# Totoro97/f2-nerf

Hardware: NVIDIA B200
Metric: training rays/sec (higher is better)
Workload: dtype f32 march/composite, f16 hash table + MLP operands (f32 accumulate)

## Files before the change

f2nerf_b200/_lib.py:

```python
import ctypes
import os

import torch

_HERE = os.path.dirname(os.path.abspath(__file__))
LIB_PATH = os.path.join(_HERE, "libf2nerf_b200.so")


class F2BError(RuntimeError):
    """Raised when a C-ABI call returns a negative status (message from f2b_last_error)."""


def _load():
    if not os.path.exists(LIB_PATH):
        raise ImportError(
            f"f2nerf_b200: CUDA extension {LIB_PATH} is missing — run `python -c 'import __graft_entry__ as g; g.build()'` "
            "(or `make`) first; there is no CPU fallback.")
    lib = ctypes.CDLL(LIB_PATH)
    lib.f2b_last_error.restype = ctypes.c_char_p
    return lib


lib = _load()

c_int, c_float, c_void_p, c_i64 = ctypes.c_int, ctypes.c_float, ctypes.c_void_p, ctypes.c_int64

_P = c_void_p
SIGNATURES = {
    "f2b_abi_version": [],
    "f2b_device_info": [_P, _P],
    "f2b_sampler_count": [_P, c_int, _P, c_int, _P, _P, _P, c_int, c_float, c_float, c_float, c_int, c_int, c_int, _P, _P, _P, _P],
    "f2b_sampler_fill": [_P, c_int, _P, c_int, _P, _P, _P, c_int, c_float, c_float, c_float, c_int, c_int, _P, _P, _P, _P, _P, _P, _P, _P],
    "f2b_sampler_march": [_P, c_int, _P, c_int, _P, _P, _P, c_int, c_float, c_float, c_float, c_int, c_int, c_int, _P, _P, _P, _P,
                          _P, _P, _P, _P, _P],
    "f2b_sampler_march_bg": [_P, c_int, _P, c_int, _P, _P, _P, c_int, c_float, c_float, c_float, c_int, c_int, c_int, _P, _P, _P, _P,
                             _P, _P, _P, _P, _P],
    "f2b_sampler_gather": [_P, _P, c_int, _P, _P, _P, _P, _P, _P, _P, _P, _P, _P],
    "f2b_edge_samples": [_P, _P, _P, _P, c_int, _P, _P, _P],
    "f2b_oct_mark_visit": [_P, c_int, _P, c_int, _P, _P, _P, _P, _P, _P, _P],
    "f2b_oct_update_stats": [_P, _P, _P, _P, _P, _P, c_int, _P],
    "f2b_hash_level_scales": [_P],
    "f2b_table_to_half": [_P, _P, c_i64, _P],
    "f2b_hash_fwd": [_P, _P, _P, c_int, c_int, _P, _P, c_int, c_int, _P, _P],
    "f2b_hash_fwd_levels": [_P, _P, _P, c_int, c_int, _P, _P, c_int, c_int, c_int, c_int, _P, _P],
    "f2b_hash_bwd": [_P, _P, c_int, c_int, _P, _P, c_int, c_int, _P, c_int, c_float, _P, _P],
    "f2b_hash_bwd_levels": [_P, _P, c_int, c_int, _P, _P, c_int, c_int, _P, c_int, c_float, _P, c_int, c_int, _P],
    "f2b_mlp_fwd": [_P, _P, c_int, c_int, _P, _P, _P],
    "f2b_mlp_fwd_f32": [_P, _P, c_int, c_int, _P, _P, _P, _P],
    "f2b_mlp_bwd": [_P, _P, _P, _P, c_int, c_int, _P, _P, _P],
    "f2b_field_shade_fwd": [_P, _P, _P, _P, _P, c_int, _P, _P, _P, _P],
    "f2b_shader_mlp_rgb_fwd": [_P, _P, c_int, _P, _P, _P, _P],
    "f2b_mlp_bwd2": [_P, _P, _P, _P, _P, c_int, c_int, _P, _P, _P],
    "f2b_mlp_fwd_v0": [_P, _P, c_int, c_int, _P, _P, _P],
    "f2b_mlp_bwd_v0": [_P, _P, _P, _P, c_int, c_int, _P, _P, _P],
    "f2b_mlp_fwd_tc": [_P, _P, c_int, c_int, _P, _P, _P],
    "f2b_mlp_bwd_tc": [_P, _P, _P, _P, c_int, c_int, _P, _P, _P],
    "f2b_field_fwd": [_P, _P, _P, c_int, c_int, _P, _P, _P, c_int, c_int, c_int, _P, _P, _P, _P],
    "f2b_field_fwd_slots": [_P, _P, _P, c_int, c_int, _P, _P, _P, c_int, _P, c_int, c_int, c_int, _P, _P, _P],
    "f2b_set_mlp_impl": [c_int],
    "f2b_get_mlp_impl": [],
    "f2b_cast_f32_to_f16": [_P, _P, c_i64, c_float, _P],
    "f2b_cast_f16_to_f32": [_P, _P, c_i64, c_float, _P],
    "f2b_sh_encode": [_P, c_int, c_int, _P, _P],
    "f2b_scatter_idx": [_P, _P, c_int, _P, _P],
    "f2b_shader_prep": [_P, _P, _P, _P, c_int, _P, _P],
    "f2b_shader_act": [_P, c_int, _P, _P],
    "f2b_shader_act_bwd": [_P, _P, c_int, c_float, _P, _P],
    "f2b_shader_prep_bwd": [_P, _P, _P, c_int, c_float, _P, _P, _P],
    "f2b_shader_prep_bwd_f16": [_P, _P, _P, _P, c_int, c_float, c_float, _P, _P, _P],
    "f2b_octree_proc": [_P, _P, _P, _P, c_int, c_int, c_int, _P, _P, _P, _P, _P, _P, _P],
    "f2b_octree_mark_invisible": [_P, c_int, _P, _P, _P, c_int, _P],
    "f2b_img2world_rays": [_P, _P, _P, _P, _P, c_int, _P, _P, _P],
    "f2b_gather_pixels": [_P, _P, _P, c_int, c_int, c_int, _P, _P],
    "f2b_adam_step": [_P, _P, _P, _P, c_i64, c_i64, ctypes.c_double, ctypes.c_double, ctypes.c_double, ctypes.c_double,
                      ctypes.c_double, c_i64, _P, _P],
    "f2b_early_stop": [_P, c_int, _P, _P, c_int, _P, _P, _P, _P, _P, _P, _P],
    "f2b_early_stop_rays": [_P, c_int, _P, _P, c_int, _P, _P, _P, _P, _P],
    "f2b_count_scan": [_P, c_int, _P, _P, _P],
    "f2b_slot_bounds": [_P, c_int, c_int, c_int, _P, _P],
    "f2b_compact_slots": [_P, _P, _P, c_int, _P, _P, _P, _P, _P, _P, _P, _P, _P, _P, _P, _P, _P],
    "f2b_compact_samples": [_P, _P, _P, c_int, _P, _P, _P, _P, _P, _P, _P, _P, _P, _P, _P, _P, _P],
    "f2b_composite_fwd": [_P, c_int, _P, _P, _P, _P, _P, c_int, _P, _P, _P, _P, _P],
    "f2b_composite_bwd": [_P, c_int, _P, _P, _P, _P, _P, c_int, _P, _P, _P, _P, c_float, _P, c_int, _P, _P],
    "f2b_composite_act_bwd": [_P, c_int, _P, _P, _P, _P, _P, c_int, _P, _P, _P, _P, c_float, _P, c_float, _P, c_int, _P, _P],
    "f2b_flex_sum": [_P, c_int, _P, c_int, _P, _P],
    "f2b_flex_accumulate_sum": [_P, _P, c_int, c_int, _P, _P],
    "f2b_weight_var_fwd": [_P, _P, c_int, _P, _P],
    "f2b_weight_var_bwd": [_P, _P, c_int, _P, _P, _P],
    "f2b_render_fwd_fused": [_P, _P, _P, c_int, c_int, _P, _P, _P, _P, _P, _P, _P, _P, _P, c_int, c_int, _P, _P, _P, _P, _P, _P, _P, _P],
    "f2b_gather_kept_weights": [_P, _P, c_int, c_int, _P, _P],
}



class RenderArgs(ctypes.Structure):
    _P, _I, _F, _L = c_void_p, c_int, c_float, c_i64
    _fields_ = [
        ("tree_nodes", _P), ("n_nodes", _I), ("trans", _P), ("n_trans", _I), ("edge_pool", _P),
        ("near_t", _F), ("far_t", _F), ("sample_l", _F), ("scale_by_dis", _I), ("max_hits", _I), ("count_all_hits", _I),
        ("table16", _P), ("prim", _P), ("bias", _P), ("n_volumes", _I), ("local_size", _I),
        ("field_params", _P), ("n_field_params", _I), ("shader_params", _P), ("n_shader_params", _I),
        ("fparams16", _P), ("sparams16", _P),
        ("app_emb", _P), ("n_emb", _I),
        ("n_rays", _I), ("rays_o", _P), ("rays_d", _P), ("noise", _P), ("bg", _P),
        ("ray_emb_idx", _P),
        ("skip_march", _I),
        ("s_pts", _P), ("s_dt", _P), ("s_t", _P), ("s_anchors", _P), ("counts", _P), ("chunk_bounds", _P), ("slot_bounds", _P),
        ("first_oct_dis", _P), ("totals", _P),
        ("logit_s", _P), ("feat_s", _P), ("w0", _P), ("a0", _P), ("keep", _P), ("kept_counts", _P), ("new_bounds", _P), ("total_kept", _P),
        ("n_kept", _I), ("n_edge_pairs", _I),
        ("pts", _P), ("dirs", _P), ("dt", _P), ("t", _P), ("anchors", _P), ("feat_q", _P),
        ("edge_idx", _P), ("edge_coord", _P), ("e_pts", _P), ("e_anc", _P),
        ("pt_emb_idx", _P),
        ("logit", _P), ("mlp_in", _P), ("f_hidden", _P), ("edge32", _P), ("raw", _P), ("rgb", _P), ("s_hidden", _P),
        ("colors", _P), ("disparity", _P), ("depth", _P), ("weights", _P),
        ("d_colors", _P), ("d_disparity", _P), ("d_depth", _P), ("d_weights", _P), ("d_edge", _P),
        ("gs_progress", _F), ("shader_loss_scale", _F), ("field_loss_scale", _F), ("table_grad_mul", _F),
        ("d_logit", _P), ("d_raw", _P), ("d_in16", _P), ("d_scene16", _P), ("dfeat16", _P),
        ("d_sparams", _P), ("d_fparams", _P), ("d_table", _P), ("table_numel", _L), ("table_live", _L), ("d_app", _P),
        ("scatter_mode", _I),
        ("nonfinite", _P),
        ("stream", _P), ("side_stream", _P),
    ]

    def set(self, **kw):
        for k, v in kw.items():
            if isinstance(v, torch.Tensor):
                if not v.is_contiguous():
                    raise ValueError(f"f2nerf_b200: tensor {k} crossing the C ABI must be contiguous")
                v = v.data_ptr()
            setattr(self, k, v)
        return self


SIGNATURES["f2b_render_sizeof"] = []
for _name in ("f2b_render_phase1", "f2b_render_phase2_fwd", "f2b_render_bwd", "f2b_render_grad_finalize"):
    SIGNATURES[_name] = [ctypes.POINTER(RenderArgs)]
lib.f2b_render_sizeof.restype = c_int
lib.f2b_render_sizeof.argtypes = []
if lib.f2b_render_sizeof() != ctypes.sizeof(RenderArgs):
    raise ImportError(f"f2nerf_b200: struct f2b_render is {lib.f2b_render_sizeof()} bytes in the library but "
                      f"{ctypes.sizeof(RenderArgs)} in the binding — header / _lib.py out of step")

for _name, _args in SIGNATURES.items():
    _fn = getattr(lib, _name)
    _fn.argtypes = _args
    _fn.restype = c_int


def ptr(t):
    if t is None:
        return None
    if isinstance(t, torch.Tensor):
        if not t.is_contiguous():
            raise ValueError("f2nerf_b200: tensor crossing the C ABI must be contiguous")
        return t.data_ptr()
    return t


def stream():
    return torch.cuda.current_stream().cuda_stream


KERNELS_PER_CALL = {"f2b_render_sizeof": 0, "f2b_render_phase1": 7, "f2b_render_phase2_fwd": 10, "f2b_render_bwd": 8, "f2b_render_grad_finalize": 2,
                    "f2b_sampler_count": 2, "f2b_sampler_march": 2, "f2b_sampler_march_bg": 2, "f2b_early_stop": 2, "f2b_hash_level_scales": 1, "f2b_device_info": 0,
                    "f2b_abi_version": 0, "f2b_set_mlp_impl": 0, "f2b_get_mlp_impl": 0}
LAUNCHES = 0
TRACE = None


def call(name, *args):
    global LAUNCHES
    fn = getattr(lib, name)
    conv = [ptr(a) if isinstance(a, torch.Tensor) or a is None else (ctypes.byref(a) if isinstance(a, ctypes.Structure) else a)
            for a in args]
    if TRACE is not None:
        e0, e1 = torch.cuda.Event(enable_timing=True), torch.cuda.Event(enable_timing=True)
        e0.record()
        rc = fn(*conv)
        e1.record()
        TRACE.append((name, e0, e1, [a for a in args if isinstance(a, int) and not isinstance(a, bool)]))
    else:
        rc = fn(*conv)
    if rc != 0:
        raise F2BError(f"{name} -> {rc}: {lib.f2b_last_error().decode()}")
    LAUNCHES += KERNELS_PER_CALL.get(name, 1)
    return rc
```

f2nerf_b200/csrc/hash.cu:

```cuda
#include "common.cuh"
#include "hash.cuh"
#include <stdlib.h>

namespace f2b {

__global__ void __launch_bounds__(128)
hash_fwd_kernel(const __half* __restrict__ table, const int* __restrict__ prim_pool,
                const float* __restrict__ bias_pool, int n_volumes, int local_size,
                const float* __restrict__ pts, const int* __restrict__ vol, int vol_stride, int n_pts,
                __half* __restrict__ out) {
  __shared__ float s_scale[F2B_N_LEVELS];
  if (threadIdx.x < F2B_N_LEVELS) s_scale[threadIdx.x] = level_scale(threadIdx.x);
  __syncthreads();
  const int i = blockIdx.x * blockDim.x + threadIdx.x;
  if (i >= n_pts) return;
  uint32_t o[16];
  encode_point(table, prim_pool, bias_pool, n_volumes, local_size, s_scale, __ldg(pts + size_t(i) * 3),
               __ldg(pts + size_t(i) * 3 + 1), __ldg(pts + size_t(i) * 3 + 2),
               __ldg(vol + size_t(i) * vol_stride), o);
  uint4* dst = reinterpret_cast<uint4*>(out + size_t(i) * 32);
#pragma unroll
  for (int q = 0; q < 4; q++) dst[q] = make_uint4(o[4 * q], o[4 * q + 1], o[4 * q + 2], o[4 * q + 3]);
}

__global__ void __launch_bounds__(128)
hash_fwd_levels_kernel(const __half* __restrict__ table, const int* __restrict__ prim_pool,
                       const float* __restrict__ bias_pool, int n_volumes, int local_size,
                       const float* __restrict__ pts, const int* __restrict__ vol, int vol_stride, int n_pts,
                       int level_lo, int n_levels, __half* __restrict__ out) {
  __shared__ float s_scale[F2B_N_LEVELS];
  if (threadIdx.x < F2B_N_LEVELS) s_scale[threadIdx.x] = level_scale(threadIdx.x);
  __syncthreads();
  const int i = blockIdx.x * blockDim.x + threadIdx.x;
  if (i >= n_pts) return;
  const float p0 = __ldg(pts + size_t(i) * 3), p1 = __ldg(pts + size_t(i) * 3 + 1), p2 = __ldg(pts + size_t(i) * 3 + 2);
  const float x0 = fmul(fadd(p0, 1.f), .5f), x1 = fmul(fadd(p1, 1.f), .5f), x2 = fmul(fadd(p2, 1.f), .5f);
  const int v = __ldg(vol + size_t(i) * vol_stride);
  uint32_t* dst = reinterpret_cast<uint32_t*>(out + size_t(i) * 32);
  for (int l = level_lo; l < level_lo + n_levels; l++) {
    const int tv = l * n_volumes + v;
    Corner8 c;
    corners(x0, x1, x2, s_scale[l], prim_pool + tv * 3, bias_pool + tv * 3, (unsigned)local_size, c);
    dst[l] = encode_level(table, l, local_size, c);
  }
}

constexpr int kDirectHeads = 24;

template <bool GRAD_F16>
__device__ __forceinline__ void hash_bwd_task(int64_t group, int l, int lane, const int* __restrict__ prim_pool,
                                              const float* __restrict__ bias_pool, int n_volumes, int local_size,
                                              const float* __restrict__ pts, const int* __restrict__ vol, int vol_stride, int n_pts,
                                              const void* __restrict__ grad_feat, float grad_mul, float* __restrict__ grad_table) {
  const int64_t i = group * 32 + lane;
  const bool valid = i < n_pts;
  float g0 = 0.f, g1 = 0.f;
  if (valid) {
    if (GRAD_F16) {
      const float2 gf = __half22float2(reinterpret_cast<const __half2*>(grad_feat)[i * 16 + l]);
      g0 = gf.x; g1 = gf.y;
    } else {
      const float2 gf = reinterpret_cast<const float2*>(grad_feat)[i * 16 + l];
      g0 = gf.x; g1 = gf.y;
    }
  }
  const bool live = valid && !(g0 == 0.f && g1 == 0.f);
  if (!__any_sync(0xffffffffu, live)) return;
  g0 *= grad_mul; g1 *= grad_mul;
  Corner8 c;
  int v = -1;
  if (live) {
    const float p0 = __ldg(pts + i * 3), p1 = __ldg(pts + i * 3 + 1), p2 = __ldg(pts + i * 3 + 2);
    const float x0 = fmul(fadd(p0, 1.f), .5f), x1 = fmul(fadd(p1, 1.f), .5f), x2 = fmul(fadd(p2, 1.f), .5f);
    v = __ldg(vol + i * vol_stride);
    const int tv = l * n_volumes + v;
    corners(x0, x1, x2, level_scale(l), prim_pool + tv * 3, bias_pool + tv * 3, (unsigned)local_size, c);
  } else {
#pragma unroll
    for (int k = 0; k < 8; k++) { c.idx[k] = 0; c.w[k] = 0.f; }
    c.cell[0] = c.cell[1] = c.cell[2] = 0;
  }
  const unsigned pcx = __shfl_up_sync(0xffffffffu, c.cell[0], 1), pcy = __shfl_up_sync(0xffffffffu, c.cell[1], 1),
                 pcz = __shfl_up_sync(0xffffffffu, c.cell[2], 1);
  const int prev_v = __shfl_up_sync(0xffffffffu, v, 1);
  const bool head = (lane == 0) || !live || c.cell[0] != pcx || c.cell[1] != pcy || c.cell[2] != pcz || v != prev_v;
  const unsigned heads = __ballot_sync(0xffffffffu, head);
  float* base = grad_table + size_t(l) * local_size;
  if (__popc(heads) > kDirectHeads) {
    if (live) {
#pragma unroll
      for (int k = 0; k < 8; k++)
        atomicAdd(reinterpret_cast<float2*>(base + size_t(c.idx[k]) * 2), make_float2(c.w[k] * g0, c.w[k] * g1));
    }
    return;
  }
  const unsigned below = heads & ((2u << lane) - 1u);
  const int run_start = 31 - __clz(below);
  float s[16];
#pragma unroll
  for (int k = 0; k < 8; k++) { s[2 * k] = c.w[k] * g0; s[2 * k + 1] = c.w[k] * g1; }
  const int max_run = __reduce_max_sync(0xffffffffu, lane - run_start + 1);
#pragma unroll
  for (int o = 1; o < 32; o <<= 1) {
    if (o >= max_run) break;
    const bool take = (lane - o) >= run_start;
#pragma unroll
    for (int k = 0; k < 16; k++) {
      const float u = __shfl_up_sync(0xffffffffu, s[k], o);
      if (take) s[k] += u;
    }
  }
  const bool tail = (lane == 31) || ((heads >> (lane + 1)) & 1u);
  if (live && tail) {
#pragma unroll
    for (int k = 0; k < 8; k++)
      atomicAdd(reinterpret_cast<float2*>(base + size_t(c.idx[k]) * 2), make_float2(s[2 * k], s[2 * k + 1]));
  }
}

template <bool GRAD_F16>
__global__ void __launch_bounds__(256)
hash_bwd_kernel(const int* __restrict__ prim_pool, const float* __restrict__ bias_pool, int n_volumes,
                int local_size, const float* __restrict__ pts, const int* __restrict__ vol,
                int vol_stride, int n_pts, const void* __restrict__ grad_feat, float grad_mul,
                float* __restrict__ grad_table, int64_t n_tasks, int level_lo, int log2_levels) {
  const int lane = threadIdx.x & 31;
  const int64_t stride = (int64_t(gridDim.x) * blockDim.x) >> 5;
  const int lmask = (1 << log2_levels) - 1;
  int k = 0;
  for (int64_t w = (int64_t(blockIdx.x) * blockDim.x + threadIdx.x) >> 5; w < n_tasks; w += stride, k++)
    hash_bwd_task<GRAD_F16>(w >> log2_levels, level_lo + ((int(w & lmask) + k) & lmask), lane, prim_pool, bias_pool, n_volumes, local_size,
                            pts, vol, vol_stride, n_pts, grad_feat, grad_mul, grad_table);
}

__global__ void level_scales_kernel(float* out) {
  if (threadIdx.x < F2B_N_LEVELS) out[threadIdx.x] = level_scale(threadIdx.x);
}

}

using namespace f2b;

extern "C" int f2b_hash_level_scales(float* scales16_host) {
  F2B_REQUIRE(scales16_host, "f2b_hash_level_scales: null pointer");
  float* d = nullptr;
  if (cudaMalloc(&d, 16 * sizeof(float)) != cudaSuccess) { set_error("f2b_hash_level_scales: cudaMalloc failed"); cudaGetLastError(); return F2B_ECUDA; }
  level_scales_kernel<<<1, 32>>>(d);
  cudaError_t e = cudaMemcpy(scales16_host, d, 16 * sizeof(float), cudaMemcpyDeviceToHost);
  cudaFree(d);
  if (e != cudaSuccess) { set_error("f2b_hash_level_scales: %s", cudaGetErrorString(e)); return F2B_ECUDA; }
  return F2B_OK;
}

extern "C" int f2b_hash_fwd(const void* table_f16, const int* prim_pool, const float* bias_pool,
                            int n_volumes, int local_size, const float* pts, const int* vol,
                            int vol_stride, int n_pts, void* out_f16, void* stream) {
  if (n_pts <= 0) return F2B_OK;
  F2B_REQUIRE(table_f16 && prim_pool && bias_pool && pts && vol && out_f16, "f2b_hash_fwd: null pointer");
  F2B_REQUIRE(n_volumes > 0 && local_size > 0 && (local_size % 2) == 0, "f2b_hash_fwd: bad n_volumes/local_size");
  hash_fwd_kernel<<<div_up(n_pts, 128), 128, 0, as_stream(stream)>>>(
      (const __half*)table_f16, prim_pool, bias_pool, n_volumes, local_size, pts, vol, vol_stride, n_pts,
      (__half*)out_f16);
  return check_launch("f2b_hash_fwd");
}

extern "C" int f2b_hash_fwd_levels(const void* table_f16, const int* prim_pool, const float* bias_pool,
                                   int n_volumes, int local_size, const float* pts, const int* vol,
                                   int vol_stride, int n_pts, int level_lo, int n_levels, void* out_f16, void* stream) {
  if (n_pts <= 0) return F2B_OK;
  F2B_REQUIRE(table_f16 && prim_pool && bias_pool && pts && vol && out_f16, "f2b_hash_fwd_levels: null pointer");
  F2B_REQUIRE(n_volumes > 0 && local_size > 0 && (local_size % 2) == 0, "f2b_hash_fwd_levels: bad n_volumes/local_size");
  F2B_REQUIRE(level_lo >= 0 && n_levels > 0 && level_lo + n_levels <= F2B_N_LEVELS, "f2b_hash_fwd_levels: level range outside [0,16)");
  hash_fwd_levels_kernel<<<div_up(n_pts, 128), 128, 0, as_stream(stream)>>>(
      (const __half*)table_f16, prim_pool, bias_pool, n_volumes, local_size, pts, vol, vol_stride, n_pts, level_lo, n_levels,
      (__half*)out_f16);
  return check_launch("f2b_hash_fwd_levels");
}

extern "C" int f2b_hash_bwd_levels(const int* prim_pool, const float* bias_pool, int n_volumes, int local_size,
                                   const float* pts, const int* vol, int vol_stride, int n_pts,
                                   const void* grad_feat, int grad_is_f16, float grad_mul, float* grad_table,
                                   int level_lo, int n_levels, void* stream) {
  if (n_pts <= 0) return F2B_OK;
  F2B_REQUIRE(prim_pool && bias_pool && pts && vol && grad_feat && grad_table, "f2b_hash_bwd: null pointer");
  F2B_REQUIRE(n_levels > 0 && (n_levels & (n_levels - 1)) == 0 && level_lo >= 0 && level_lo + n_levels <= F2B_N_LEVELS,
              "f2b_hash_bwd_levels: n_levels must be a power of two and the range inside [0,16)");
  int log2_levels = 0;
  while ((1 << log2_levels) < n_levels) log2_levels++;
  const int64_t n_tasks = int64_t(div_up(n_pts, 32)) * n_levels;
  static int ctas_per_sm = -1;
  if (ctas_per_sm < 0) { const char* e = getenv("F2B_SCATTER_CTAS"); ctas_per_sm = e ? atoi(e) : 8; if (ctas_per_sm < 1) ctas_per_sm = 1; }
  int sms = 148;
  f2b_device_info(&sms, nullptr);
  const int64_t want = div_up(n_tasks * 32, int64_t(256));
  int blocks = int(want < int64_t(sms) * ctas_per_sm ? want : int64_t(sms) * ctas_per_sm);
  if (blocks < want && ((blocks * 8) % n_levels) != 0) blocks = blocks > 1 ? blocks - 1 : int(want);
  if (grad_is_f16)
    hash_bwd_kernel<true><<<blocks, 256, 0, as_stream(stream)>>>(prim_pool, bias_pool, n_volumes, local_size, pts, vol, vol_stride,
                                                                 n_pts, grad_feat, grad_mul, grad_table, n_tasks, level_lo, log2_levels);
  else
    hash_bwd_kernel<false><<<blocks, 256, 0, as_stream(stream)>>>(prim_pool, bias_pool, n_volumes, local_size, pts, vol, vol_stride,
                                                                  n_pts, grad_feat, grad_mul, grad_table, n_tasks, level_lo, log2_levels);
  return check_launch("f2b_hash_bwd");
}

extern "C" int f2b_hash_bwd(const int* prim_pool, const float* bias_pool, int n_volumes, int local_size,
                            const float* pts, const int* vol, int vol_stride, int n_pts,
                            const void* grad_feat, int grad_is_f16, float grad_mul, float* grad_table,
                            void* stream) {
  return f2b_hash_bwd_levels(prim_pool, bias_pool, n_volumes, local_size, pts, vol, vol_stride, n_pts, grad_feat, grad_is_f16, grad_mul,
                             grad_table, 0, F2B_N_LEVELS, stream);
}
```

f2nerf_b200/csrc/hash.cuh:

```cuda
#pragma once
#include "common.cuh"

namespace f2b {

__device__ __forceinline__ float level_scale(int l) {
  return exp2f(fadd(fdiv((float)(7 * l), 15.f), 3.f));
}

struct Corner8 {
  unsigned idx[8];
  float w[8];
  unsigned cell[3];
};

__device__ __forceinline__ void corners(float x0, float x1, float x2, float scale,
                                        const int* __restrict__ prim, const float* __restrict__ bias,
                                        unsigned local_size, Corner8& c) {
  const float px = ffma(x0, scale, __ldg(bias)), py = ffma(x1, scale, __ldg(bias + 1)),
              pz = ffma(x2, scale, __ldg(bias + 2));
  const float fx = floorf(px), fy = floorf(py), fz = floorf(pz);
  const unsigned ix = (unsigned)fx, iy = (unsigned)fy, iz = (unsigned)fz;
  c.cell[0] = ix; c.cell[1] = iy; c.cell[2] = iz;
  const unsigned pa = (unsigned)__ldg(prim), pb = (unsigned)__ldg(prim + 1), pc = (unsigned)__ldg(prim + 2);
  const unsigned hx0 = ix * pa, hx1 = hx0 + pa, hy0 = iy * pb, hy1 = hy0 + pb, hz0 = iz * pc, hz1 = hz0 + pc;
  const bool pow2 = (local_size & (local_size - 1)) == 0;
  const unsigned mask = local_size - 1;
#define F2B_MOD(v) (pow2 ? ((v) & mask) : ((v) % local_size))
  c.idx[0] = F2B_MOD(hx0 ^ hy0 ^ hz0);
  c.idx[1] = F2B_MOD(hx0 ^ hy0 ^ hz1);
  c.idx[2] = F2B_MOD(hx0 ^ hy1 ^ hz0);
  c.idx[3] = F2B_MOD(hx0 ^ hy1 ^ hz1);
  c.idx[4] = F2B_MOD(hx1 ^ hy0 ^ hz0);
  c.idx[5] = F2B_MOD(hx1 ^ hy0 ^ hz1);
  c.idx[6] = F2B_MOD(hx1 ^ hy1 ^ hz0);
  c.idx[7] = F2B_MOD(hx1 ^ hy1 ^ hz1);
#undef F2B_MOD
  const float a = fsub(px, fx), b = fsub(py, fy), cc = fsub(pz, fz);
  const float na = fsub(1.f, a), nb = fsub(1.f, b), nc = fsub(1.f, cc);
  const float nanb = fmul(na, nb), nab = fmul(na, b), anb = fmul(a, nb), ab = fmul(a, b);
  c.w[0] = fmul(nanb, nc); c.w[1] = fmul(cc, nanb);
  c.w[2] = fmul(nab, nc);  c.w[3] = fmul(nab, cc);
  c.w[4] = fmul(anb, nc);  c.w[5] = fmul(cc, anb);
  c.w[6] = fmul(ab, nc);   c.w[7] = fmul(ab, cc);
}

__device__ __forceinline__ uint32_t ldg_nc_u32(const void* p) {
  uint32_t v;
  asm volatile("ld.global.nc.b32 %0, [%1];" : "=r"(v) : "l"(p));
  return v;
}

__device__ __forceinline__ uint32_t encode_level(const __half* __restrict__ table, int l, int local_size,
                                                 const Corner8& c) {
  const __half* base = table + size_t(l) * local_size;
  uint32_t raw[8];
#pragma unroll
  for (int k = 0; k < 8; k++) raw[k] = ldg_nc_u32(base + size_t(c.idx[k]) * 2);
  float2 f[8];
#pragma unroll
  for (int k = 0; k < 8; k++) f[k] = __half22float2(*reinterpret_cast<const __half2*>(&raw[k]));
  float a0 = fmul(c.w[1], f[1].x), a1 = fmul(c.w[1], f[1].y);
  a0 = ffma(c.w[0], f[0].x, a0); a1 = ffma(c.w[0], f[0].y, a1);
#pragma unroll
  for (int k = 2; k < 8; k++) { a0 = ffma(c.w[k], f[k].x, a0); a1 = ffma(c.w[k], f[k].y, a1); }
  const __half2 h = __floats2half2_rn(a0, a1);
  return *reinterpret_cast<const uint32_t*>(&h);
}

__device__ __forceinline__ void encode_point(const __half* __restrict__ table,
                                             const int* __restrict__ prim_pool,
                                             const float* __restrict__ bias_pool, int n_volumes,
                                             int local_size, const float* scales, float p0, float p1,
                                             float p2, int v, uint32_t out[16]) {
  const float x0 = fmul(fadd(p0, 1.f), .5f), x1 = fmul(fadd(p1, 1.f), .5f), x2 = fmul(fadd(p2, 1.f), .5f);
#pragma unroll
  for (int l = 0; l < F2B_N_LEVELS; l++) {
    const int tv = l * n_volumes + v;
    Corner8 c;
    corners(x0, x1, x2, scales[l], prim_pool + tv * 3, bias_pool + tv * 3, (unsigned)local_size, c);
    out[l] = encode_level(table, l, local_size, c);
  }
}

}
```

f2nerf_b200/csrc/mlp_tc_bwd.cu:

```cuda
#include "common.cuh"
#include "tc.cuh"

namespace f2b {
using namespace tc;

constexpr int kBT = 128;

template <int NH>
struct BwdSmem {
  static constexpr int W0 = 0;
  static constexpr int WH = 4096;
  static constexpr int WO = NH ? 12288 : 4096;
  static constexpr int STAGE0 = WO + 2048;
  static constexpr int DO = 0;
  static constexpr int X = 4096;
  static constexpr int H0 = 12288;
  static constexpr int H1 = 28672;
  static constexpr int STAGE_BYTES = NH ? 45056 : 28672;
  static constexpr int BAR = STAGE0 + 2 * STAGE_BYTES;
  static constexpr int BYTES = BAR + 64 + 1024;
  static constexpr int TMEM_COLS = NH ? 256 : 128;
  static constexpr int C_ACT = 0, C_GW0 = 64, C_GWO = 96, C_GWH = 128;
};

__device__ __forceinline__ uint32_t pk(float a, float b) {
  const __half2 h = __floats2half2_rn(a, b);
  return *reinterpret_cast<const uint32_t*>(&h);
}

__device__ __forceinline__ uint64_t mnmajor_desc(uint32_t tile, int row_bytes, int k_step) {
  const uint64_t layout = row_bytes == 128 ? kLayoutSW128 : (row_bytes == 64 ? kLayoutSW64 : kLayoutSW32);
  return make_desc(tile + k_step * 16 * row_bytes, 16, 8 * row_bytes, layout);
}

template <int K>
__device__ __forceinline__ void stage_w(const __half* __restrict__ w, int rows, unsigned char* dst) {
  constexpr int chunks = K / 8;
  for (int i = threadIdx.x; i < rows * chunks; i += blockDim.x) {
    const int r = i / chunks, c = i % chunks;
    *reinterpret_cast<uint4*>(dst + (K == 64 ? sw128_off(r, c) : sw64_off(r, c))) = *reinterpret_cast<const uint4*>(w + r * K + c * 8);
  }
}

__device__ __forceinline__ void cp16(uint32_t dst, const void* src, uint32_t src_bytes) {
  asm volatile("cp.async.cg.shared.global [%0], [%1], 16, %2;" ::"r"(dst), "l"(src), "r"(src_bytes) : "memory");
}

template <int NH>
__device__ __forceinline__ void prefetch_tile(const __half* __restrict__ dout, const __half* __restrict__ in,
                                              const __half* __restrict__ hidden, const __half* __restrict__ hid_last,
                                              int tile, int n_pts, uint32_t stage) {
  using S = BwdSmem<NH>;
  const int rows = min(kBT, n_pts - tile * kBT);
  const size_t t0 = size_t(tile) * kBT;
  const unsigned char* s_do = reinterpret_cast<const unsigned char*>(dout + t0 * 16);
  const unsigned char* s_x = reinterpret_cast<const unsigned char*>(in + t0 * 32);
  const unsigned char* s_h0 = reinterpret_cast<const unsigned char*>(hidden + t0 * 64);
  const unsigned char* s_h1 = reinterpret_cast<const unsigned char*>(hid_last + t0 * 64);
#pragma unroll
  for (int j = 0; j < 2; j++) {
    const int c = threadIdx.x + kBT * j, r = c >> 1;
    const bool ok = r < rows;
    cp16(stage + S::DO + sw32_off(r, c & 1), s_do + (ok ? size_t(c) * 16 : 0), ok ? 16u : 0u);
  }
#pragma unroll
  for (int j = 0; j < 4; j++) {
    const int c = threadIdx.x + kBT * j, r = c >> 2;
    const bool ok = r < rows;
    cp16(stage + S::X + sw64_off(r, c & 3), s_x + (ok ? size_t(c) * 16 : 0), ok ? 16u : 0u);
  }
#pragma unroll
  for (int j = 0; j < 8; j++) {
    const int c = threadIdx.x + kBT * j, r = c >> 3;
    const bool ok = r < rows;
    cp16(stage + S::H0 + sw128_off(r, c & 7), s_h0 + (ok ? size_t(c) * 16 : 0), ok ? 16u : 0u);
    if (NH) cp16(stage + S::H1 + sw128_off(r, c & 7), s_h1 + (ok ? size_t(c) * 16 : 0), ok ? 16u : 0u);
  }
}

__device__ __forceinline__ void relu_bwd_epilogue(uint32_t tmem_row, const unsigned char* h_tile, unsigned char* dh_tile, int row) {
#pragma unroll
  for (int q = 0; q < 4; q++) {
    uint32_t r[16];
    tmem_ld16(tmem_row + 16 * q, r);
    tmem_ld_wait();
    uint4 hv[2], o[2];
    hv[0] = *reinterpret_cast<const uint4*>(h_tile + sw128_off(row, 2 * q));
    hv[1] = *reinterpret_cast<const uint4*>(h_tile + sw128_off(row, 2 * q + 1));
    const __half2* hh = reinterpret_cast<const __half2*>(hv);
    uint32_t* ow = reinterpret_cast<uint32_t*>(o);
#pragma unroll
    for (int e = 0; e < 8; e++) {
      const float2 hf = __half22float2(hh[e]);
      ow[e] = pk(hf.x > 0.f ? __uint_as_float(r[2 * e]) : 0.f, hf.y > 0.f ? __uint_as_float(r[2 * e + 1]) : 0.f);
    }
    *reinterpret_cast<uint4*>(dh_tile + sw128_off(row, 2 * q)) = o[0];
    *reinterpret_cast<uint4*>(dh_tile + sw128_off(row, 2 * q + 1)) = o[1];
  }
}

template <int NH>
__global__ void __launch_bounds__(kBT)
mlp_bwd_tc_kernel(const __half* __restrict__ dout, const __half* __restrict__ in, const __half* __restrict__ hidden,
                  const __half* __restrict__ hid_last, const __half* __restrict__ params, int n_pts,
                  __half* __restrict__ din, float* __restrict__ dparams) {
  using S = BwdSmem<NH>;
  extern __shared__ unsigned char smem_raw[];
  unsigned char* sm = reinterpret_cast<unsigned char*>((reinterpret_cast<uintptr_t>(smem_raw) + 1023) & ~uintptr_t(1023));
  uint64_t* mbar = reinterpret_cast<uint64_t*>(sm + S::BAR);
  uint32_t* tmem_slot = reinterpret_cast<uint32_t*>(sm + S::BAR + 8);
  const int tid = threadIdx.x, warp = tid >> 5, lane = tid & 31;
  const int n_tiles = (n_pts + kBT - 1) / kBT;
  const uint32_t stage0 = smem_u32(sm + S::STAGE0);

  int tile = blockIdx.x;
  if (tile < n_tiles) prefetch_tile<NH>(dout, in, hidden, hid_last, tile, n_pts, stage0);
  asm volatile("cp.async.commit_group;" ::: "memory");
  stage_w<32>(params, 64, sm + S::W0);
  if (NH) stage_w<64>(params + 64 * 32, 64, sm + S::WH);
  stage_w<64>(params + 64 * 32 + NH * 64 * 64, 16, sm + S::WO);
  if (tid == 0) mbar_init(mbar, 1);
  if (warp == 0) tmem_alloc(tmem_slot, S::TMEM_COLS);
  fence_before_sync();
  __syncthreads();
  fence_after_sync();
  const uint32_t tmem = *tmem_slot;
  const uint32_t tmem_row = tmem + (uint32_t(warp * 32) << 16);
  const uint32_t s_w0 = smem_u32(sm + S::W0), s_wh = smem_u32(sm + S::WH), s_wo = smem_u32(sm + S::WO);
  constexpr uint32_t id_act64 = idesc_f16_f32(128, 64, 0, 1);
  constexpr uint32_t id_act32 = idesc_f16_f32(128, 32, 0, 1);
  constexpr uint32_t id_gw16 = idesc_f16_f32(64, 16, 1, 1);
  constexpr uint32_t id_gw32 = idesc_f16_f32(64, 32, 1, 1);
  constexpr uint32_t id_gw64 = idesc_f16_f32(64, 64, 1, 1);
  uint32_t phase = 0, first = 1, buf = 0;

  for (; tile < n_tiles; tile += gridDim.x, buf ^= 1) {
    const int p = tile * kBT + tid;
    const bool valid = p < n_pts;
    const int next = tile + gridDim.x;
    if (next < n_tiles) prefetch_tile<NH>(dout, in, hidden, hid_last, next, n_pts, stage0 + (buf ^ 1) * S::STAGE_BYTES);
    asm volatile("cp.async.commit_group;" ::: "memory");
    asm volatile("cp.async.wait_group 1;" ::: "memory");
    fence_async_smem();
    fence_before_sync();
    __syncthreads();
    unsigned char* const st = sm + S::STAGE0 + buf * S::STAGE_BYTES;
    const uint32_t sb = stage0 + buf * S::STAGE_BYTES;
    const uint32_t s_do = sb + S::DO, s_x = sb + S::X, s_h0 = sb + S::H0, s_h1 = sb + S::H1;
    const uint32_t s_hl = NH ? s_h1 : s_h0;
    const uint32_t acc = (first ^ 1);
    if (tid == 0) {
      fence_after_sync();
      mma_f16(tmem + S::C_ACT, kmajor_desc(s_do, 32), mnmajor_desc(s_wo, 128, 0), id_act64, 0);
#pragma unroll
      for (int k = 0; k < 8; k++)
        mma_f16(tmem + S::C_GWO, mnmajor_desc(s_hl, 128, k), mnmajor_desc(s_do, 32, k), id_gw16, (k > 0) | acc);
      mma_commit(mbar);
    }
    mbar_wait(mbar, phase); phase ^= 1;
    fence_after_sync();
    relu_bwd_epilogue(tmem_row + S::C_ACT, st + (NH ? S::H1 : S::H0), st + (NH ? S::H1 : S::H0), tid);
    fence_before_sync();
    fence_async_smem();
    __syncthreads();
    if (NH) {
      if (tid == 0) {
        fence_after_sync();
#pragma unroll
        for (int k = 0; k < 4; k++)
          mma_f16(tmem + S::C_ACT, kmajor_desc(s_h1 + 32 * k, 128), mnmajor_desc(s_wh, 128, k), id_act64, k);
#pragma unroll
        for (int k = 0; k < 8; k++)
          mma_f16(tmem + S::C_GWH, mnmajor_desc(s_h1, 128, k), mnmajor_desc(s_h0, 128, k), id_gw64, (k > 0) | acc);
        mma_commit(mbar);
      }
      mbar_wait(mbar, phase); phase ^= 1;
      fence_after_sync();
      relu_bwd_epilogue(tmem_row + S::C_ACT, st + S::H0, st + S::H0, tid);
      fence_before_sync();
      fence_async_smem();
      __syncthreads();
    }
    if (tid == 0) {
      fence_after_sync();
#pragma unroll
      for (int k = 0; k < 4; k++)
        mma_f16(tmem + S::C_ACT, kmajor_desc(s_h0 + 32 * k, 128), mnmajor_desc(s_w0, 64, k), id_act32, k);
#pragma unroll
      for (int k = 0; k < 8; k++)
        mma_f16(tmem + S::C_GW0, mnmajor_desc(s_h0, 128, k), mnmajor_desc(s_x, 64, k), id_gw32, (k > 0) | acc);
      mma_commit(mbar);
    }
    first = 0;
    mbar_wait(mbar, phase); phase ^= 1;
    fence_after_sync();
    {
#pragma unroll
      for (int q = 0; q < 2; q++) {
        uint32_t r[16];
        tmem_ld16(tmem_row + S::C_ACT + 16 * q, r);
        tmem_ld_wait();
        if (din && valid) {
          uint4 o[2];
          uint32_t* ow = reinterpret_cast<uint32_t*>(o);
#pragma unroll
          for (int e = 0; e < 8; e++) ow[e] = pk(__uint_as_float(r[2 * e]), __uint_as_float(r[2 * e + 1]));
          uint4* dst = reinterpret_cast<uint4*>(din + size_t(p) * 32) + 2 * q;
          dst[0] = o[0]; dst[1] = o[1];
        }
      }
    }
  }
  asm volatile("cp.async.wait_group 0;" ::: "memory");
  fence_before_sync();
  __syncthreads();
  if (!first) {
    fence_after_sync();
    const int row = warp * 16 + lane;
    float* g0 = dparams;
    float* gh = dparams + 64 * 32;
    float* go = gh + NH * 64 * 64;
#pragma unroll
    for (int q = 0; q < 2; q++) {
      uint32_t r[16];
      tmem_ld16(tmem_row + S::C_GW0 + 16 * q, r);
      tmem_ld_wait();
      if (lane < 16)
#pragma unroll
        for (int e = 0; e < 16; e++) atomicAdd(g0 + row * 32 + 16 * q + e, __uint_as_float(r[e]));
    }
    {
      uint32_t r[16];
      tmem_ld16(tmem_row + S::C_GWO, r);
      tmem_ld_wait();
      if (lane < 16)
#pragma unroll
        for (int e = 0; e < 16; e++) atomicAdd(go + e * 64 + row, __uint_as_float(r[e]));
    }
    if (NH) {
#pragma unroll
      for (int q = 0; q < 4; q++) {
        uint32_t r[16];
        tmem_ld16(tmem_row + S::C_GWH + 16 * q, r);
        tmem_ld_wait();
        if (lane < 16)
#pragma unroll
          for (int e = 0; e < 16; e++) atomicAdd(gh + row * 64 + 16 * q + e, __uint_as_float(r[e]));
      }
    }
    fence_before_sync();
  }
  __syncthreads();
  if (warp == 0) tmem_dealloc(tmem, S::TMEM_COLS);
}


template <int NH>
struct RcSmem {
  static constexpr int W0 = 0;
  static constexpr int WH = 4096;
  static constexpr int WO = NH ? 12288 : 4096;
  static constexpr int H0 = WO + 2048;
  static constexpr int H1 = H0 + 16384;
  static constexpr int D1 = H1 + 16384;
  static constexpr int STAGE0 = NH ? D1 + 16384 : H0 + 16384;
  static constexpr int DO = 0;
  static constexpr int X = 4096;
  static constexpr int STAGE_BYTES = 12288;
  static constexpr int BAR = STAGE0 + 2 * STAGE_BYTES;
  static constexpr int BYTES = BAR + 64 + 1024;
  static constexpr int TMEM_COLS = NH ? 256 : 128;
  static constexpr int C_ACT = 0, C_GW0 = 64, C_GWO = 96, C_GWH = 128, C_ACT2 = 192;
};

template <int NH>
__device__ __forceinline__ void prefetch_tile_rc(const __half* __restrict__ dout, const __half* __restrict__ in, int tile, int n_pts,
                                                 uint32_t stage) {
  using S = RcSmem<NH>;
  const int rows = min(kBT, n_pts - tile * kBT);
  const size_t t0 = size_t(tile) * kBT;
  const unsigned char* s_do = reinterpret_cast<const unsigned char*>(dout + t0 * 16);
  const unsigned char* s_x = reinterpret_cast<const unsigned char*>(in + t0 * 32);
#pragma unroll
  for (int j = 0; j < 2; j++) {
    const int c = threadIdx.x + kBT * j, r = c >> 1;
    const bool ok = r < rows;
    cp16(stage + S::DO + sw32_off(r, c & 1), s_do + (ok ? size_t(c) * 16 : 0), ok ? 16u : 0u);
  }
#pragma unroll
  for (int j = 0; j < 4; j++) {
    const int c = threadIdx.x + kBT * j, r = c >> 2;
    const bool ok = r < rows;
    cp16(stage + S::X + sw64_off(r, c & 3), s_x + (ok ? size_t(c) * 16 : 0), ok ? 16u : 0u);
  }
}

__device__ __forceinline__ void relu_fwd_epilogue(uint32_t tmem_row, unsigned char* h_tile, int row) {
#pragma unroll
  for (int q = 0; q < 4; q++) {
    uint32_t r[16];
    tmem_ld16(tmem_row + 16 * q, r);
    tmem_ld_wait();
    uint4 o[2];
    uint32_t* ow = reinterpret_cast<uint32_t*>(o);
#pragma unroll
    for (int e = 0; e < 8; e++) ow[e] = pk(fmaxf(__uint_as_float(r[2 * e]), 0.f), fmaxf(__uint_as_float(r[2 * e + 1]), 0.f));
    *reinterpret_cast<uint4*>(h_tile + sw128_off(row, 2 * q)) = o[0];
    *reinterpret_cast<uint4*>(h_tile + sw128_off(row, 2 * q + 1)) = o[1];
  }
}

__device__ __forceinline__ void relu_fwd_mask_epilogue(uint32_t tmem_h, uint32_t tmem_g, unsigned char* h_tile, unsigned char* d_tile, int row) {
#pragma unroll
  for (int q = 0; q < 4; q++) {
    uint32_t r[16], g[16];
    tmem_ld16(tmem_h + 16 * q, r);
    tmem_ld16(tmem_g + 16 * q, g);
    tmem_ld_wait();
    uint4 o[2], d[2];
    uint32_t* ow = reinterpret_cast<uint32_t*>(o);
    uint32_t* dw = reinterpret_cast<uint32_t*>(d);
#pragma unroll
    for (int e = 0; e < 8; e++) {
      const __half2 h = __floats2half2_rn(fmaxf(__uint_as_float(r[2 * e]), 0.f), fmaxf(__uint_as_float(r[2 * e + 1]), 0.f));
      ow[e] = *reinterpret_cast<const uint32_t*>(&h);
      const float2 hf = __half22float2(h);
      dw[e] = pk(hf.x > 0.f ? __uint_as_float(g[2 * e]) : 0.f, hf.y > 0.f ? __uint_as_float(g[2 * e + 1]) : 0.f);
    }
    *reinterpret_cast<uint4*>(h_tile + sw128_off(row, 2 * q)) = o[0];
    *reinterpret_cast<uint4*>(h_tile + sw128_off(row, 2 * q + 1)) = o[1];
    *reinterpret_cast<uint4*>(d_tile + sw128_off(row, 2 * q)) = d[0];
    *reinterpret_cast<uint4*>(d_tile + sw128_off(row, 2 * q + 1)) = d[1];
  }
}

template <int NH>
__global__ void __launch_bounds__(kBT)
mlp_bwd_rc_kernel(const __half* __restrict__ dout, const __half* __restrict__ in, const __half* __restrict__ params, int n_pts,
                  __half* __restrict__ din, float* __restrict__ dparams) {
  using S = RcSmem<NH>;
  extern __shared__ unsigned char smem_raw[];
  unsigned char* sm = reinterpret_cast<unsigned char*>((reinterpret_cast<uintptr_t>(smem_raw) + 1023) & ~uintptr_t(1023));
  uint64_t* mbar = reinterpret_cast<uint64_t*>(sm + S::BAR);
  uint32_t* tmem_slot = reinterpret_cast<uint32_t*>(sm + S::BAR + 8);
  const int tid = threadIdx.x, warp = tid >> 5, lane = tid & 31;
  const int n_tiles = (n_pts + kBT - 1) / kBT;
  const uint32_t stage0 = smem_u32(sm + S::STAGE0);

  int tile = blockIdx.x;
  if (tile < n_tiles) prefetch_tile_rc<NH>(dout, in, tile, n_pts, stage0);
  asm volatile("cp.async.commit_group;" ::: "memory");
  stage_w<32>(params, 64, sm + S::W0);
  if (NH) stage_w<64>(params + 64 * 32, 64, sm + S::WH);
  stage_w<64>(params + 64 * 32 + NH * 64 * 64, 16, sm + S::WO);
  if (tid == 0) mbar_init(mbar, 1);
  if (warp == 0) tmem_alloc(tmem_slot, S::TMEM_COLS);
  fence_before_sync();
  __syncthreads();
  fence_after_sync();
  const uint32_t tmem = *tmem_slot;
  const uint32_t tmem_row = tmem + (uint32_t(warp * 32) << 16);
  const uint32_t s_w0 = smem_u32(sm + S::W0), s_wh = smem_u32(sm + S::WH), s_wo = smem_u32(sm + S::WO);
  const uint32_t s_h0 = smem_u32(sm + S::H0), s_h1 = smem_u32(sm + S::H1), s_d1 = smem_u32(sm + S::D1);
  constexpr uint32_t id_fwd64 = idesc_f16_f32(128, 64);
  constexpr uint32_t id_act64 = idesc_f16_f32(128, 64, 0, 1);
  constexpr uint32_t id_act32 = idesc_f16_f32(128, 32, 0, 1);
  constexpr uint32_t id_gw16 = idesc_f16_f32(64, 16, 1, 1);
  constexpr uint32_t id_gw32 = idesc_f16_f32(64, 32, 1, 1);
  constexpr uint32_t id_gw64 = idesc_f16_f32(64, 64, 1, 1);
  uint32_t phase = 0, first = 1, buf = 0;

  for (; tile < n_tiles; tile += gridDim.x, buf ^= 1) {
    const int p = tile * kBT + tid;
    const bool valid = p < n_pts;
    const int next = tile + gridDim.x;
    if (next < n_tiles) prefetch_tile_rc<NH>(dout, in, next, n_pts, stage0 + (buf ^ 1) * S::STAGE_BYTES);
    asm volatile("cp.async.commit_group;" ::: "memory");
    asm volatile("cp.async.wait_group 1;" ::: "memory");
    fence_async_smem();
    fence_before_sync();
    __syncthreads();
    const uint32_t sb = stage0 + buf * S::STAGE_BYTES;
    const uint32_t s_do = sb + S::DO, s_x = sb + S::X;
    const uint32_t acc = (first ^ 1);
    if (tid == 0) {
      fence_after_sync();
#pragma unroll
      for (int k = 0; k < 2; k++) mma_f16(tmem + S::C_ACT, kmajor_desc(s_x + 32 * k, 64), kmajor_desc(s_w0 + 32 * k, 64), id_fwd64, k);
      if (NH) mma_f16(tmem + S::C_ACT2, kmajor_desc(s_do, 32), mnmajor_desc(s_wo, 128, 0), id_act64, 0);
      mma_commit(mbar);
    }
    mbar_wait(mbar, phase); phase ^= 1;
    fence_after_sync();
    relu_fwd_epilogue(tmem_row + S::C_ACT, sm + S::H0, tid);
    fence_before_sync();
    fence_async_smem();
    __syncthreads();
    if (NH) {
      if (tid == 0) {
        fence_after_sync();
#pragma unroll
        for (int k = 0; k < 4; k++) mma_f16(tmem + S::C_ACT, kmajor_desc(s_h0 + 32 * k, 128), kmajor_desc(s_wh + 32 * k, 128), id_fwd64, k);
        mma_commit(mbar);
      }
      mbar_wait(mbar, phase); phase ^= 1;
      fence_after_sync();
      relu_fwd_mask_epilogue(tmem_row + S::C_ACT, tmem_row + S::C_ACT2, sm + S::H1, sm + S::D1, tid);
      fence_before_sync();
      fence_async_smem();
      __syncthreads();
      if (tid == 0) {
        fence_after_sync();
#pragma unroll
        for (int k = 0; k < 8; k++)
          mma_f16(tmem + S::C_GWO, mnmajor_desc(s_h1, 128, k), mnmajor_desc(s_do, 32, k), id_gw16, (k > 0) | acc);
#pragma unroll
        for (int k = 0; k < 4; k++)
          mma_f16(tmem + S::C_ACT, kmajor_desc(s_d1 + 32 * k, 128), mnmajor_desc(s_wh, 128, k), id_act64, k);
#pragma unroll
        for (int k = 0; k < 8; k++)
          mma_f16(tmem + S::C_GWH, mnmajor_desc(s_d1, 128, k), mnmajor_desc(s_h0, 128, k), id_gw64, (k > 0) | acc);
        mma_commit(mbar);
      }
    } else {
      if (tid == 0) {
        fence_after_sync();
        mma_f16(tmem + S::C_ACT, kmajor_desc(s_do, 32), mnmajor_desc(s_wo, 128, 0), id_act64, 0);
#pragma unroll
        for (int k = 0; k < 8; k++)
          mma_f16(tmem + S::C_GWO, mnmajor_desc(s_h0, 128, k), mnmajor_desc(s_do, 32, k), id_gw16, (k > 0) | acc);
        mma_commit(mbar);
      }
    }
    mbar_wait(mbar, phase); phase ^= 1;
    fence_after_sync();
    relu_bwd_epilogue(tmem_row + S::C_ACT, sm + S::H0, sm + S::H0, tid);
    fence_before_sync();
    fence_async_smem();
    __syncthreads();
    if (tid == 0) {
      fence_after_sync();
#pragma unroll
      for (int k = 0; k < 4; k++)
        mma_f16(tmem + S::C_ACT, kmajor_desc(s_h0 + 32 * k, 128), mnmajor_desc(s_w0, 64, k), id_act32, k);
#pragma unroll
      for (int k = 0; k < 8; k++)
        mma_f16(tmem + S::C_GW0, mnmajor_desc(s_h0, 128, k), mnmajor_desc(s_x, 64, k), id_gw32, (k > 0) | acc);
      mma_commit(mbar);
    }
    first = 0;
    mbar_wait(mbar, phase); phase ^= 1;
    fence_after_sync();
#pragma unroll
    for (int q = 0; q < 2; q++) {
      uint32_t r[16];
      tmem_ld16(tmem_row + S::C_ACT + 16 * q, r);
      tmem_ld_wait();
      if (din && valid) {
        uint4 o[2];
        uint32_t* ow = reinterpret_cast<uint32_t*>(o);
#pragma unroll
        for (int e = 0; e < 8; e++) ow[e] = pk(__uint_as_float(r[2 * e]), __uint_as_float(r[2 * e + 1]));
        uint4* dst = reinterpret_cast<uint4*>(din + size_t(p) * 32) + 2 * q;
        dst[0] = o[0]; dst[1] = o[1];
      }
    }
  }
  asm volatile("cp.async.wait_group 0;" ::: "memory");
  fence_before_sync();
  __syncthreads();
  if (!first) {
    fence_after_sync();
    const int row = warp * 16 + lane;
    float* g0 = dparams;
    float* gh = dparams + 64 * 32;
    float* go = gh + NH * 64 * 64;
#pragma unroll
    for (int q = 0; q < 2; q++) {
      uint32_t r[16];
      tmem_ld16(tmem_row + S::C_GW0 + 16 * q, r);
      tmem_ld_wait();
      if (lane < 16)
#pragma unroll
        for (int e = 0; e < 16; e++) atomicAdd(g0 + row * 32 + 16 * q + e, __uint_as_float(r[e]));
    }
    {
      uint32_t r[16];
      tmem_ld16(tmem_row + S::C_GWO, r);
      tmem_ld_wait();
      if (lane < 16)
#pragma unroll
        for (int e = 0; e < 16; e++) atomicAdd(go + e * 64 + row, __uint_as_float(r[e]));
    }
    if (NH) {
#pragma unroll
      for (int q = 0; q < 4; q++) {
        uint32_t r[16];
        tmem_ld16(tmem_row + S::C_GWH + 16 * q, r);
        tmem_ld_wait();
        if (lane < 16)
#pragma unroll
          for (int e = 0; e < 16; e++) atomicAdd(gh + row * 64 + 16 * q + e, __uint_as_float(r[e]));
      }
    }
    fence_before_sync();
  }
  __syncthreads();
  if (warp == 0) tmem_dealloc(tmem, S::TMEM_COLS);
}

}

using namespace f2b;

extern "C" int f2b_mlp_bwd2_tc(const void* dout_f16, const void* in_f16, const void* hidden0_f16, const void* hidden1_f16,
                               const void* params_f16, int n_hidden_matmuls, int n_pts, void* din_f16,
                               float* dparams_f32, void* stream) {
  if (n_pts <= 0) return F2B_OK;
  F2B_REQUIRE(dout_f16 && in_f16 && params_f16 && dparams_f32, "f2b_mlp_bwd: null pointer");
  F2B_REQUIRE(n_hidden_matmuls == 0 || n_hidden_matmuls == 1, "f2b_mlp_bwd: n_hidden_matmuls must be 0 or 1");
  int sms = 148;
  f2b_device_info(&sms, nullptr);
  const int n_tiles = div_up(n_pts, kBT);
  if (!hidden0_f16) {
    if (n_hidden_matmuls == 0) {
      const int grid = n_tiles < sms * 4 ? n_tiles : sms * 4;
      cudaFuncSetAttribute(mlp_bwd_rc_kernel<0>, cudaFuncAttributeMaxDynamicSharedMemorySize, RcSmem<0>::BYTES);
      mlp_bwd_rc_kernel<0><<<grid, kBT, RcSmem<0>::BYTES, as_stream(stream)>>>((const __half*)dout_f16, (const __half*)in_f16,
                                                                              (const __half*)params_f16, n_pts, (__half*)din_f16, dparams_f32);
    } else {
      const int grid = n_tiles < sms * 2 ? n_tiles : sms * 2;
      cudaFuncSetAttribute(mlp_bwd_rc_kernel<1>, cudaFuncAttributeMaxDynamicSharedMemorySize, RcSmem<1>::BYTES);
      mlp_bwd_rc_kernel<1><<<grid, kBT, RcSmem<1>::BYTES, as_stream(stream)>>>((const __half*)dout_f16, (const __half*)in_f16,
                                                                              (const __half*)params_f16, n_pts, (__half*)din_f16, dparams_f32);
    }
    return check_launch("f2b_mlp_bwd(tcgen05, recompute)");
  }
  F2B_REQUIRE(n_hidden_matmuls == 0 || hidden1_f16, "f2b_mlp_bwd: hidden1 missing (n_hidden_matmuls == 1 with saved activations)");
  if (n_hidden_matmuls == 0) {
    const int grid = n_tiles < sms * 3 ? n_tiles : sms * 3;
    cudaFuncSetAttribute(mlp_bwd_tc_kernel<0>, cudaFuncAttributeMaxDynamicSharedMemorySize, BwdSmem<0>::BYTES);
    mlp_bwd_tc_kernel<0><<<grid, kBT, BwdSmem<0>::BYTES, as_stream(stream)>>>(
        (const __half*)dout_f16, (const __half*)in_f16, (const __half*)hidden0_f16, (const __half*)hidden0_f16,
        (const __half*)params_f16, n_pts, (__half*)din_f16, dparams_f32);
  } else {
    const int grid = n_tiles < sms * 2 ? n_tiles : sms * 2;
    cudaFuncSetAttribute(mlp_bwd_tc_kernel<1>, cudaFuncAttributeMaxDynamicSharedMemorySize, BwdSmem<1>::BYTES);
    mlp_bwd_tc_kernel<1><<<grid, kBT, BwdSmem<1>::BYTES, as_stream(stream)>>>(
        (const __half*)dout_f16, (const __half*)in_f16, (const __half*)hidden0_f16, (const __half*)hidden1_f16,
        (const __half*)params_f16, n_pts, (__half*)din_f16, dparams_f32);
  }
  return check_launch("f2b_mlp_bwd(tcgen05)");
}

extern "C" int f2b_mlp_bwd_tc(const void* dout_f16, const void* in_f16, const void* hidden_save_f16,
                              const void* params_f16, int n_hidden_matmuls, int n_pts, void* din_f16,
                              float* dparams_f32, void* stream) {
  if (n_pts <= 0) return F2B_OK;
  F2B_REQUIRE(hidden_save_f16, "f2b_mlp_bwd: null pointer");
  const __half* h = (const __half*)hidden_save_f16;
  return f2b_mlp_bwd2_tc(dout_f16, in_f16, h, h + size_t(n_hidden_matmuls ? 1 : 0) * n_pts * 64, params_f16, n_hidden_matmuls, n_pts,
                         din_f16, dparams_f32, stream);
}
```

f2nerf_b200/csrc/render.cu:

```cuda
#include "common.cuh"

namespace f2b {

__global__ void finalize_small_kernel(float* __restrict__ d_sparams, int n_s, float inv_s, float* __restrict__ d_fparams, int n_f,
                                      float inv_f, const float* __restrict__ d_app, int n_app, int* __restrict__ flags) {
  const int i = blockIdx.x * blockDim.x + threadIdx.x;
  int bad_s = 0, bad_f = 0;
  if (i < n_s) { const float v = d_sparams[i] * inv_s; d_sparams[i] = v; bad_s |= !isfinite(v); }
  if (i < n_f) { const float v = d_fparams[i] * inv_f; d_fparams[i] = v; bad_f |= !isfinite(v); }
  if (d_app && i < n_app) bad_s |= !isfinite(d_app[i]);
  if (__any_sync(0xffffffffu, bad_s) && (threadIdx.x & 31) == 0) atomicOr(flags, 1);
  if (__any_sync(0xffffffffu, bad_f) && (threadIdx.x & 31) == 0) atomicOr(flags + 1, 1);
}
__global__ void finalize_table_kernel(const float4* __restrict__ g, int64_t n4, int* __restrict__ flags) {
  int bad = 0;
  for (int64_t i = int64_t(blockIdx.x) * blockDim.x + threadIdx.x; i < n4; i += int64_t(gridDim.x) * blockDim.x) {
    const float4 v = g[i];
    bad |= !(isfinite(v.x) && isfinite(v.y) && isfinite(v.z) && isfinite(v.w));
  }
  if (__any_sync(0xffffffffu, bad) && (threadIdx.x & 31) == 0) atomicOr(flags + 1, 1);
}

}

using namespace f2b;

#define F2B_TRY(expr)            \
  do {                           \
    const int rc_ = (expr);      \
    if (rc_ != F2B_OK) return rc_; \
  } while (0)
#define F2B_CUDA(expr, what)                                                                          \
  do {                                                                                                \
    const cudaError_t e_ = (expr);                                                                    \
    if (e_ != cudaSuccess) { set_error("%s: CUDA error %d (%s)", what, (int)e_, cudaGetErrorString(e_)); return F2B_ECUDA; } \
  } while (0)

static inline char* off(void* p, int64_t bytes) { return reinterpret_cast<char*>(p) + bytes; }

extern "C" int f2b_render_sizeof(void) { return (int)sizeof(f2b_render); }

extern "C" int f2b_render_phase1(const f2b_render* r) {
  F2B_REQUIRE(r, "f2b_render_phase1: null argument block");
  if (r->n_rays <= 0) return F2B_OK;
  const int S = F2B_MAX_SAMPLE_PER_RAY;
  if (!r->skip_march) {
    F2B_TRY(f2b_sampler_march(r->tree_nodes, r->n_nodes, r->trans, r->n_trans, r->rays_o, r->rays_d, r->noise, r->n_rays, r->near_t,
                              r->far_t, r->sample_l, r->scale_by_dis, r->max_hits, r->count_all_hits, r->s_pts, r->s_dt, r->s_t,
                              r->s_anchors, r->counts, r->chunk_bounds, r->totals, r->first_oct_dis, r->stream));
    F2B_TRY(f2b_slot_bounds(r->counts, r->n_rays, S, 0, r->slot_bounds, r->stream));
  }
  F2B_TRY(f2b_cast_f32_to_f16(r->field_params, r->fparams16, r->n_field_params, 1.f, r->stream));
  F2B_TRY(f2b_field_fwd_slots(r->table16, r->prim, r->bias, r->n_volumes, r->local_size, r->fparams16, r->s_pts, r->s_anchors, 2,
                              r->counts, r->n_rays, S, 1, r->logit_s, r->feat_s, r->stream));
  F2B_TRY(f2b_early_stop_rays(r->logit_s, 1, r->s_dt, r->slot_bounds, r->n_rays, r->w0, r->a0, r->keep, r->kept_counts, r->stream));
  F2B_CUDA(cudaMemsetAsync(r->total_kept, 0, sizeof(int), as_stream(r->stream)), "f2b_render_phase1");
  return f2b_count_scan(r->kept_counts, r->n_rays, r->new_bounds, r->total_kept, r->stream);
}

extern "C" int f2b_render_phase2_fwd(const f2b_render* r) {
  F2B_REQUIRE(r, "f2b_render_phase2_fwd: null argument block");
  if (r->n_rays <= 0) return F2B_OK;
  const int64_t nk = r->n_kept, ne = 2 * int64_t(r->n_edge_pairs);
  F2B_TRY(f2b_compact_slots(r->keep, r->slot_bounds, r->new_bounds, r->n_rays, r->rays_d, r->s_pts, r->s_dt, r->s_t, r->s_anchors,
                            r->feat_s, r->pts, r->dirs, r->dt, r->t, r->anchors, r->feat_q, r->stream));
  if (ne > 0) {
    F2B_TRY(f2b_edge_samples(r->edge_pool, r->trans, r->edge_idx, r->edge_coord, r->n_edge_pairs, r->e_pts, r->e_anc, r->stream));
    F2B_TRY(f2b_hash_fwd(r->table16, r->prim, r->bias, r->n_volumes, r->local_size, r->e_pts, r->e_anc, 1, (int)ne,
                         off(r->feat_q, nk * 64), r->stream));
  }
  const bool emb = r->app_emb && r->ray_emb_idx;
  if (emb && nk > 0) F2B_TRY(f2b_scatter_idx(r->new_bounds, r->ray_emb_idx, r->n_rays, r->pt_emb_idx, r->stream));
  F2B_TRY(f2b_cast_f32_to_f16(r->field_params, r->fparams16, r->n_field_params, 1.f, r->stream));
  F2B_TRY(f2b_cast_f32_to_f16(r->shader_params, r->sparams16, r->n_shader_params, 1.f, r->stream));
  F2B_TRY(f2b_field_shade_fwd(r->feat_q, r->fparams16, r->dirs, emb ? r->app_emb : nullptr, emb ? r->pt_emb_idx : nullptr, (int)nk,
                              r->logit, r->mlp_in, r->f_hidden, r->stream));
  if (ne > 0)
    F2B_TRY(f2b_mlp_fwd_f32(off(r->feat_q, nk * 64), r->fparams16, 0, (int)ne, r->edge32, nullptr,
                            r->f_hidden ? off(r->f_hidden, nk * 128) : nullptr, r->stream));
  F2B_TRY(f2b_shader_mlp_rgb_fwd(r->mlp_in, r->sparams16, (int)nk, r->raw, r->rgb, r->s_hidden, r->stream));
  return f2b_composite_fwd(r->logit, 1, r->rgb, r->dt, r->t, r->new_bounds, r->bg, r->n_rays, r->colors, r->disparity, r->depth,
                           r->weights, r->stream);
}

extern "C" int f2b_render_bwd(const f2b_render* r) {
  F2B_REQUIRE(r, "f2b_render_bwd: null argument block");
  const int64_t nk = r->n_kept, ne = 2 * int64_t(r->n_edge_pairs), nq = nk + ne;
  cudaStream_t st = as_stream(r->stream), side = as_stream(r->side_stream);
  const bool emb = r->app_emb && r->ray_emb_idx;
  F2B_CUDA(cudaMemsetAsync(r->d_sparams, 0, sizeof(float) * r->n_shader_params, st), "f2b_render_bwd");
  F2B_CUDA(cudaMemsetAsync(r->d_fparams, 0, sizeof(float) * r->n_field_params, st), "f2b_render_bwd");
  F2B_CUDA(cudaMemsetAsync(r->d_table, 0, sizeof(float) * r->table_numel, st), "f2b_render_bwd");
  F2B_CUDA(cudaMemsetAsync(r->nonfinite, 0, 2 * sizeof(int), st), "f2b_render_bwd");
  if (emb) F2B_CUDA(cudaMemsetAsync(r->d_app, 0, sizeof(float) * 16 * r->n_emb, st), "f2b_render_bwd");
  if (ne > 0) {
    if (r->d_edge) F2B_TRY(f2b_cast_f32_to_f16(r->d_edge, off(r->d_scene16, nk * 32), ne * 16, r->field_loss_scale, r->stream));
    else F2B_CUDA(cudaMemsetAsync(off(r->d_scene16, nk * 32), 0, ne * 32, st), "f2b_render_bwd");
  }
  if (nk > 0) {
    F2B_TRY(f2b_composite_act_bwd(r->logit, 1, r->rgb, r->dt, r->t, r->new_bounds, r->bg, r->n_rays, r->d_colors, r->d_disparity,
                                  r->d_depth, r->d_weights, r->gs_progress, r->raw, r->shader_loss_scale, r->d_logit, 1, r->d_raw,
                                  r->stream));
    F2B_TRY(f2b_mlp_bwd2(r->d_raw, r->mlp_in, r->s_hidden, r->s_hidden ? off(r->s_hidden, nk * 128) : nullptr, r->sparams16, 1, (int)nk, r->d_in16, r->d_sparams,
                         r->stream));
    F2B_TRY(f2b_shader_prep_bwd_f16(r->d_in16, r->d_logit, r->new_bounds, emb ? r->ray_emb_idx : nullptr, r->n_rays,
                                    1.f / r->shader_loss_scale, r->field_loss_scale, r->d_scene16, emb ? r->d_app : nullptr, r->stream));
    F2B_TRY(f2b_mlp_bwd2(r->d_scene16, r->feat_q, r->f_hidden, nullptr, r->fparams16, 0, (int)nk, r->dfeat16, r->d_fparams, r->stream));
  }
  if (ne > 0)
    F2B_TRY(f2b_mlp_bwd2(off(r->d_scene16, nk * 32), off(r->feat_q, nk * 64), r->f_hidden ? off(r->f_hidden, nk * 128) : nullptr, nullptr, r->fparams16, 0, (int)ne,
                         off(r->dfeat16, nk * 64), r->d_fparams, r->stream));
  if (r->scatter_mode != 0) return F2B_OK;
  cudaEvent_t fork, join;
  F2B_CUDA(cudaEventCreateWithFlags(&fork, cudaEventDisableTiming), "f2b_render_bwd");
  F2B_CUDA(cudaEventCreateWithFlags(&join, cudaEventDisableTiming), "f2b_render_bwd");
  cudaEventRecord(fork, st);
  cudaStreamWaitEvent(side, fork, 0);
  int rc = F2B_OK;
  if (nk > 0)
    rc = f2b_hash_bwd(r->prim, r->bias, r->n_volumes, r->local_size, r->pts, r->anchors, 3, (int)nk, r->dfeat16, 1, r->table_grad_mul,
                      r->d_table, r->side_stream);
  if (rc == F2B_OK && ne > 0)
    rc = f2b_hash_bwd(r->prim, r->bias, r->n_volumes, r->local_size, r->e_pts, r->e_anc, 1, (int)ne, off(r->dfeat16, nk * 64), 1,
                      r->table_grad_mul, r->d_table, r->side_stream);
  cudaEventRecord(join, side);
  cudaStreamWaitEvent(st, join, 0);
  cudaEventDestroy(fork);
  cudaEventDestroy(join);
  (void)nq;
  return rc;
}

extern "C" int f2b_render_grad_finalize(const f2b_render* r) {
  F2B_REQUIRE(r && r->d_sparams && r->d_fparams && r->nonfinite, "f2b_render_grad_finalize: null pointer");
  const bool emb = r->app_emb && r->ray_emb_idx;
  const int n_app = emb ? 16 * r->n_emb : 0;
  int n = r->n_shader_params > r->n_field_params ? r->n_shader_params : r->n_field_params;
  if (n_app > n) n = n_app;
  finalize_small_kernel<<<div_up(n, 256), 256, 0, as_stream(r->stream)>>>(r->d_sparams, r->n_shader_params, 1.f / r->shader_loss_scale,
                                                                           r->d_fparams, r->n_field_params, 1.f / r->field_loss_scale,
                                                                           emb ? r->d_app : nullptr, n_app, r->nonfinite);
  if (r->d_table && r->table_live >= 4) {
    int sms = 148;
    f2b_device_info(&sms, nullptr);
    finalize_table_kernel<<<sms * 4, 256, 0, as_stream(r->stream)>>>(reinterpret_cast<const float4*>(r->d_table), r->table_live / 4,
                                                                     r->nonfinite);
  }
  return check_launch("f2b_render_grad_finalize");
}
```

f2nerf_b200/csrc/tc.cuh:

```cuda
#pragma once
#include <cuda_runtime.h>
#include <stdint.h>

namespace f2b { namespace tc {

__device__ __forceinline__ uint32_t smem_u32(const void* p) { return (uint32_t)__cvta_generic_to_shared(p); }

enum : uint64_t { kLayoutNone = 0, kLayoutSW128 = 2, kLayoutSW64 = 4, kLayoutSW32 = 6 };

__device__ __forceinline__ uint64_t make_desc(uint32_t saddr, uint32_t lbo_bytes, uint32_t sbo_bytes, uint64_t layout) {
  return (uint64_t)((saddr & 0x3FFFF) >> 4) | ((uint64_t)(lbo_bytes >> 4) << 16) | ((uint64_t)(sbo_bytes >> 4) << 32) |
         (1ull << 46) | (layout << 61);
}
__device__ __forceinline__ uint64_t kmajor_desc(uint32_t saddr, int row_bytes) {
  const uint64_t layout = row_bytes == 128 ? kLayoutSW128 : (row_bytes == 64 ? kLayoutSW64 : kLayoutSW32);
  return make_desc(saddr, 16, 8 * row_bytes, layout);
}
__host__ __device__ constexpr uint32_t idesc_f16_f32(int M, int N, int a_mn_major = 0, int b_mn_major = 0) {
  return (1u << 4) | ((uint32_t)a_mn_major << 15) | ((uint32_t)b_mn_major << 16) | ((uint32_t)(N >> 3) << 17) |
         ((uint32_t)(M >> 4) << 24);
}

__device__ __forceinline__ uint32_t sw128_off(int r, int c) { return r * 128 + ((c ^ (r & 7)) << 4); }
__device__ __forceinline__ uint32_t sw64_off(int r, int c) { return r * 64 + ((c ^ ((r >> 1) & 3)) << 4); }
__device__ __forceinline__ uint32_t sw32_off(int r, int c) { return r * 32 + ((c ^ ((r >> 2) & 1)) << 4); }

__device__ __forceinline__ void tmem_alloc(uint32_t* smem_dst, uint32_t ncols) {
  asm volatile("tcgen05.alloc.cta_group::1.sync.aligned.shared::cta.b32 [%0], %1;" ::"r"(smem_u32(smem_dst)), "r"(ncols) : "memory");
  asm volatile("tcgen05.relinquish_alloc_permit.cta_group::1.sync.aligned;" ::: "memory");
}
__device__ __forceinline__ void tmem_dealloc(uint32_t taddr, uint32_t ncols) {
  asm volatile("tcgen05.dealloc.cta_group::1.sync.aligned.b32 %0, %1;" ::"r"(taddr), "r"(ncols) : "memory");
}
__device__ __forceinline__ void fence_before_sync() { asm volatile("tcgen05.fence::before_thread_sync;" ::: "memory"); }
__device__ __forceinline__ void fence_after_sync() { asm volatile("tcgen05.fence::after_thread_sync;" ::: "memory"); }
__device__ __forceinline__ void fence_async_smem() { asm volatile("fence.proxy.async.shared::cta;" ::: "memory"); }

__device__ __forceinline__ void mma_f16(uint32_t tmem_d, uint64_t adesc, uint64_t bdesc, uint32_t idesc, uint32_t accumulate) {
  asm volatile(
      "{\n\t.reg .pred p;\n\tsetp.ne.b32 p, %4, 0;\n\t"
      "tcgen05.mma.cta_group::1.kind::f16 [%0], %1, %2, %3, p;\n\t}\n" ::"r"(tmem_d),
      "l"(adesc), "l"(bdesc), "r"(idesc), "r"(accumulate)
      : "memory");
}
__device__ __forceinline__ void mma_commit(uint64_t* mbar) {
  asm volatile("tcgen05.commit.cta_group::1.mbarrier::arrive::one.shared::cluster.b64 [%0];" ::"r"(smem_u32(mbar)) : "memory");
}

__device__ __forceinline__ void mbar_init(uint64_t* mbar, uint32_t count) {
  asm volatile("mbarrier.init.shared::cta.b64 [%0], %1;" ::"r"(smem_u32(mbar)), "r"(count) : "memory");
}
__device__ __forceinline__ void mbar_wait(uint64_t* mbar, uint32_t parity) {
  asm volatile(
      "{\n\t.reg .pred P1;\n\tLAB_WAIT:\n\t"
      "mbarrier.try_wait.parity.shared::cta.b64 P1, [%0], %1;\n\t"
      "@P1 bra DONE;\n\tbra LAB_WAIT;\n\tDONE:\n\t}\n" ::"r"(smem_u32(mbar)),
      "r"(parity)
      : "memory");
}

__device__ __forceinline__ void tmem_ld16(uint32_t taddr, uint32_t (&r)[16]) {
  asm volatile(
      "tcgen05.ld.sync.aligned.32x32b.x16.b32 {%0,%1,%2,%3,%4,%5,%6,%7,%8,%9,%10,%11,%12,%13,%14,%15}, [%16];"
      : "=r"(r[0]), "=r"(r[1]), "=r"(r[2]), "=r"(r[3]), "=r"(r[4]), "=r"(r[5]), "=r"(r[6]), "=r"(r[7]), "=r"(r[8]),
        "=r"(r[9]), "=r"(r[10]), "=r"(r[11]), "=r"(r[12]), "=r"(r[13]), "=r"(r[14]), "=r"(r[15])
      : "r"(taddr)
      : "memory");
}
__device__ __forceinline__ void tmem_ld_wait() { asm volatile("tcgen05.wait::ld.sync.aligned;" ::: "memory"); }

}}
```

f2nerf_b200/ops.py:

```python
import torch

from . import _lib
from ._lib import call, stream

F16, F32, I32, U8 = torch.float16, torch.float32, torch.int32, torch.uint8


def _chk(t, dtype, name):
    if not t.is_cuda:
        raise ValueError(f"{name}: expected a CUDA tensor (the reference's CHECK_TS / CUDA* options)")
    if t.dtype != dtype:
        raise ValueError(f"{name}: expected dtype {dtype}, got {t.dtype}")
    if not t.is_contiguous():
        raise ValueError(f"{name}: expected a contiguous tensor (the reference's CK_CONT)")
    return t


def dev_empty(shape, dtype, like):
    return torch.empty(shape, dtype=dtype, device=like.device)


def sampler_count(tree_nodes, trans, rays_o, rays_d, noise, near, far, sample_l, scale_by_dis, max_hits, count_all_hits=True):
    R = rays_o.shape[0]
    counts = dev_empty((max(R, 1),), I32, rays_o)
    bounds = dev_empty((R, 2), I32, rays_o)
    totals = dev_empty((2,), I32, rays_o)
    call("f2b_sampler_count", tree_nodes, tree_nodes.numel() // 64, trans, trans.numel() // 544, rays_o, rays_d,
         noise, R, float(near), float(far), float(sample_l), int(bool(scale_by_dis)), int(max_hits), int(bool(count_all_hits)),
         counts, bounds, totals, stream())
    return bounds, totals


def sampler_fill(tree_nodes, trans, rays_o, rays_d, noise, near, far, sample_l, scale_by_dis, max_hits, bounds, n_pts):
    R = rays_o.shape[0]
    pts = dev_empty((n_pts, 3), F32, rays_o)
    dirs = dev_empty((n_pts, 3), F32, rays_o)
    dt = dev_empty((n_pts,), F32, rays_o)
    t = dev_empty((n_pts,), F32, rays_o)
    anchors = dev_empty((n_pts, 3), I32, rays_o)
    first = dev_empty((R, 1), F32, rays_o)
    call("f2b_sampler_fill", tree_nodes, tree_nodes.numel() // 64, trans, trans.numel() // 544, rays_o, rays_d, noise,
         R, float(near), float(far), float(sample_l), int(bool(scale_by_dis)), int(max_hits), bounds, pts, dirs, dt, t,
         anchors, first, stream())
    return pts, dirs, dt, t, anchors, first


def sampler_march(tree_nodes, trans, rays_o, rays_d, noise, near, far, sample_l, scale_by_dis, max_hits, scratch,
                  count_all_hits=False):
    R = rays_o.shape[0]
    counts = dev_empty((max(R, 1),), I32, rays_o)
    bounds = dev_empty((R, 2), I32, rays_o)
    totals = dev_empty((2,), I32, rays_o)
    first = dev_empty((R, 1), F32, rays_o)
    call("f2b_sampler_march", tree_nodes, tree_nodes.numel() // 64, trans, trans.numel() // 544, rays_o, rays_d, noise, R,
         float(near), float(far), float(sample_l), int(bool(scale_by_dis)), int(max_hits), int(bool(count_all_hits)),
         *scratch, counts, bounds, totals, first, stream())
    return bounds, totals, first


def sampler_gather(rays_d, bounds, n_pts, scratch):
    pts = dev_empty((n_pts, 3), F32, rays_d)
    dirs = dev_empty((n_pts, 3), F32, rays_d)
    dt = dev_empty((n_pts,), F32, rays_d)
    t = dev_empty((n_pts,), F32, rays_d)
    anchors = dev_empty((n_pts, 3), I32, rays_d)
    call("f2b_sampler_gather", rays_d, bounds, bounds.shape[0], *scratch, pts, dirs, dt, t, anchors, stream())
    return pts, dirs, dt, t, anchors


def edge_samples(edge_pool, trans, edge_idx, edge_coord):
    n = edge_idx.shape[0]
    out_pts = dev_empty((n, 2, 3), F32, edge_coord)
    out_idx = dev_empty((n, 2), I32, edge_coord)
    call("f2b_edge_samples", edge_pool, trans, edge_idx, edge_coord, n, out_pts, out_idx, stream())
    return out_pts, out_idx


def hash_level_scales():
    import ctypes
    buf = (ctypes.c_float * 16)()
    call("f2b_hash_level_scales", ctypes.addressof(buf))
    return torch.tensor(list(buf), dtype=F32)


def table_to_half(table_f32):
    out = torch.empty_like(table_f32, dtype=F16)
    call("f2b_table_to_half", table_f32, out, table_f32.numel(), stream())
    return out


def hash_fwd(table_f16, prim_pool, bias_pool, n_volumes, local_size, pts, vol, vol_stride=1):
    n = pts.shape[0]
    out = dev_empty((n, 32), F16, pts)
    call("f2b_hash_fwd", table_f16, prim_pool, bias_pool, int(n_volumes), int(local_size), pts, vol, int(vol_stride), n,
         out, stream())
    return out


def hash_bwd(prim_pool, bias_pool, n_volumes, local_size, pts, vol, vol_stride, grad_feat, grad_mul, grad_table):
    n = pts.shape[0]
    call("f2b_hash_bwd", prim_pool, bias_pool, int(n_volumes), int(local_size), pts, vol, int(vol_stride), n,
         grad_feat, int(grad_feat.dtype == F16), float(grad_mul), grad_table, stream())
    return grad_table


def field_fwd(table_f16, prim_pool, bias_pool, n_volumes, local_size, params_f16, pts, vol, vol_stride=1, logit_only=False,
              save=False, save_feat=None):
    n = pts.shape[0]
    save_feat = save if save_feat is None else save_feat
    out = dev_empty((n,) if logit_only else (n, 16), F32, pts)
    feat = dev_empty((n, 32), F16, pts) if save_feat else None
    hidden = dev_empty((1, n, 64), F16, pts) if (save and not logit_only) else None
    call("f2b_field_fwd", table_f16, prim_pool, bias_pool, int(n_volumes), int(local_size), params_f16, pts, vol,
         int(vol_stride), n, int(bool(logit_only)), out, feat, hidden, stream())
    return out, feat, hidden


def mlp_fwd(x_f16, params_f16, n_hidden_matmuls, save_hidden=False, impl=None):
    n = x_f16.shape[0]
    out = dev_empty((n, 16), F16, x_f16)
    hidden = dev_empty((n_hidden_matmuls + 1, n, 64), F16, x_f16) if save_hidden else None
    name = "f2b_mlp_fwd" if impl is None else f"f2b_mlp_fwd_{impl}"
    call(name, x_f16, params_f16, int(n_hidden_matmuls), n, out, hidden, stream())
    return out, hidden


def mlp_fwd_f32(x_f16, params_f16, n_hidden_matmuls, save_hidden=False, want_f16=False):
    from . import _lib
    n = x_f16.shape[0]
    out32 = dev_empty((n, 16), F32, x_f16)
    out16 = dev_empty((n, 16), F16, x_f16) if (want_f16 or _lib.lib.f2b_get_mlp_impl() != 1) else None
    hidden = dev_empty((n_hidden_matmuls + 1, n, 64), F16, x_f16) if save_hidden else None
    call("f2b_mlp_fwd_f32", x_f16, params_f16, int(n_hidden_matmuls), n, out32, out16, hidden, stream())
    return out32, out16, hidden


def mlp_bwd(dout_f16, x_f16, hidden, params_f16, n_hidden_matmuls, need_din=True, impl=None):
    n = x_f16.shape[0]
    din = dev_empty((n, 32), F16, x_f16) if need_din else None
    dparams = torch.zeros(params_f16.numel(), dtype=F32, device=x_f16.device)
    name = "f2b_mlp_bwd" if impl is None else f"f2b_mlp_bwd_{impl}"
    call(name, dout_f16, x_f16, hidden, params_f16, int(n_hidden_matmuls), n, din, dparams, stream())
    return din, dparams


def cast_f32_to_f16(x, scale=1.0):
    out = torch.empty_like(x, dtype=F16)
    call("f2b_cast_f32_to_f16", x, out, x.numel(), float(scale), stream())
    return out


def cast_f16_to_f32(x, scale=1.0):
    out = torch.empty_like(x, dtype=F32)
    call("f2b_cast_f16_to_f32", x, out, x.numel(), float(scale), stream())
    return out


def sh_encode(dirs, degree=4):
    n = dirs.shape[0]
    out = dev_empty((n, degree * degree), F32, dirs)
    call("f2b_sh_encode", dirs, n, int(degree), out, stream())
    return out


def scatter_idx(n_all_pts, idx_start_end, emb_idx):
    out = dev_empty((n_all_pts,), I32, idx_start_end)
    call("f2b_scatter_idx", idx_start_end, emb_idx, idx_start_end.shape[0], out, stream())
    return out


def shader_prep(scene_feat, dirs, app_emb=None, pt_emb_idx=None):
    n = scene_feat.shape[0]
    out = dev_empty((n, 32), F16, scene_feat)
    call("f2b_shader_prep", scene_feat, dirs, app_emb, pt_emb_idx, n, out, stream())
    return out


def shader_act(raw_f16):
    n = raw_f16.shape[0]
    rgb = dev_empty((n, 3), F32, raw_f16)
    call("f2b_shader_act", raw_f16, n, rgb, stream())
    return rgb


def shader_act_bwd(raw_f16, d_rgb, loss_scale):
    n = raw_f16.shape[0]
    out = dev_empty((n, 16), F16, raw_f16)
    call("f2b_shader_act_bwd", raw_f16, d_rgb, n, float(loss_scale), out, stream())
    return out


def shader_prep_bwd(d_mlp_in_f16, bounds, emb_idx, inv_loss_scale, d_scene_feat, d_app_emb):
    call("f2b_shader_prep_bwd", d_mlp_in_f16, bounds, emb_idx, bounds.shape[0], float(inv_loss_scale), d_scene_feat,
         d_app_emb, stream())


def shader_prep_bwd_f16(d_mlp_in_f16, d_logit, bounds, emb_idx, inv_loss_scale, field_loss_scale, d_field_out_f16, d_app_emb):
    call("f2b_shader_prep_bwd_f16", d_mlp_in_f16, d_logit, bounds, emb_idx, bounds.shape[0], float(inv_loss_scale),
         float(field_loss_scale), d_field_out_f16, d_app_emb, stream())


def early_stop(logit, logit_stride, dt, bounds):
    R, P = bounds.shape[0], dt.shape[0]
    weights, alphas = dev_empty((P,), F32, dt), dev_empty((P,), F32, dt)
    keep = dev_empty((P,), U8, dt)
    counts = dev_empty((max(R, 1),), I32, dt)
    new_bounds = dev_empty((R, 2), I32, dt)
    total = dev_empty((1,), I32, dt)
    call("f2b_early_stop", logit, int(logit_stride), dt, bounds, R, weights, alphas, keep, counts, new_bounds, total,
         stream())
    return weights, alphas, keep, new_bounds, total


def field_fwd_slots(table_f16, prim_pool, bias_pool, n_volumes, local_size, params_f16, slot_pts, slot_anchors, counts, n_rays,
                    slot, out_logit, feat_slots):
    call("f2b_field_fwd_slots", table_f16, prim_pool, bias_pool, int(n_volumes), int(local_size), params_f16, slot_pts,
         slot_anchors, int(slot_anchors.shape[1]), counts, int(n_rays), int(slot), 1, out_logit, feat_slots, stream())


def early_stop_rays(logit, logit_stride, dt, bounds, weights, alphas, keep, counts):
    call("f2b_early_stop_rays", logit, int(logit_stride), dt, bounds, bounds.shape[0], weights, alphas, keep, counts, stream())


def count_scan(counts, n):
    bounds = dev_empty((n, 2), I32, counts)
    total = torch.zeros((1,), dtype=I32, device=counts.device)
    call("f2b_count_scan", counts, int(n), bounds, total, stream())
    return bounds, total


def compact_slots(keep, slot_bounds, new_bounds, rays_d, s_pts, s_dt, s_t, s_anchors, feat_slots, outs, feat_out):
    call("f2b_compact_slots", keep, slot_bounds, new_bounds, slot_bounds.shape[0], rays_d, s_pts, s_dt, s_t, s_anchors,
         feat_slots, *outs, feat_out, stream())


def compact_samples(keep, old_bounds, new_bounds, n_kept, pts, dirs, dt, t, anchors, feat=None, feat_out=None):
    outs = (dev_empty((n_kept, 3), F32, pts), dev_empty((n_kept, 3), F32, pts), dev_empty((n_kept,), F32, pts),
            dev_empty((n_kept,), F32, pts), dev_empty((n_kept, 3), I32, pts))
    call("f2b_compact_samples", keep, old_bounds, new_bounds, old_bounds.shape[0], pts, dirs, dt, t, anchors, feat, *outs,
         feat_out, stream())
    return outs


def composite_fwd(logit, logit_stride, rgb, dt, t, bounds, bg):
    R, P = bounds.shape[0], dt.shape[0]
    colors, disp, depth = dev_empty((R, 3), F32, dt), dev_empty((R,), F32, dt), dev_empty((R,), F32, dt)
    weights = dev_empty((P,), F32, dt)
    call("f2b_composite_fwd", logit, int(logit_stride), rgb, dt, t, bounds, bg, R, colors, disp, depth, weights, stream())
    return colors, disp, depth, weights


def composite_bwd(logit, logit_stride, rgb, dt, t, bounds, bg, d_colors, d_disp, d_depth, d_weights, gs_progress,
                  d_logit, dlogit_stride):
    R, P = bounds.shape[0], dt.shape[0]
    d_rgb = dev_empty((P, 3), F32, dt)
    call("f2b_composite_bwd", logit, int(logit_stride), rgb, dt, t, bounds, bg, R, d_colors, d_disp, d_depth, d_weights,
         float(gs_progress), d_logit, int(dlogit_stride), d_rgb, stream())
    return d_rgb


class _FlexSum(torch.autograd.Function):
    @staticmethod
    def forward(ctx, val, idx_start_end):
        n, vec = idx_start_end.shape[0], (1 if val.dim() == 1 else val.shape[1])
        out = dev_empty((n,) if val.dim() == 1 else (n, vec), F32, val)
        call("f2b_flex_sum", val, vec, idx_start_end, n, out, stream())
        ctx.save_for_backward(idx_start_end)
        ctx.shape = val.shape
        return out

    @staticmethod
    def backward(ctx, g):
        (idx,) = ctx.saved_tensors
        lens = (idx[:, 1] - idx[:, 0]).long()
        return torch.repeat_interleave(g.contiguous(), lens, dim=0).reshape(ctx.shape), None


class _FlexAccumulateSum(torch.autograd.Function):
    @staticmethod
    def forward(ctx, val, idx_start_end, include_this):
        out = torch.empty_like(val)
        call("f2b_flex_accumulate_sum", val, idx_start_end, idx_start_end.shape[0], int(include_this), out, stream())
        ctx.save_for_backward(idx_start_end)
        ctx.include_this = include_this
        return out

    @staticmethod
    def backward(ctx, g):
        (idx,) = ctx.saved_tensors
        g = g.contiguous()
        fwd = torch.empty_like(g)
        call("f2b_flex_accumulate_sum", g, idx, idx.shape[0], int(not ctx.include_this), fwd, stream())
        tot = dev_empty((idx.shape[0],), F32, g)
        call("f2b_flex_sum", g, 1, idx, idx.shape[0], tot, stream())
        lens = (idx[:, 1] - idx[:, 0]).long()
        return torch.repeat_interleave(tot, lens) - fwd, None, None


class FlexOps:

    @staticmethod
    def Sum(val, idx_start_end):
        return _FlexSum.apply(_chk(val.contiguous(), F32, "val"), _chk(idx_start_end.contiguous(), I32, "idx_start_end"))

    @staticmethod
    def AccumulateSum(val, idx_start_end, include_this):
        return _FlexAccumulateSum.apply(_chk(val.contiguous(), F32, "val"),
                                        _chk(idx_start_end.contiguous(), I32, "idx_start_end"), bool(include_this))


class _WeightVar(torch.autograd.Function):
    @staticmethod
    def forward(ctx, weights, idx_start_end):
        n = idx_start_end.shape[0]
        out = dev_empty((n,), F32, weights)
        call("f2b_weight_var_fwd", weights, idx_start_end, n, out, stream())
        ctx.save_for_backward(weights, idx_start_end)
        return out

    @staticmethod
    def backward(ctx, g):
        weights, idx = ctx.saved_tensors
        dw = torch.zeros_like(weights)
        call("f2b_weight_var_bwd", weights, idx, idx.shape[0], g.contiguous(), dw, stream())
        return dw, None


class _TruncExp(torch.autograd.Function):

    @staticmethod
    def forward(ctx, x):
        ctx.save_for_backward(x)
        return torch.exp(x)

    @staticmethod
    def backward(ctx, g):
        (x,) = ctx.saved_tensors
        return g * torch.exp(x.clamp(-100.0, 5.0))


class CustomOps:

    @staticmethod
    def WeightVar(weights, idx_start_end):
        return _WeightVar.apply(_chk(weights.contiguous(), F32, "weights"),
                                _chk(idx_start_end.contiguous(), I32, "idx_start_end"))

    @staticmethod
    def ScatterIdx(n_all_pts, idx_start_end, emb_idx):
        return scatter_idx(n_all_pts, _chk(idx_start_end, I32, "idx_start_end"), _chk(emb_idx, I32, "emb_idx"))

    TruncExp = _TruncExp
```

f2nerf_b200/renderer.py:

```python
import os
from dataclasses import dataclass
from typing import Optional

import torch

from . import _lib, ops
from ._lib import call, stream
from .field import field_backward, field_forward, field_forward_from_features
from .rng import burn_mlp_output, burn_rand
from .sampler import TRAIN, VALIDATE, LazySampleResult, SampleResultFlex

N_EDGE_PTS = 8192
MLP_RECOMPUTE = os.environ.get("F2B_MLP_RECOMPUTE", "1") == "1"


@dataclass
class RenderResult:
    colors: torch.Tensor
    first_oct_dis: torch.Tensor
    disparity: torch.Tensor
    edge_feats: Optional[torch.Tensor]
    depth: torch.Tensor
    weights: Optional[torch.Tensor]
    idx_start_end: Optional[torch.Tensor]


class ForwardRenderResult:
    edge_feats = None

    def __init__(self, colors, first_oct_dis, disparity, depth, kept_counts, w_slots, slot, owner, stamp, total_all):
        self.colors, self.first_oct_dis, self.disparity, self.depth = colors, first_oct_dis, disparity, depth
        self.kept_counts = kept_counts
        self._w_slots, self._slot, self._owner, self._stamp, self._packed = w_slots, slot, owner, stamp, None
        self._total_all = total_all

    def _pack(self):
        if self._packed is None:
            if self._owner._fwd_stamp.get(self._stamp[0]) != self._stamp[1]:
                raise RuntimeError("RenderResult.weights: a later Render re-used this result's slot-layout weights")
            n_rays, dev = self.kept_counts.shape[0], self.kept_counts.device
            bounds, total = ops.count_scan(self.kept_counts, n_rays)
            n_kept, n_all = torch.cat([total, self._total_all[:1]]).tolist()
            if n_all <= 0:
                self._packed = (None, None)
                return self._packed
            w = torch.empty((int(n_kept),), dtype=torch.float32, device=dev)
            if n_kept > 0:
                call("f2b_gather_kept_weights", self._w_slots, bounds, n_rays, int(self._slot), w, stream())
            self._packed = (w, bounds)
        return self._packed

    @property
    def weights(self):
        return self._pack()[0]

    @property
    def idx_start_end(self):
        return self._pack()[1]


class Renderer:
    def __init__(self, global_data_pool, pts_sampler, scene_field, shader, n_images, use_app_emb=False,
                 bg_color="rand_noise", device="cuda"):
        self.global_data_pool_ = global_data_pool
        self.pts_sampler_, self.scene_field_, self.shader_ = pts_sampler, scene_field, shader
        self.use_app_emb_ = bool(use_app_emb)
        self.app_emb_ = (torch.randn((n_images, 16), dtype=torch.float32, device=device) * .1).requires_grad_(True)
        if bg_color not in ("white", "black", "rand_noise"):
            bg_color = "rand_noise"
        self.bg_color_type_ = bg_color
        self.sample_result_ = None

    def _bg(self, n_rays, dev):
        gdp = self.global_data_pool_
        if self.bg_color_type_ == "white":
            return torch.ones((n_rays, 3), dtype=torch.float32, device=dev)
        if self.bg_color_type_ == "rand_noise":
            if gdp.mode_ == TRAIN:
                return torch.rand((n_rays, 3), dtype=torch.float32, device=dev)
            return torch.ones((n_rays, 3), dtype=torch.float32, device=dev) * .5
        return torch.zeros((n_rays, 3), dtype=torch.float32, device=dev)

    def Render(self, rays_o, rays_d, bounds, emb_idx=None):
        gdp = self.global_data_pool_
        field, shader, sampler = self.scene_field_, self.shader_, self.pts_sampler_
        n_rays, dev = rays_o.shape[0], rays_o.device
        train = gdp.mode_ == TRAIN
        if not train and self._fused_forward_ok(n_rays):
            return self.render_forward(rays_o, rays_d)
        if self._fused_launch_ok(n_rays):
            return self._render_fused_launches(rays_o, rays_d, emb_idx)
        pf = sampler.take_prefetched(rays_o, rays_d) if n_rays > 0 else None
        if pf is not None:
            slots = pf["slots"]
            gen = torch.cuda.default_generators[dev.index if dev.index is not None else torch.cuda.current_device()]
            gen.set_offset(gen.get_offset() + pf["noise_inc"])
            torch.cuda.current_stream(dev).wait_event(pf["done"])
        else:
            slots = sampler.begin_march(rays_o, rays_d)
        self.sample_result_ = LazySampleResult(slots)
        bg = self._bg(n_rays, dev)
        if n_rays <= 0:
            z = torch.zeros
            return RenderResult(bg, z((0, 1), device=dev), z((0,), device=dev), None, z((0,), device=dev), None, None)
        S = slots.slot
        with torch.no_grad():
            table16 = field.table_f16()
            fparams16 = field.mlp_.params_f16()
            logit_s = self._buf("logit", (n_rays * S,), torch.float32, dev)
            feat_s = self._buf("feat", (n_rays * S, 32), torch.float16, dev)
            weights0 = self._buf("w0", (n_rays * S,), torch.float32, dev)
            alphas0 = self._buf("a0", (n_rays * S,), torch.float32, dev)
            keep = self._buf("keep", (n_rays * S,), torch.uint8, dev)
            kept_counts = self._buf("kept", (n_rays,), torch.int32, dev)
            main = torch.cuda.current_stream(dev)
            chunks = self._ray_chunks(n_rays)
            lanes = [main] + [self._side_stream(dev, i) for i in range(1, len(chunks))]
            ready = torch.cuda.Event()
            ready.record(main)
            for (r0, r1), st in zip(chunks, lanes):
                if st is not main:
                    st.wait_event(ready)
                with torch.cuda.stream(st):
                    if pf is None:
                        sampler.march_rays(slots, r0, r1)
                    ops.field_fwd_slots(table16, field.prim_pool_, field.bias_pool_, field.n_volumes_, field.local_size_,
                                        fparams16, slots.s_pts[r0 * S:r1 * S], slots.s_anchors[r0 * S:r1 * S],
                                        slots.counts[r0:r1], r1 - r0, S, logit_s[r0 * S:r1 * S], feat_s[r0 * S:r1 * S])
                    ops.early_stop_rays(logit_s, 1, slots.s_dt, slots.slot_bounds[r0:r1], weights0, alphas0, keep,
                                        kept_counts[r0:r1])
            for st in lanes[1:]:
                main.wait_stream(st)
            new_bounds, total = ops.count_scan(kept_counts, n_rays)
            cut_rays = self._bwd_cut_rays(n_rays)
            head = [total] + ([new_bounds[cut_rays, 0]] if cut_rays is not None else [])
            n_head = 1 + (0 if cut_rays is None else cut_rays.numel())
            vals = torch.cat(head + [t.reshape(-1) for t in slots.totals]).tolist()
            n_kept = int(vals[0])
            n_all, n_all_oct = int(sum(vals[n_head::2])), int(sum(vals[n_head + 1::2]))
            rcut = [0] + ([] if cut_rays is None else self._cut_list) + [n_rays]
            scut = [0] + [int(v) for v in vals[1:n_head]] + [n_kept]
            self._bwd_cuts_ = [(rcut[i], rcut[i + 1], scut[i], scut[i + 1]) for i in range(len(rcut) - 1)]
            sampler.note_totals(n_rays, n_all_oct)
            slots.noted = True
            self.n_sampled_pts_, self.n_kept_pts_ = n_all, n_kept
            if train:
                gdp.sampled_pts_per_ray_ = gdp.sampled_pts_per_ray_ * .9 + (n_all / n_rays) * .1
            if n_all <= 0:
                if train:
                    gdp.meaningful_sampled_pts_per_ray_ *= .9
                z = torch.zeros
                return RenderResult(bg, z((n_rays, 1), device=dev), z((n_rays,), device=dev), None,
                                    torch.full((n_rays,), 512., device=dev), None, None)
            burn_mlp_output(n_all, dev)
            side = None
            if train:
                side = self._side_stream(dev, 1)
                side.wait_stream(main)
                with torch.cuda.stream(side):
                    sampler.update_oct_nodes_raw(slots.slot_bounds, slots.s_anchors, weights0, alphas0)
                gdp.meaningful_sampled_pts_per_ray_ = gdp.meaningful_sampled_pts_per_ray_ * .9 + (n_kept / n_rays) * .1
            n_edge = 2 * N_EDGE_PTS if train else 0
            feat_q = torch.empty((n_kept + n_edge, 32), dtype=torch.float16, device=dev)
            f32 = lambda *sh: torch.empty(sh, dtype=torch.float32, device=dev)
            pts, dirs, dt, t = f32(n_kept, 3), f32(n_kept, 3), f32(n_kept), f32(n_kept)
            anchors = torch.empty((n_kept, 3), dtype=torch.int32, device=dev)
            ops.compact_slots(keep, slots.slot_bounds, new_bounds, slots.rays_d, slots.s_pts, slots.s_dt, slots.s_t,
                              slots.s_anchors, feat_s, (pts, dirs, dt, t, anchors), feat_q)
            es = SampleResultFlex(pts, dirs, dt, t, anchors, new_bounds, slots.first_oct_dis.clone())
            if train:
                edge_pts, edge_anchors = sampler.GetEdgeSamples(N_EDGE_PTS)
                e_pts, e_anc = edge_pts.reshape(N_EDGE_PTS * 2, 3), edge_anchors.reshape(N_EDGE_PTS * 2)
                e_pts, e_anc = e_pts.contiguous(), e_anc.contiguous()
                feat_q[n_kept:] = ops.hash_fwd(table16, field.prim_pool_, field.bias_pool_, field.n_volumes_, field.local_size_,
                                               e_pts, e_anc, 1)
                segments = [(pts, anchors, 3, 0, n_kept), (e_pts, e_anc, 1, n_kept, n_edge)]
            else:
                segments = [(pts, anchors, 3, 0, n_kept)]
            burn_mlp_output(n_kept + n_edge, dev)
            burn_mlp_output(n_kept, dev)
            pt_emb_idx = ray_emb_idx = None
            if train and self.use_app_emb_:
                ray_emb_idx = emb_idx.to(torch.int32).contiguous()
                pt_emb_idx = ops.scatter_idx(n_kept, new_bounds, ray_emb_idx)

        grad_on = torch.is_grad_enabled() and train
        args = (self, es, segments, None, pt_emb_idx, ray_emb_idx, bg, feat_q, n_kept, grad_on)
        colors, disparity, depth, weights, edge_feats = _RenderFunction.apply(
            field.feat_pool_, field.mlp_.params_, shader.mlp_.params_, self.app_emb_, *args)
        if not train:
            edge_feats = None
        if side is not None:
            torch.cuda.current_stream(dev).wait_stream(side)
        return RenderResult(colors, es.first_oct_dis, disparity, edge_feats, depth, weights, new_bounds)

    def _fused_launch_ok(self, n_rays):
        if n_rays <= 0 or _lib.TRACE is not None or os.environ.get("F2B_FUSED_LAUNCH", "1") != "1":
            return False
        if _lib.lib.f2b_get_mlp_impl() != 1 or self.scene_field_.mlp_.n_hidden_matmuls != 0 or self.shader_.mlp_.n_hidden_matmuls != 1:
            return False
        return len(self._ray_chunks(n_rays)) == 1 and self._bwd_cut_rays(n_rays) is None

    def _render_fused_launches(self, rays_o, rays_d, emb_idx):
        gdp = self.global_data_pool_
        field, shader, sampler = self.scene_field_, self.shader_, self.pts_sampler_
        n_rays, dev = rays_o.shape[0], rays_o.device
        train = gdp.mode_ == TRAIN
        main = torch.cuda.current_stream(dev)
        grad_on = torch.is_grad_enabled() and train
        pf = sampler.take_prefetched(rays_o, rays_d)
        if pf is not None:
            slots = pf["slots"]
            gen = torch.cuda.default_generators[dev.index if dev.index is not None else torch.cuda.current_device()]
            gen.set_offset(gen.get_offset() + pf["noise_inc"])
            main.wait_event(pf["done"])
        else:
            slots = sampler.begin_march(rays_o, rays_d)
        self.sample_result_ = LazySampleResult(slots)
        bg = self._bg(n_rays, dev)
        S = slots.slot
        with torch.no_grad():
            table16 = field.table_f16()
            i32 = lambda *sh: torch.empty(sh, dtype=torch.int32, device=dev)
            f16 = lambda *sh: torch.empty(sh, dtype=torch.float16, device=dev)
            f32 = lambda *sh: torch.empty(sh, dtype=torch.float32, device=dev)
            fparams16, sparams16 = f16(field.mlp_.params_.numel()), f16(shader.mlp_.params_.numel())
            logit_s = self._buf("logit", (n_rays * S,), torch.float32, dev)
            feat_s = self._buf("feat", (n_rays * S, 32), torch.float16, dev)
            weights0 = self._buf("w0", (n_rays * S,), torch.float32, dev)
            alphas0 = self._buf("a0", (n_rays * S,), torch.float32, dev)
            keep = self._buf("keep", (n_rays * S,), torch.uint8, dev)
            kept_counts = self._buf("kept", (n_rays,), torch.int32, dev)
            new_bounds, heads = i32(n_rays, 2), i32(3)
            ra = _lib.RenderArgs()
            ra.set(tree_nodes=sampler.tree_nodes_gpu_, n_nodes=sampler.n_nodes, trans=sampler.pers_trans_gpu_,
                   n_trans=sampler.pers_trans_gpu_.numel() // 544, edge_pool=sampler.edge_pool_gpu_ if sampler.n_edges else None,
                   near_t=float(sampler.global_near_), far_t=1e8, sample_l=float(sampler.sample_l_),
                   scale_by_dis=int(sampler.scale_by_dis_), max_hits=int(sampler.max_oct_intersect_per_ray_),
                   count_all_hits=int(bool(sampler.exact_oct_stat_)),
                   table16=table16, prim=field.prim_pool_, bias=field.bias_pool_, n_volumes=int(field.n_volumes_),
                   local_size=int(field.local_size_), field_params=field.mlp_.params_.detach(), n_field_params=fparams16.numel(),
                   shader_params=shader.mlp_.params_.detach(), n_shader_params=sparams16.numel(), fparams16=fparams16,
                   sparams16=sparams16, n_rays=n_rays, rays_o=slots.rays_o, rays_d=slots.rays_d, noise=slots.noise, bg=bg,
                   skip_march=int(pf is not None), s_pts=slots.s_pts, s_dt=slots.s_dt, s_t=slots.s_t, s_anchors=slots.s_anchors,
                   counts=slots.counts, chunk_bounds=slots.chunk_bounds, slot_bounds=slots.slot_bounds,
                   first_oct_dis=slots.first_oct_dis, totals=heads[1:], logit_s=logit_s, feat_s=feat_s, w0=weights0, a0=alphas0,
                   keep=keep, kept_counts=kept_counts, new_bounds=new_bounds, total_kept=heads, stream=stream())
            if pf is not None:
                heads[1:].copy_(slots.totals[0])
            call("f2b_render_phase1", ra)
            if pf is not None:
                _lib.LAUNCHES -= 3
            n_pairs = N_EDGE_PTS if train else 0
            n_edge = 2 * n_pairs
            side = votes_done = None

            def launch_votes():
                nonlocal side, votes_done
                side = self._side_stream(dev, 1)
                side.wait_stream(main)
                with torch.cuda.stream(side):
                    sampler.update_oct_nodes_raw(slots.slot_bounds, slots.s_anchors, weights0, alphas0)
                votes_done = torch.cuda.Event()
                votes_done.record(side)

            def phase2_buffers(rows):
                T = dict(pts=f32(rows, 3), dirs=f32(rows, 3), dt=f32(rows), t=f32(rows), anchors=i32(rows, 3),
                         feat_q=f16(rows + n_edge, 32), logit=f32(rows), mlp_in=f16(rows, 32), raw=f16(rows, 16),
                         rgb=f32(rows, 3), edge32=f32(n_edge, 16), colors=f32(n_rays, 3), disparity=f32(n_rays), depth=f32(n_rays),
                         weights=f32(rows))
                if grad_on and not MLP_RECOMPUTE:
                    T.update(f_hidden=f16(1, rows + n_edge, 64), s_hidden=f16(2, rows, 64))
                if train:
                    if sampler.n_edges <= 0:
                        raise RuntimeError("GetEdgeSamples: empty edge pool (needs >= 2 face-adjacent valid leaves)")
                    T.update(edge_idx=torch.randint(0, sampler.n_edges, (n_pairs,), dtype=torch.int32, device=dev),
                             edge_coord=torch.rand((n_pairs, 2), dtype=torch.float32, device=dev) * 2. - 1.,
                             e_pts=f32(n_edge, 3), e_anc=i32(n_edge))
                if train and self.use_app_emb_:
                    T.update(ray_emb_idx=emb_idx.to(torch.int32).contiguous(), pt_emb_idx=i32(rows))
                return T

            pre_all = None
            if pf is not None and pf.get("host_totals") is not None:
                pf["done"].synchronize()
                pre_all = int(pf["host_totals"][0])
            T = None
            if pre_all is not None and pre_all > 0 and os.environ.get("F2B_PRESYNC_HOST", "1") == "1":
                burn_mlp_output(pre_all, dev)
                if train:
                    launch_votes()
                T = phase2_buffers(pre_all)
            n_kept, n_all, n_all_oct = heads.tolist()
            self._bwd_cuts_ = None
            sampler.note_totals(n_rays, n_all_oct)
            slots.noted = True
            slots.totals = [heads[1:]]
            self.n_sampled_pts_, self.n_kept_pts_ = n_all, n_kept
            if train:
                gdp.sampled_pts_per_ray_ = gdp.sampled_pts_per_ray_ * .9 + (n_all / n_rays) * .1
            if n_all <= 0:
                if train:
                    gdp.meaningful_sampled_pts_per_ray_ *= .9
                z = torch.zeros
                return RenderResult(bg, z((n_rays, 1), device=dev), z((n_rays,), device=dev), None,
                                    torch.full((n_rays,), 512., device=dev), None, None)
            if T is None:
                burn_mlp_output(n_all, dev)
                if train:
                    launch_votes()
                T = phase2_buffers(n_kept)
            elif pre_all != n_all:
                raise RuntimeError(f"Renderer.Render: prefetched march total {pre_all} != {n_all}")
            T["weights"] = T["weights"][:n_kept]
            if train:
                gdp.meaningful_sampled_pts_per_ray_ = gdp.meaningful_sampled_pts_per_ray_ * .9 + (n_kept / n_rays) * .1
            burn_mlp_output(n_kept + n_edge, dev)
            burn_mlp_output(n_kept, dev)
            if train and self.use_app_emb_:
                ra.set(app_emb=self.app_emb_.detach(), n_emb=self.app_emb_.shape[0])
            ra.set(n_kept=n_kept, n_edge_pairs=n_pairs, **T)
            keepalive = (slots, table16, fparams16, sparams16, new_bounds, heads, bg, T)
        colors, disparity, depth, weights, edge_feats = _FusedRenderFunction.apply(
            field.feat_pool_, field.mlp_.params_, shader.mlp_.params_, self.app_emb_, self, ra, keepalive, grad_on)
        if train and getattr(self, "next_rays_", None) is not None:
            pending = [n_kept * 3, n_kept] if (gdp.gradient_scaling_progress_ < 1. and n_kept > 0) else []
            nxt, self.next_rays_ = self.next_rays_, None
            sampler.prefetch_march(nxt[0], nxt[1], side, pending)
        if side is not None:
            main.wait_event(votes_done)
        return RenderResult(colors, slots.first_oct_dis.clone(), disparity, edge_feats if train else None, depth, weights, new_bounds)

    def _fused_forward_ok(self, n_rays):
        if n_rays <= 0 or _lib.TRACE is not None or os.environ.get("F2B_FUSED_FORWARD", "1") != "1":
            return False
        return (_lib.lib.f2b_get_mlp_impl() == 1 and self.scene_field_.mlp_.n_hidden_matmuls == 0
                and self.shader_.mlp_.n_hidden_matmuls == 1)

    def render_forward(self, rays_o, rays_d, out=None, lane=0):
        field, shader, sampler = self.scene_field_, self.shader_, self.pts_sampler_
        n_rays, dev = rays_o.shape[0], rays_o.device
        slots = sampler.begin_march(rays_o, rays_d, lane=lane)
        sampler.march_rays(slots, 0, n_rays)
        if lane == 0:
            self.sample_result_ = LazySampleResult(slots)
        bg = self._bg(n_rays, dev)
        S = slots.slot
        with torch.no_grad():
            table16 = field.table_f16()
            fparams16, sparams16 = field.mlp_.params_f16(), shader.mlp_.params_f16()
            f32 = lambda *sh: torch.empty(sh, dtype=torch.float32, device=dev)
            colors, disparity, depth = out if out is not None else (f32(n_rays, 3), f32(n_rays), f32(n_rays))
            kept = torch.empty((n_rays,), dtype=torch.int32, device=dev)
            ticket = torch.empty((1,), dtype=torch.int32, device=dev)
            w_slots = self._buf(f"w_fwd{lane}", (n_rays * S,), torch.float32, dev)
            stamps = self.__dict__.setdefault("_fwd_stamp", {})
            stamps[lane] = stamps.get(lane, 0) + 1
            call("f2b_render_fwd_fused", table16, field.prim_pool_, field.bias_pool_, int(field.n_volumes_), int(field.local_size_),
                 fparams16, sparams16, slots.s_pts, slots.s_dt, slots.s_t, slots.s_anchors, slots.counts, slots.rays_d, bg, n_rays, S,
                 slots.totals[0], ticket, colors, disparity, depth, kept, w_slots, stream())
        res = ForwardRenderResult(colors, slots.first_oct_dis, disparity, depth, kept, w_slots, S, self, (lane, stamps[lane]),
                                  slots.totals[0])
        res._keep = (slots, table16, fparams16, sparams16, bg, ticket)
        return res

    def set_next_rays(self, rays_o, rays_d):
        self.next_rays_ = (rays_o, rays_d)

    def prefetch_next(self, rays_o, rays_d):
        gdp = self.global_data_pool_
        dev = rays_o.device
        pf = getattr(self.pts_sampler_, "_prefetched", None)
        if pf is not None and pf["key"][:3] == (rays_o.data_ptr(), rays_d.data_ptr(), rays_o.shape[0]):
            return
        self.next_rays_ = None
        pending = ()
        if gdp.gradient_scaling_progress_ < 1. and getattr(self, "n_kept_pts_", 0) > 0:
            pending = (self.n_kept_pts_ * 3, self.n_kept_pts_)
        self.pts_sampler_.prefetch_march(rays_o, rays_d, self._side_stream(dev, 1), pending)

    def _table_grad_buffer(self, shape, dev):
        self._table_grad_tail_zero = False
        n = 1
        for d in shape:
            n *= int(d)
        st = getattr(self, "_d_table_storage_", None)
        try:
            if st is not None and st.nbytes() == 4 * n and st.device == torch.device(dev) and torch._C._storage_Use_Count(st._cdata) == 1:
                self._table_grad_tail_zero = True
                return torch.empty(0, dtype=torch.float32, device=dev).set_(st, 0, tuple(shape))
            buf = torch.zeros(tuple(shape), dtype=torch.float32, device=dev)
            self._d_table_storage_ = buf.untyped_storage()
            self._table_grad_tail_zero = True
            return buf
        except (AttributeError, RuntimeError):
            self._d_table_storage_ = None
            return torch.empty(tuple(shape), dtype=torch.float32, device=dev)

    def _side_stream(self, dev, i=1):
        pool = self.__dict__.setdefault("_streams_", {})
        key = (torch.device(dev).index, i)
        if key not in pool:
            pool[key] = torch.cuda.Stream(device=dev)
        return pool[key]

    def _buf(self, name, shape, dtype, dev):
        pool = self.__dict__.setdefault("_bufs_", {})
        n = 1
        for d in shape:
            n *= d
        t = pool.get(name)
        if t is None or t.numel() < n or t.dtype != dtype or t.device != torch.device(dev):
            t = pool[name] = torch.empty((max(n, 1),), dtype=dtype, device=dev)
        return t[:n].view(*shape)

    def _bwd_cut_rays(self, n_rays):
        if not hasattr(self, "bwd_chunks_"):
            self.bwd_chunks_ = int(os.environ.get("F2B_BWD_CHUNKS", "1"))
        k = max(1, min(int(self.bwd_chunks_), 16, (n_rays + 255) // 256))
        if k <= 1:
            self._cut_list = []
            return None
        key = (n_rays, k)
        if getattr(self, "_cut_key", None) != key:
            step = -(-n_rays // k)
            self._cut_list = [r for r in range(step, n_rays, step)]
            self._cut_dev = torch.tensor(self._cut_list, dtype=torch.int64, device=self.app_emb_.device) if self._cut_list else None
            self._cut_key = key
        return self._cut_dev

    def _ray_chunks(self, n_rays):
        if not hasattr(self, "ray_chunks_"):
            self.ray_chunks_ = int(os.environ.get("F2B_RAY_CHUNKS", "1"))
        k = max(1, min(int(self.ray_chunks_), 4, (n_rays + 255) // 256))
        step = -(-n_rays // k)
        return [(r0, min(r0 + step, n_rays)) for r0 in range(0, n_rays, step)]

    def States(self):
        out = []
        for p in (self.pts_sampler_, self.scene_field_, self.shader_):
            out += p.States()
        return out + [self.app_emb_.data]

    def LoadStates(self, states, idx=0):
        for p in (self.pts_sampler_, self.scene_field_, self.shader_):
            idx = p.LoadStates(states, idx)
        self.app_emb_.data.copy_(states[idx].to(self.app_emb_.device)); idx += 1
        return idx

    def OptimParamGroups(self):
        lr = self.global_data_pool_.learning_rate_
        groups = self.scene_field_.OptimParamGroups() + self.shader_.OptimParamGroups()
        return groups + [dict(params=[self.app_emb_], lr=lr, betas=(0.9, 0.99), eps=1e-15, weight_decay=1e-6)]

    def Reset(self):
        self.scene_field_.Reset()
        self.shader_.Reset()


class _FusedRenderFunction(torch.autograd.Function):

    @staticmethod
    def forward(ctx, feat_pool, field_params, shader_params, app_emb, renderer, ra, keepalive, grad_on):
        T = keepalive[-1]
        call("f2b_render_phase2_fwd", ra)
        if ra.n_edge_pairs == 0:
            _lib.LAUNCHES -= 3
        ctx.renderer, ctx.ra, ctx.keepalive, ctx.grad_on = renderer, ra, keepalive, grad_on
        ctx.gs_progress = renderer.global_data_pool_.gradient_scaling_progress_
        ctx.table_shape, ctx.emb_shape = feat_pool.shape, app_emb.shape
        return T["colors"], T["disparity"], T["depth"], T["weights"], T["edge32"].reshape(-1, 2, 16)

    @staticmethod
    def backward(ctx, d_colors, d_disp, d_depth, d_weights, d_edge):
        renderer, ra = ctx.renderer, ctx.ra
        if ctx.keepalive is None:
            raise RuntimeError("Renderer.Render backward: the saved activations were released by a previous backward "
                               "(like tiny-cuda-nn's context, TCNNWP.cpp:207, the graph can be traversed once)")
        if not ctx.grad_on:
            raise RuntimeError("Renderer.Render backward: forward ran without grad (VALIDATE mode / no_grad)")
        field, shader = renderer.scene_field_, renderer.shader_
        T = ctx.keepalive[-1]
        dev = T["colors"].device
        n_kept, n_edge, n_rays = ra.n_kept, 2 * ra.n_edge_pairs, ra.n_rays
        main = torch.cuda.current_stream(dev)
        c = lambda g: None if g is None else g.contiguous()
        d_colors = c(d_colors) if d_colors is not None else torch.zeros((n_rays, 3), dtype=torch.float32, device=dev)
        d_disp, d_depth, d_weights = c(d_disp), c(d_depth), c(d_weights)
        d_edge = None if d_edge is None else d_edge.reshape(-1, 16).contiguous()
        if ctx.gs_progress < 1.:
            burn_rand(n_kept * 3, dev)
            burn_rand(n_kept, dev)
        f16 = lambda *sh: torch.empty(sh, dtype=torch.float16, device=dev)
        f32 = lambda *sh: torch.empty(sh, dtype=torch.float32, device=dev)
        emb_on = "ray_emb_idx" in T
        slab_hook = getattr(renderer, "grad_slab_hook_", None)
        f_scale = field.mlp_.loss_scale_
        grad_mul = (1.0 / f_scale) * (getattr(renderer, "grad_premul_", 1.0) if slab_hook is not None else 1.0)
        B = dict(d_logit=f32(n_kept), d_raw=f16(n_kept, 16), d_in16=f16(n_kept, 32), d_scene16=f16(n_kept + n_edge, 16),
                 dfeat16=f16(n_kept + n_edge, 32), d_sparams=f32(ra.n_shader_params), d_fparams=f32(ra.n_field_params),
                 d_table=renderer._table_grad_buffer(ctx.table_shape, dev),
                 nonfinite=torch.empty((2,), dtype=torch.int32, device=dev))
        if emb_on:
            B["d_app"] = torch.empty(ctx.emb_shape, dtype=torch.float32, device=dev)
        side = renderer._side_stream(dev, 2)
        ra.set(d_colors=d_colors, d_disparity=d_disp, d_depth=d_depth, d_weights=d_weights, d_edge=d_edge,
               gs_progress=float(ctx.gs_progress), shader_loss_scale=float(shader.mlp_.loss_scale_), field_loss_scale=float(f_scale),
               table_grad_mul=float(grad_mul),
               table_numel=min(B["d_table"].numel(), 17 * int(field.local_size_)) if renderer._table_grad_tail_zero else B["d_table"].numel(),
               table_live=min(B["d_table"].numel(), 17 * int(field.local_size_)), scatter_mode=int(slab_hook is not None),
               stream=main.cuda_stream, side_stream=side.cuda_stream, **B)
        call("f2b_render_bwd", ra)
        if slab_hook is not None:
            hash_args = (field.prim_pool_, field.bias_pool_, int(field.n_volumes_), int(field.local_size_))
            jobs = [(T["pts"], T["anchors"], 3, 0, n_kept)] + ([(T["e_pts"], T["e_anc"], 1, n_kept, n_kept + n_edge)] if n_edge else [])
            ev = torch.cuda.Event()
            ev.record(main)
            side.wait_event(ev)
            with torch.cuda.stream(side):
                for lo, nl in slab_groups():
                    for pts_j, anc_j, stride_j, s0, s1 in jobs:
                        if s1 > s0:
                            call("f2b_hash_bwd_levels", *hash_args, pts_j, anc_j, int(stride_j), int(s1 - s0), B["dfeat16"][s0:s1], 1,
                                 float(grad_mul), B["d_table"], lo, nl, stream())
                    slab_hook(B["d_table"], lo, int(field.local_size_))
            main.wait_stream(side)
            renderer.grad_slab_finish_()
        call("f2b_render_grad_finalize", ra)
        bad = B["nonfinite"] != 0
        prev = getattr(renderer, "nonfinite_flag_", None)
        renderer.nonfinite_flag_ = bad if prev is None else (prev | bad)
        ctx.keepalive = None
        return B["d_table"], B["d_fparams"], B["d_sparams"], B.get("d_app"), None, None, None, None


class _RenderFunction(torch.autograd.Function):

    @staticmethod
    def forward(ctx, feat_pool, field_params, shader_params, app_emb, renderer, es, q_pts, q_anchors, pt_emb_idx,
                ray_emb_idx, bg, feat16, n_kept, grad_on):
        field, shader = renderer.scene_field_, renderer.shader_
        fparams16 = ops.cast_f32_to_f16(field_params)
        sparams16 = ops.cast_f32_to_f16(shader_params)
        dev = bg.device
        n_q = feat16.shape[0]
        emb = app_emb if pt_emb_idx is not None else None
        if _lib.lib.f2b_get_mlp_impl() == 1 and field.mlp_.n_hidden_matmuls == 0 and shader.mlp_.n_hidden_matmuls == 1:
            save = grad_on and not MLP_RECOMPUTE
            f_hidden = torch.empty((1, n_q, 64), dtype=torch.float16, device=dev) if save else None
            logit = torch.empty((n_kept,), dtype=torch.float32, device=dev)
            mlp_in = torch.empty((n_kept, 32), dtype=torch.float16, device=dev)
            call("f2b_field_shade_fwd", feat16, fparams16, es.dirs, emb, pt_emb_idx, n_kept, logit, mlp_in, f_hidden, stream())
            if n_q > n_kept:
                edge32 = torch.empty((n_q - n_kept, 16), dtype=torch.float32, device=dev)
                call("f2b_mlp_fwd_f32", feat16[n_kept:], fparams16, 0, n_q - n_kept, edge32, None,
                     f_hidden[0, n_kept:] if save else None, stream())
            else:
                edge32 = torch.empty((0, 16), dtype=torch.float32, device=dev)
            s_hidden = torch.empty((2, n_kept, 64), dtype=torch.float16, device=dev) if save else None
            raw = torch.empty((n_kept, 16), dtype=torch.float16, device=dev)
            rgb = torch.empty((n_kept, 3), dtype=torch.float32, device=dev)
            call("f2b_shader_mlp_rgb_fwd", mlp_in, sparams16, n_kept, raw, rgb, s_hidden, stream())
            logit_stride = 1
        else:
            scene_feat, f_hidden = field_forward_from_features(field, fparams16, feat16, save=grad_on)
            mlp_in = ops.shader_prep(scene_feat[:n_kept], es.dirs, emb, pt_emb_idx) if n_kept > 0 else \
                torch.empty((0, 32), dtype=torch.float16, device=bg.device)
            raw, s_hidden = ops.mlp_fwd(mlp_in, sparams16, shader.mlp_.n_hidden_matmuls, save_hidden=grad_on)
            rgb = ops.shader_act(raw)
            logit, logit_stride, edge32 = scene_feat, 16, scene_feat[n_kept:]
        colors, disparity, depth, weights = ops.composite_fwd(logit, logit_stride, rgb, es.dt, es.t, es.pts_idx_bounds, bg)
        scene_feat = (logit, logit_stride)
        edge_feats = edge32.reshape(-1, 2, 16)
        ctx.renderer, ctx.es, ctx.n_kept = renderer, es, n_kept
        ctx.cuts = renderer._bwd_cuts_ if getattr(renderer, "_bwd_cuts_", None) else [(0, es.pts_idx_bounds.shape[0], 0, n_kept)]
        ctx.pack = (fparams16, sparams16, q_pts, q_anchors, ray_emb_idx, bg, scene_feat, feat16, f_hidden, mlp_in, raw,
                    s_hidden, rgb)
        ctx.gs_progress = renderer.global_data_pool_.gradient_scaling_progress_
        ctx.grad_on = grad_on
        return colors, disparity, depth, weights, edge_feats

    @staticmethod
    def backward(ctx, d_colors, d_disp, d_depth, d_weights, d_edge):
        renderer, es, n_kept = ctx.renderer, ctx.es, ctx.n_kept
        field, shader, gdp = renderer.scene_field_, renderer.shader_, renderer.global_data_pool_
        if ctx.pack is None:
            raise RuntimeError("Renderer.Render backward: the saved activations were released by a previous backward "
                               "(like tiny-cuda-nn's context, TCNNWP.cpp:207, the graph can be traversed once)")
        (fparams16, sparams16, q_pts, q_anchors, ray_emb_idx, bg, scene_feat, feat16, f_hidden, mlp_in, raw, s_hidden,
         rgb) = ctx.pack
        if not ctx.grad_on:
            raise RuntimeError("Renderer.Render backward: forward ran without grad (VALIDATE mode / no_grad)")
        segments = q_pts
        n_q, dev = feat16.shape[0], feat16.device
        n_rays = es.pts_idx_bounds.shape[0]
        zeros = lambda *s: torch.zeros(s, dtype=torch.float32, device=dev)
        d_colors = d_colors.contiguous() if d_colors is not None else zeros(n_rays, 3)
        d_disp = d_disp.contiguous() if d_disp is not None else None
        d_depth = d_depth.contiguous() if d_depth is not None else None
        d_weights = d_weights.contiguous() if d_weights is not None else None
        if ctx.gs_progress < 1.:
            burn_rand(n_kept * 3, dev)
            burn_rand(n_kept, dev)
        s_scale, f_scale = shader.mlp_.loss_scale_, field.mlp_.loss_scale_
        nh_s, nh_f = shader.mlp_.n_hidden_matmuls, field.mlp_.n_hidden_matmuls
        f16 = lambda *sh: torch.empty(sh, dtype=torch.float16, device=dev)
        d_logit = torch.empty((n_kept,), dtype=torch.float32, device=dev)
        d_raw, d_in16, d_scene16, dfeat16 = f16(n_kept, 16), f16(n_kept, 32), f16(n_q, 16), f16(n_q, 32)
        d_sparams, d_fparams = zeros(sparams16.numel()), zeros(fparams16.numel())
        d_table = torch.zeros_like(field.feat_pool_)
        d_app = torch.zeros_like(renderer.app_emb_) if ray_emb_idx is not None else None
        if n_q > n_kept:
            if d_edge is not None:
                d_scene16[n_kept:] = (d_edge.reshape(-1, 16) * f_scale).to(torch.float16)
            else:
                d_scene16[n_kept:].zero_()
        main = torch.cuda.current_stream(dev)
        side = renderer._side_stream(dev, 2)
        bounds = es.pts_idx_bounds
        hash_args = (field.prim_pool_, field.bias_pool_, int(field.n_volumes_), int(field.local_size_))

        slab_hook = getattr(renderer, "grad_slab_hook_", None)
        grad_mul = (1.0 / f_scale) * (getattr(renderer, "grad_premul_", 1.0) if slab_hook is not None else 1.0)
        jobs = []

        def scatter(pts, anc, stride, s0, s1):
            if slab_hook is not None:
                jobs.append((pts, anc, stride, s0, s1))
                return
            ev = torch.cuda.Event()
            ev.record(main)
            side.wait_event(ev)
            with torch.cuda.stream(side):
                ops.hash_bwd(*hash_args, pts, anc, stride, dfeat16[s0:s1], grad_mul, d_table)

        for r0, r1, s0, s1 in ctx.cuts:
            if s1 <= s0:
                continue
            nr, ns = r1 - r0, s1 - s0
            call("f2b_composite_act_bwd", scene_feat[0], int(scene_feat[1]), rgb, es.dt, es.t, bounds[r0:r1], bg[r0:r1], nr,
                 d_colors[r0:r1], None if d_disp is None else d_disp[r0:r1], None if d_depth is None else d_depth[r0:r1],
                 d_weights, float(ctx.gs_progress), raw, float(s_scale), d_logit, 1, d_raw, stream())
            call("f2b_mlp_bwd2", d_raw[s0:s1], mlp_in[s0:s1], None if s_hidden is None else s_hidden[0, s0:s1],
                 s_hidden[1, s0:s1] if (nh_s and s_hidden is not None) else None, sparams16, int(nh_s), ns, d_in16[s0:s1], d_sparams,
                 stream())
            ops.shader_prep_bwd_f16(d_in16, d_logit, bounds[r0:r1], None if ray_emb_idx is None else ray_emb_idx[r0:r1],
                                    1.0 / s_scale, f_scale, d_scene16, d_app)
            call("f2b_mlp_bwd2", d_scene16[s0:s1], feat16[s0:s1], None if f_hidden is None else f_hidden[0, s0:s1],
                 f_hidden[1, s0:s1] if (nh_f and f_hidden is not None) else None, fparams16, int(nh_f), ns, dfeat16[s0:s1], d_fparams,
                 stream())
            scatter(segments[0][0][s0:s1], segments[0][1][s0:s1], segments[0][2], s0, s1)
        for pts_e, anc_e, stride_e, first, rows in segments[1:]:
            if rows > 0:
                call("f2b_mlp_bwd2", d_scene16[first:first + rows], feat16[first:first + rows],
                     None if f_hidden is None else f_hidden[0, first:first + rows],
                     f_hidden[1, first:first + rows] if (nh_f and f_hidden is not None) else None, fparams16, int(nh_f), rows,
                     dfeat16[first:first + rows], d_fparams, stream())
                scatter(pts_e, anc_e, stride_e, first, first + rows)
        if slab_hook is not None:
            ev = torch.cuda.Event()
            ev.record(main)
            side.wait_event(ev)
            with torch.cuda.stream(side):
                for lo, nl in slab_groups():
                    for pts_j, anc_j, stride_j, s0, s1 in jobs:
                        call("f2b_hash_bwd_levels", *hash_args, pts_j, anc_j, int(stride_j), int(s1 - s0), dfeat16[s0:s1], 1, float(grad_mul),
                             d_table, lo, nl, stream())
                    slab_hook(d_table, lo, int(field.local_size_))
        main.wait_stream(side)
        if slab_hook is not None:
            renderer.grad_slab_finish_()
        d_sparams = d_sparams / s_scale
        d_fparams = d_fparams / f_scale
        live = min(d_table.shape[0], (17 * int(field.local_size_)) // 2)
        ok_s = torch.isfinite(d_sparams).all()
        if d_app is not None:
            ok_s = ok_s & torch.isfinite(d_app).all()
        ok_f = torch.isfinite(d_fparams).all() & torch.isfinite(d_table[:live]).all()
        bad = torch.stack([~ok_s, ~ok_f])
        prev = getattr(renderer, "nonfinite_flag_", None)
        renderer.nonfinite_flag_ = bad if prev is None else (prev | bad)
        ctx.pack = None
        return d_table, d_fparams, d_sparams, d_app, None, None, None, None, None, None, None, None, None, None


def slab_groups():
    n = int(os.environ.get("F2B_DP_SLABS", "4"))
    return {4: ((12, 4), (8, 4), (4, 4), (0, 4)), 2: ((8, 8), (0, 8)), 1: ((0, 16),)}.get(n, ((12, 4), (8, 4), (4, 4), (0, 4)))


def check_backward_nan(renderer):
    flag = getattr(renderer, "nonfinite_flag_", None)
    renderer.nonfinite_flag_ = None
    if flag is None:
        return False
    hit = flag.reshape(-1).tolist()
    if len(hit) == 1:
        hit = [hit[0], hit[0]]
    for m, h in ((renderer.shader_.mlp_, hit[0]), (renderer.scene_field_.mlp_, hit[1])):
        if h:
            m.loss_scale_ = max(m.loss_scale_ / 2.0, 1.0)
    if any(hit):
        renderer.global_data_pool_.backward_nan_ = True
        return True
    return False
```

f2nerf_b200/shim/B200Renderer.cpp:

```cpp
#include <torch/torch.h>
#include <ATen/cuda/CUDAContext.h>
#include <ATen/cuda/CUDAGeneratorImpl.h>
#include <ATen/cuda/CUDAEvent.h>
#include <c10/cuda/CUDAStream.h>
#include <c10/cuda/CUDAGuard.h>
#include <chrono>
#include <cstdio>
#include <cstdlib>
#include <mutex>
#include <unordered_map>
#include "Common.h"
#include "Renderer/Renderer.h"
#include "PtsSampler/PersSampler.h"
#include "Field/Hash3DAnchored.h"
#include "Shader/SHShader.h"
#include "f2nerf_b200.h"
#include "B200Renderer.h"

using Tensor = torch::Tensor;
using torch::autograd::AutogradContext;
using torch::autograd::variable_list;

RenderResult f2b_reference_render(Renderer* r, const Tensor& rays_o, const Tensor& rays_d, const Tensor& bounds,
                                  const Tensor& emb_idx);

#define F2B_CHECK(expr)                                                            \
  do {                                                                             \
    int f2b_rc_ = (expr);                                                          \
    CHECK(f2b_rc_ == 0) << #expr << " -> " << f2b_rc_ << ": " << f2b_last_error(); \
  } while (0)

static bool g_keep_samples = [] { const char* e = std::getenv("F2B_KEEP_SAMPLES"); return e && e[0] == '1'; }();
static bool g_use_reference = [] { const char* e = std::getenv("F2B_RENDER"); return e && std::string(e) == "reference"; }();
void f2b_render_keep_samples(bool on) { g_keep_samples = on; }
void f2b_render_use_reference(bool on) { g_use_reference = on; }

namespace {

constexpr int kSlot = 1024;
constexpr int kEdgePts = 8192;
const auto kHalf = torch::TensorOptions().dtype(torch::kFloat16).device(torch::kCUDA);
const auto kByte = torch::TensorOptions().dtype(torch::kUInt8).device(torch::kCUDA);

void* cur_stream() { return (void*) at::cuda::getCurrentCUDAStream().stream(); }
void* P(const Tensor& t) { return t.defined() ? t.data_ptr() : nullptr; }
bool fused_forward() {
  static const bool on = [] { const char* e = getenv("F2B_FUSED_FORWARD"); return !e || atoi(e) != 0; }();
  return on;
}
bool validate_weights() {
  static const bool on = [] { const char* e = getenv("F2B_VALIDATE_WEIGHTS"); return !e || atoi(e) != 0; }();
  return on;
}
struct ShimProfile {
  bool on = false;
  double t_render_train = 0, t_render_val = 0, t_backward = 0;
  long n_train = 0, n_val = 0, n_bwd = 0;
  ShimProfile() { const char* e = getenv("F2B_SHIM_PROFILE"); on = e && atoi(e) != 0; }
  ~ShimProfile() {
    if (on)
      std::printf("{\"f2b_shim_profile\": {\"render_train_s\": %.3f, \"n_render_train\": %ld, \"render_validate_s\": %.3f, "
                  "\"n_render_validate\": %ld, \"backward_s\": %.3f, \"n_backward\": %ld}}\n",
                  t_render_train, n_train, t_render_val, n_val, t_backward, n_bwd);
  }
};
ShimProfile g_prof;
struct ScopedTimer {
  double* acc; long* cnt; std::chrono::steady_clock::time_point t0;
  ScopedTimer(double* a, long* c) : acc(g_prof.on ? a : nullptr), cnt(c), t0(std::chrono::steady_clock::now()) {}
  ~ScopedTimer() { if (acc) { *acc += std::chrono::duration<double>(std::chrono::steady_clock::now() - t0).count(); ++*cnt; } }
};

bool mlp_recompute() {
  static const bool on = [] { const char* e = getenv("F2B_MLP_RECOMPUTE"); return !e || atoi(e) != 0; }();
  return on;
}
float* PF(const Tensor& t) { return t.defined() ? t.data_ptr<float>() : nullptr; }
int* PI(const Tensor& t) { return t.defined() ? t.data_ptr<int>() : nullptr; }

void burn_rand(int64_t numel) {
  if (numel <= 0) return;
  const auto* prop = at::cuda::getCurrentDeviceProperties();
  const int64_t block = 256, unroll = 4;
  const int64_t max_grid = int64_t(prop->multiProcessorCount) * (prop->maxThreadsPerMultiProcessor / block);
  const int64_t grid = std::min(max_grid, (numel + block - 1) / block);
  const uint64_t inc = uint64_t(((numel - 1) / (block * grid * unroll) + 1) * 4);
  auto gen = at::cuda::detail::getDefaultCUDAGenerator();
  auto* impl = at::check_generator<at::CUDAGeneratorImpl>(gen);
  std::lock_guard<std::mutex> lock(impl->mutex_);
  impl->set_philox_offset_per_thread(impl->philox_offset_per_thread() + inc);
}
void burn_mlp_output(int64_t batch) { if (batch > 0) burn_rand(((batch + 127) / 128 * 128) * 16); }

struct Work {
  int64_t cap_rays = 0;
  Tensor s_pts, s_dt, s_t, s_anchors, logit_s, feat_s, w0, a0, keep, kept_counts, table16;
  c10::Storage d_table_storage;
  c10::optional<c10::cuda::CUDAStream> side_votes, side_scatter;
  void ensure(int64_t n_rays, int64_t table_numel) {
    if (n_rays > cap_rays) {
      const int64_t n = n_rays * kSlot;
      s_pts = torch::empty({n, 3}, CUDAFloat); s_dt = torch::empty({n}, CUDAFloat); s_t = torch::empty({n}, CUDAFloat);
      s_anchors = torch::empty({n, 2}, CUDAInt);
      logit_s = torch::empty({n}, CUDAFloat); feat_s = torch::empty({n, 32}, kHalf);
      w0 = torch::empty({n}, CUDAFloat); a0 = torch::empty({n}, CUDAFloat); keep = torch::empty({n}, kByte);
      kept_counts = torch::empty({n_rays}, CUDAInt);
      cap_rays = n_rays;
    }
    if (!table16.defined() || table16.numel() != table_numel) table16 = torch::empty({table_numel}, kHalf);
    if (!side_votes) { side_votes = c10::cuda::getStreamFromPool(); side_scatter = c10::cuda::getStreamFromPool(); }
  }
};
Work& work_of(const Renderer* r) {
  static std::unordered_map<const Renderer*, Work> pool;
  return pool[r];
}

void stream_wait(const c10::cuda::CUDAStream& waiter, const c10::cuda::CUDAStream& on) {
  at::cuda::CUDAEvent ev;
  ev.record(on);
  ev.block(waiter);
}

struct Pack {
  Renderer* renderer = nullptr;
  Hash3DAnchored* field = nullptr;
  SHShader* shader = nullptr;
  Tensor pts, dirs, dt, t, anchors, bounds, bg, feat16, e_pts, e_anc, pt_emb_idx, ray_emb_idx;
  int64_t n_kept = 0, n_edge = 0;
  bool grad_on = false;
  float gs_progress = 1.f;
  Tensor fparams16, sparams16, logit, mlp_in, raw, rgb, f_hidden, s_hidden;
};
std::mutex g_pack_mu;
std::unordered_map<int64_t, std::shared_ptr<Pack>> g_packs;
int64_t g_pack_next = 1;

class RenderFn : public torch::autograd::Function<RenderFn> {
public:
  static variable_list forward(AutogradContext* ctx, Tensor feat_pool, Tensor field_params, Tensor shader_params, Tensor app_emb,
                               int64_t pack_id) {
    std::shared_ptr<Pack> pk;
    { std::lock_guard<std::mutex> l(g_pack_mu); pk = g_packs.at(pack_id); }
    Pack& k = *pk;
    const int64_t n_kept = k.n_kept, n_q = k.feat16.size(0);
    k.fparams16 = torch::empty({field_params.numel()}, kHalf);
    k.sparams16 = torch::empty({shader_params.numel()}, kHalf);
    F2B_CHECK(f2b_cast_f32_to_f16(field_params.data_ptr<float>(), P(k.fparams16), field_params.numel(), 1.f, cur_stream()));
    F2B_CHECK(f2b_cast_f32_to_f16(shader_params.data_ptr<float>(), P(k.sparams16), shader_params.numel(), 1.f, cur_stream()));
    const bool emb_on = k.pt_emb_idx.defined();
    const bool save = k.grad_on && !mlp_recompute();
    if (save) k.f_hidden = torch::empty({1, n_q, 64}, kHalf);
    k.logit = torch::empty({n_kept}, CUDAFloat);
    k.mlp_in = torch::empty({n_kept, 32}, kHalf);
    F2B_CHECK(f2b_field_shade_fwd(P(k.feat16), P(k.fparams16), PF(k.dirs), emb_on ? app_emb.data_ptr<float>() : nullptr,
                                  emb_on ? PI(k.pt_emb_idx) : nullptr, (int) n_kept, PF(k.logit), P(k.mlp_in),
                                  P(k.f_hidden), cur_stream()));
    Tensor edge32 = torch::empty({n_q - n_kept, 16}, CUDAFloat);
    if (n_q > n_kept) {
      F2B_CHECK(f2b_mlp_fwd_f32((char*) P(k.feat16) + n_kept * 64, P(k.fparams16), 0, (int) (n_q - n_kept), PF(edge32), nullptr,
                                save ? (void*) ((char*) P(k.f_hidden) + n_kept * 128) : nullptr, cur_stream()));
    }
    if (save) k.s_hidden = torch::empty({2, n_kept, 64}, kHalf);
    k.raw = torch::empty({n_kept, 16}, kHalf);
    k.rgb = torch::empty({n_kept, 3}, CUDAFloat);
    F2B_CHECK(f2b_shader_mlp_rgb_fwd(P(k.mlp_in), P(k.sparams16), (int) n_kept, P(k.raw), PF(k.rgb),
                                     P(k.s_hidden), cur_stream()));
    const int n_rays = k.bounds.size(0);
    Tensor colors = torch::empty({n_rays, 3}, CUDAFloat), disp = torch::empty({n_rays}, CUDAFloat),
           depth = torch::empty({n_rays}, CUDAFloat), weights = torch::empty({n_kept}, CUDAFloat);
    F2B_CHECK(f2b_composite_fwd(PF(k.logit), 1, PF(k.rgb), PF(k.dt), PF(k.t), PI(k.bounds), PF(k.bg), n_rays, PF(colors),
                                PF(disp), PF(depth), PF(weights), cur_stream()));
    ctx->saved_data["pack"] = pack_id;
    ctx->saved_data["table_numel"] = feat_pool.numel();
    ctx->saved_data["n_emb"] = app_emb.size(0);
    return {colors, disp, depth, weights, edge32.reshape({-1, 2, 16})};
  }

  static variable_list backward(AutogradContext* ctx, variable_list g) {
    ScopedTimer prof_timer(&g_prof.t_backward, &g_prof.n_bwd);
    const int64_t pack_id = ctx->saved_data["pack"].toInt();
    std::shared_ptr<Pack> pk;
    {
      std::lock_guard<std::mutex> l(g_pack_mu);
      auto it = g_packs.find(pack_id);
      CHECK(it != g_packs.end()) << "Renderer::Render backward: the saved activations were released by a previous backward";
      pk = it->second;
      g_packs.erase(it);
    }
    Pack& k = *pk;
    CHECK(k.grad_on) << "Renderer::Render backward: forward ran without grad (VALIDATE mode / NoGradGuard)";
    const int64_t n_kept = k.n_kept, n_q = k.feat16.size(0);
    const int n_rays = k.bounds.size(0);
    Hash3DAnchored* field = k.field;
    SHShader* shader = k.shader;
    Tensor d_colors = g[0].defined() ? g[0].contiguous() : torch::zeros({n_rays, 3}, CUDAFloat);
    Tensor d_disp = g[1].defined() ? g[1].contiguous() : Tensor();
    Tensor d_depth = g[2].defined() ? g[2].contiguous() : Tensor();
    Tensor d_weights = g[3].defined() ? g[3].contiguous() : Tensor();
    Tensor d_edge = g[4];
    if (k.gs_progress < 1.f) { burn_rand(n_kept * 3); burn_rand(n_kept); }
    const float s_scale = shader->mlp_->loss_scale_, f_scale = field->mlp_->loss_scale_;
    Tensor d_logit = torch::empty({n_kept}, CUDAFloat);
    Tensor d_raw = torch::empty({n_kept, 16}, kHalf), d_in16 = torch::empty({n_kept, 32}, kHalf);
    Tensor d_scene16 = torch::empty({n_q, 16}, kHalf), dfeat16 = torch::empty({n_q, 32}, kHalf);
    Tensor d_sparams = torch::zeros({k.sparams16.numel()}, CUDAFloat), d_fparams = torch::zeros({k.fparams16.numel()}, CUDAFloat);
    const int64_t table_numel = ctx->saved_data["table_numel"].toInt();
    const int local_size = ((field->pool_size_ / N_LEVELS) >> 4) << 4;
    const int64_t live = std::min<int64_t>(table_numel, int64_t(N_LEVELS + 1) * local_size);
    Work& wk = work_of(k.renderer);
    Tensor d_table;
    if (wk.d_table_storage && wk.d_table_storage.nbytes() == size_t(table_numel) * 4 && wk.d_table_storage.use_count() == 1) {
      d_table = torch::empty({0}, CUDAFloat).set_(wk.d_table_storage, 0, {table_numel / 2, 2});
      d_table.view({-1}).slice(0, 0, live).zero_();
    } else {
      d_table = torch::zeros({table_numel / 2, 2}, CUDAFloat);
      wk.d_table_storage = d_table.storage();
    }
    const bool emb_on = k.ray_emb_idx.defined();
    Tensor d_app = emb_on ? torch::zeros({ctx->saved_data["n_emb"].toInt(), 16}, CUDAFloat) : Tensor();
    if (n_q > n_kept) {
      if (d_edge.defined()) d_scene16.slice(0, n_kept, n_q).copy_((d_edge.reshape({-1, 16}) * f_scale).to(torch::kFloat16));
      else d_scene16.slice(0, n_kept, n_q).zero_();
    }
    F2B_CHECK(f2b_composite_act_bwd(PF(k.logit), 1, PF(k.rgb), PF(k.dt), PF(k.t), PI(k.bounds), PF(k.bg), n_rays, PF(d_colors),
                                    PF(d_disp), PF(d_depth), PF(d_weights), k.gs_progress, P(k.raw), s_scale, PF(d_logit), 1,
                                    P(d_raw), cur_stream()));
    F2B_CHECK(f2b_mlp_bwd2(P(d_raw), P(k.mlp_in), P(k.s_hidden),
                           k.s_hidden.defined() ? (void*) ((char*) P(k.s_hidden) + n_kept * 128) : nullptr, P(k.sparams16), 1,
                           (int) n_kept, P(d_in16), PF(d_sparams), cur_stream()));
    F2B_CHECK(f2b_shader_prep_bwd_f16(P(d_in16), PF(d_logit), PI(k.bounds), emb_on ? PI(k.ray_emb_idx) : nullptr, n_rays,
                                      1.f / s_scale, f_scale, P(d_scene16), PF(d_app), cur_stream()));
    F2B_CHECK(f2b_mlp_bwd2(P(d_scene16), P(k.feat16), P(k.f_hidden), nullptr, P(k.fparams16), 0, (int) n_q, P(dfeat16),
                           PF(d_fparams), cur_stream()));
    F2B_CHECK(f2b_hash_bwd(field->prim_pool_.data_ptr<int>(), field->bias_pool_.data_ptr<float>(), field->n_volumes_, local_size,
                           PF(k.pts), PI(k.anchors), 3, (int) n_kept, P(dfeat16), 1, 1.f / f_scale, PF(d_table), cur_stream()));
    if (n_q > n_kept) {
      F2B_CHECK(f2b_hash_bwd(field->prim_pool_.data_ptr<int>(), field->bias_pool_.data_ptr<float>(), field->n_volumes_, local_size,
                             PF(k.e_pts), PI(k.e_anc), 1, (int) (n_q - n_kept), (char*) P(dfeat16) + n_kept * 64, 1, 1.f / f_scale,
                             PF(d_table), cur_stream()));
    }
    d_sparams = d_sparams / s_scale;
    d_fparams = d_fparams / f_scale;
    Tensor ok_s = torch::isfinite(d_sparams).all();
    if (emb_on) ok_s = ok_s & torch::isfinite(d_app).all();
    Tensor ok_f = torch::isfinite(d_fparams).all() & torch::isfinite(d_table.view({-1}).slice(0, 0, live)).all();
    Tensor flags = torch::stack({ok_s, ok_f}).to(torch::kCPU);
    if (!flags[0].item<bool>()) { shader->global_data_pool_->backward_nan_ = true; shader->mlp_->loss_scale_ = std::max(s_scale / 2.f, 1.f); }
    if (!flags[1].item<bool>()) { field->global_data_pool_->backward_nan_ = true; field->mlp_->loss_scale_ = std::max(f_scale / 2.f, 1.f); }
    return {d_table, d_fparams, d_sparams, emb_on ? d_app : Tensor(), Tensor()};
  }
};

}

RenderResult Renderer::Render(const Tensor& rays_o_raw, const Tensor& rays_d_raw, const Tensor& bounds_raw, const Tensor& emb_idx) {
  if (g_use_reference) return f2b_reference_render(this, rays_o_raw, rays_d_raw, bounds_raw, emb_idx);
  const bool prof_train = global_data_pool_->mode_ == RunningMode::TRAIN;
  ScopedTimer prof_timer(prof_train ? &g_prof.t_render_train : &g_prof.t_render_val, prof_train ? &g_prof.n_train : &g_prof.n_val);
  auto* sampler = dynamic_cast<PersSampler*>(pts_sampler_.get());
  auto* field = dynamic_cast<Hash3DAnchored*>(scene_field_.get());
  auto* shader = dynamic_cast<SHShader*>(shader_.get());
  CHECK(sampler && field && shader) << "B200 Renderer::Render: needs PersSampler + Hash3DAnchored + SHShader";
  CHECK(field->n_hidden_layers_ == 1 && shader->n_hiddens_ == 2) << "B200 Renderer::Render: MLP shapes 32->64->16 / 32->64->64->16 only";
  GlobalDataPool* gdp = global_data_pool_;
  const bool train = gdp->mode_ == RunningMode::TRAIN;
  const int n_rays = rays_o_raw.size(0);
  auto& oct = *sampler->pers_octree_;
  auto main = at::cuda::getCurrentCUDAStream();
  const bool caller_grad = torch::GradMode::is_enabled();
  torch::NoGradGuard no_grad;

  Tensor rays_o = rays_o_raw.contiguous();
  Tensor rays_d = (rays_d_raw / torch::linalg_norm(rays_d_raw, 2, -1, true)).contiguous();
  Tensor noise;
  if (gdp->mode_ == RunningMode::VALIDATE) noise = torch::ones({kSlot + n_rays + 10}, CUDAFloat);
  else noise = ((torch::rand({kSlot + n_rays + 10}, CUDAFloat) - .5f) + 1.f).contiguous();
  noise.mul_(gdp->ray_march_fineness_);
  Tensor bg;
  if (bg_color_type_ == BGColorType::white) bg = torch::ones({n_rays, 3}, CUDAFloat);
  else if (bg_color_type_ == BGColorType::rand_noise) bg = train ? torch::rand({n_rays, 3}, CUDAFloat) : torch::ones({n_rays, 3}, CUDAFloat) * .5f;
  else bg = torch::zeros({n_rays, 3}, CUDAFloat);
  if (n_rays <= 0) return {bg, torch::zeros({0, 1}, CUDAFloat), torch::zeros({0}, CUDAFloat), Tensor(), torch::zeros({0}, CUDAFloat), Tensor(), Tensor()};

  Work& w = work_of(this);
  w.ensure(n_rays, field->feat_pool_.numel());
  const int local_size = ((field->pool_size_ / N_LEVELS) >> 4) << 4;
  const int64_t live = std::min<int64_t>(field->feat_pool_.numel(), int64_t(N_LEVELS + 1) * local_size);
  F2B_CHECK(f2b_table_to_half(field->feat_pool_.data_ptr<float>(), P(w.table16), live, cur_stream()));
  Tensor fparams16 = torch::empty({field->mlp_->params_.numel()}, kHalf);
  F2B_CHECK(f2b_cast_f32_to_f16(field->mlp_->params_.data_ptr<float>(), P(fparams16), fparams16.numel(), 1.f, cur_stream()));
  Tensor counts = torch::empty({n_rays}, CUDAInt), chunk_bounds = torch::empty({n_rays, 2}, CUDAInt);
  Tensor slot_bounds = torch::empty({n_rays, 2}, CUDAInt), first_oct_dis = torch::empty({n_rays, 1}, CUDAFloat);
  Tensor heads = torch::empty({3}, CUDAInt);
  const int n_nodes = oct.tree_nodes_gpu_.numel() / 64, n_trans = oct.pers_trans_gpu_.numel() / 544;
  F2B_CHECK(f2b_sampler_march(P(oct.tree_nodes_gpu_), n_nodes, P(oct.pers_trans_gpu_), n_trans, PF(rays_o), PF(rays_d), PF(noise), n_rays,
                              sampler->global_near_, 1e8f, sampler->sample_l_, sampler->scale_by_dis_ ? 1 : 0,
                              sampler->max_oct_intersect_per_ray_, 0, PF(w.s_pts), PF(w.s_dt), PF(w.s_t), PI(w.s_anchors),
                              PI(counts), PI(chunk_bounds), PI(heads) + 1, PF(first_oct_dis), cur_stream()));
  F2B_CHECK(f2b_slot_bounds(PI(counts), n_rays, kSlot, 0, PI(slot_bounds), cur_stream()));
  if (!train && fused_forward()) {
    Tensor sparams16 = torch::empty({shader->mlp_->params_.numel()}, kHalf);
    F2B_CHECK(f2b_cast_f32_to_f16(shader->mlp_->params_.data_ptr<float>(), P(sparams16), sparams16.numel(), 1.f, cur_stream()));
    Tensor colors = torch::empty({n_rays, 3}, CUDAFloat), disp = torch::empty({n_rays}, CUDAFloat), depth = torch::empty({n_rays}, CUDAFloat);
    Tensor kept = torch::empty({n_rays}, CUDAInt), ticket = torch::empty({1}, CUDAInt);
    F2B_CHECK(f2b_render_fwd_fused(P(w.table16), field->prim_pool_.data_ptr<int>(), field->bias_pool_.data_ptr<float>(), field->n_volumes_,
                                   local_size, P(fparams16), P(sparams16), PF(w.s_pts), PF(w.s_dt), PF(w.s_t), PI(w.s_anchors), PI(counts),
                                   PF(rays_d), PF(bg), n_rays, kSlot, PI(heads) + 1, PI(ticket), PF(colors), PF(disp), PF(depth), PI(kept),
                                   PF(w.w0), cur_stream()));
    sample_result_ = SampleResultFlex();
    sample_result_.first_oct_dis = first_oct_dis;
    if (!validate_weights()) return {colors, first_oct_dis, disp, Tensor(), depth, Tensor(), Tensor()};
    Tensor new_bounds = torch::empty({n_rays, 2}, CUDAInt);
    F2B_CHECK(f2b_count_scan(PI(kept), n_rays, PI(new_bounds), PI(heads), cur_stream()));
    Tensor heads_cpu = heads.to(torch::kCPU);
    const int64_t n_kept = heads_cpu[0].item<int>(), n_all = heads_cpu[1].item<int>();
    sample_result_.pts = torch::empty({n_all, 0}, CUDAFloat);
    if (n_all > 0) { burn_mlp_output(n_all); burn_mlp_output(n_kept); burn_mlp_output(n_kept); }
    Tensor weights = torch::empty({n_kept}, CUDAFloat);
    if (n_kept > 0) F2B_CHECK(f2b_gather_kept_weights(PF(w.w0), PI(new_bounds), n_rays, kSlot, PF(weights), cur_stream()));
    if (n_all <= 0) return {bg, torch::zeros({n_rays, 1}, CUDAFloat), torch::zeros({n_rays}, CUDAFloat), Tensor(), torch::full({n_rays}, 512.f, CUDAFloat), Tensor(), Tensor()};
    return {colors, first_oct_dis, disp, Tensor(), depth, weights, new_bounds};
  }
  F2B_CHECK(f2b_field_fwd_slots(P(w.table16), field->prim_pool_.data_ptr<int>(), field->bias_pool_.data_ptr<float>(), field->n_volumes_,
                                local_size, P(fparams16), PF(w.s_pts), PI(w.s_anchors), 2, PI(counts), n_rays, kSlot, 1, PF(w.logit_s),
                                P(w.feat_s), cur_stream()));
  F2B_CHECK(f2b_early_stop_rays(PF(w.logit_s), 1, PF(w.s_dt), PI(slot_bounds), n_rays, PF(w.w0), PF(w.a0), w.keep.data_ptr<uint8_t>(),
                                PI(w.kept_counts), cur_stream()));
  Tensor new_bounds = torch::empty({n_rays, 2}, CUDAInt);
  F2B_CHECK(f2b_count_scan(PI(w.kept_counts), n_rays, PI(new_bounds), PI(heads), cur_stream()));
  Tensor heads_cpu = heads.to(torch::kCPU);
  const int64_t n_kept = heads_cpu[0].item<int>(), n_all = heads_cpu[1].item<int>(), n_all_oct = heads_cpu[2].item<int>();
  if (gdp->mode_ != RunningMode::VALIDATE)
    gdp->sampled_oct_per_ray_ = gdp->sampled_oct_per_ray_ * .9f + (float(n_all_oct) / float(n_rays)) * .1f;
  if (train) gdp->sampled_pts_per_ray_ = gdp->sampled_pts_per_ray_ * .9f + (float(n_all) / float(n_rays)) * .1f;
  if (n_all <= 0) {
    if (train) gdp->meaningful_sampled_pts_per_ray_ *= .9f;
    return {bg, torch::zeros({n_rays, 1}, CUDAFloat), torch::zeros({n_rays}, CUDAFloat), Tensor(), torch::full({n_rays}, 512.f, CUDAFloat), Tensor(), Tensor()};
  }
  burn_mlp_output(n_all);

  if (g_keep_samples) {
    Tensor b = torch::empty({n_rays, 2}, CUDAInt), tot = torch::zeros({1}, CUDAInt);
    F2B_CHECK(f2b_count_scan(PI(counts), n_rays, PI(b), PI(tot), cur_stream()));
    SampleResultFlex s;
    s.pts = torch::empty({n_all, 3}, CUDAFloat); s.dirs = torch::empty({n_all, 3}, CUDAFloat); s.dt = torch::empty({n_all}, CUDAFloat);
    s.t = torch::empty({n_all}, CUDAFloat); s.anchors = torch::empty({n_all, 3}, CUDAInt); s.pts_idx_bounds = b; s.first_oct_dis = first_oct_dis;
    F2B_CHECK(f2b_sampler_gather(PF(rays_d), PI(b), n_rays, PF(w.s_pts), PF(w.s_dt), PF(w.s_t), PI(w.s_anchors), PF(s.pts), PF(s.dirs),
                                 PF(s.dt), PF(s.t), PI(s.anchors), cur_stream()));
    sample_result_ = s;
  } else {
    sample_result_ = SampleResultFlex();
    sample_result_.pts = torch::empty({n_all, 0}, CUDAFloat);
    sample_result_.first_oct_dis = first_oct_dis;
  }

  bool votes_on_side = false;
  if (train) {
    bool maintenance = gdp->iter_step_ % sampler->compact_freq_ == 0 ||
                       (!sampler->sub_div_milestones_.empty() && sampler->sub_div_milestones_.back() <= gdp->iter_step_);
    Tensor vote_w = torch::full({n_nodes}, -1, CUDAInt), vote_a = torch::full({n_nodes}, -1, CUDAInt), mark = torch::zeros({n_nodes}, CUDAInt);
    auto launch = [&](void* st) {
      F2B_CHECK(f2b_oct_mark_visit(PI(slot_bounds), n_rays, PI(w.s_anchors) + 1, 2, PF(w.w0), PF(w.a0), PI(vote_w), PI(vote_a), PI(mark),
                                   PI(oct.tree_visit_cnt_), st));
      F2B_CHECK(f2b_oct_update_stats(PI(vote_w), PI(vote_a), PI(mark), PI(oct.tree_weight_stats_), PI(oct.tree_alpha_stats_),
                                     P(oct.tree_nodes_gpu_), n_nodes, st));
    };
    if (maintenance) {
      launch(cur_stream());
      while (!sampler->sub_div_milestones_.empty() && sampler->sub_div_milestones_.back() <= gdp->iter_step_) {
        oct.ProcOctree(true, true, sampler->sub_div_milestones_.back() <= 0);
        oct.MarkInvisibleNodes();
        oct.ProcOctree(true, false, false);
        sampler->sub_div_milestones_.pop_back();
      }
      if (gdp->iter_step_ % sampler->compact_freq_ == 0) oct.ProcOctree(true, false, false);
    } else {
      stream_wait(*w.side_votes, main);
      {
        c10::cuda::CUDAStreamGuard g(*w.side_votes);
        vote_w.record_stream(*w.side_votes); vote_a.record_stream(*w.side_votes); mark.record_stream(*w.side_votes);
        launch((void*) w.side_votes->stream());
      }
      votes_on_side = true;
    }
    gdp->meaningful_sampled_pts_per_ray_ = gdp->meaningful_sampled_pts_per_ray_ * .9f + (float(n_kept) / float(n_rays)) * .1f;
  }

  auto pk = std::make_shared<Pack>();
  Pack& k = *pk;
  k.renderer = this; k.field = field; k.shader = shader;
  const int64_t n_edge = train ? 2 * kEdgePts : 0;
  k.n_kept = n_kept; k.n_edge = n_edge;
  k.feat16 = torch::empty({n_kept + n_edge, 32}, kHalf);
  k.pts = torch::empty({n_kept, 3}, CUDAFloat); k.dirs = torch::empty({n_kept, 3}, CUDAFloat);
  k.dt = torch::empty({n_kept}, CUDAFloat); k.t = torch::empty({n_kept}, CUDAFloat); k.anchors = torch::empty({n_kept, 3}, CUDAInt);
  k.bounds = new_bounds; k.bg = bg;
  F2B_CHECK(f2b_compact_slots(w.keep.data_ptr<uint8_t>(), PI(slot_bounds), PI(new_bounds), n_rays, PF(rays_d), PF(w.s_pts), PF(w.s_dt),
                              PF(w.s_t), PI(w.s_anchors), P(w.feat_s), PF(k.pts), PF(k.dirs), PF(k.dt), PF(k.t), PI(k.anchors), P(k.feat16),
                              cur_stream()));
  if (train) {
    const int n_edges = oct.edge_pool_.size();
    Tensor edge_idx = torch::randint(0, n_edges, {kEdgePts}, CUDAInt).contiguous();
    Tensor edge_coord = (torch::rand({kEdgePts, 2}, CUDAFloat) * 2.f - 1.f).contiguous();
    k.e_pts = torch::empty({kEdgePts * 2, 3}, CUDAFloat); k.e_anc = torch::empty({kEdgePts * 2}, CUDAInt);
    F2B_CHECK(f2b_edge_samples(P(oct.edge_pool_gpu_), P(oct.pers_trans_gpu_), PI(edge_idx), PF(edge_coord), kEdgePts, PF(k.e_pts), PI(k.e_anc),
                               cur_stream()));
    F2B_CHECK(f2b_hash_fwd(P(w.table16), field->prim_pool_.data_ptr<int>(), field->bias_pool_.data_ptr<float>(), field->n_volumes_, local_size,
                           PF(k.e_pts), PI(k.e_anc), 1, (int) n_edge, (char*) P(k.feat16) + n_kept * 64, cur_stream()));
  }
  burn_mlp_output(n_kept + n_edge);
  burn_mlp_output(n_kept);
  if (train && use_app_emb_) {
    k.ray_emb_idx = emb_idx.to(torch::kInt32).contiguous();
    k.pt_emb_idx = torch::empty({n_kept}, CUDAInt);
    F2B_CHECK(f2b_scatter_idx(PI(new_bounds), PI(k.ray_emb_idx), n_rays, PI(k.pt_emb_idx), cur_stream()));
  }
  k.gs_progress = gdp->gradient_scaling_progress_;
  k.grad_on = caller_grad && train;
  int64_t id;
  {
    std::lock_guard<std::mutex> l(g_pack_mu);
    id = g_pack_next++;
    g_packs[id] = pk;
    for (auto it = g_packs.begin(); it != g_packs.end();)
      it = (it->first + 4 < id) ? g_packs.erase(it) : std::next(it);
  }
  variable_list out;
  {
    torch::AutoGradMode grad_mode(k.grad_on);
    out = RenderFn::apply(field->feat_pool_, field->mlp_->params_, shader->mlp_->params_, app_emb_, id);
  }
  if (!k.grad_on) { std::lock_guard<std::mutex> l(g_pack_mu); g_packs.erase(id); }
  if (votes_on_side) stream_wait(main, *w.side_votes);
  return {out[0], first_oct_dis, out[1], train ? out[4] : Tensor(), out[2], out[3], new_bounds};
}
```

include/f2nerf_b200.h:

```cpp
#ifndef F2NERF_B200_H
#define F2NERF_B200_H
#include <stdint.h>
#ifdef __cplusplus
extern "C" {
#endif

#define F2B_OK            0
#define F2B_EINVAL      (-1)
#define F2B_ECUDA       (-2)
#define F2B_EUNSUPPORTED (-3)

#define F2B_N_LEVELS    16
#define F2B_N_CHANNELS   2
#define F2B_N_PROS      12
#define F2B_MAX_SAMPLE_PER_RAY 1024
#define F2B_MLP_WIDTH   64
#define F2B_MLP_IN      32
#define F2B_MLP_OUT_PAD 16

const char* f2b_last_error(void);
int  f2b_abi_version(void);
int  f2b_device_info(int* sm_count, int* l2_bytes);

int f2b_sampler_count(const void* tree_nodes, int n_nodes, const void* trans, int n_trans,
                      const float* rays_o, const float* rays_d, const float* rays_noise, int n_rays,
                      float near, float far, float sample_l, int scale_by_dis,
                      int max_oct_intersect_per_ray, int count_all_hits,
                      int* ray_counts ,
                      int* pts_idx_bounds , int* totals ,
                      void* stream);
int f2b_sampler_fill(const void* tree_nodes, int n_nodes, const void* trans, int n_trans,
                     const float* rays_o, const float* rays_d, const float* rays_noise, int n_rays,
                     float near, float far, float sample_l, int scale_by_dis,
                     int max_oct_intersect_per_ray, const int* pts_idx_bounds,
                     float* pts , float* dirs , float* dt ,
                     float* t , int* anchors , float* first_oct_dis ,
                     void* stream);
int f2b_sampler_march(const void* tree_nodes, int n_nodes, const void* trans, int n_trans,
                      const float* rays_o, const float* rays_d, const float* rays_noise, int n_rays,
                      float near, float far, float sample_l, int scale_by_dis,
                      int max_oct_intersect_per_ray, int count_all_hits,
                      float* s_pts, float* s_dt, float* s_t, int* s_anchors,
                      int* ray_counts , int* pts_idx_bounds , int* totals ,
                      float* first_oct_dis , void* stream);
int f2b_sampler_march_bg(const void* tree_nodes, int n_nodes, const void* trans, int n_trans,
                      const float* rays_o, const float* rays_d, const float* rays_noise, int n_rays,
                      float near, float far, float sample_l, int scale_by_dis,
                      int max_oct_intersect_per_ray, int count_all_hits,
                      float* s_pts, float* s_dt, float* s_t, int* s_anchors,
                      int* ray_counts , int* pts_idx_bounds , int* totals ,
                      float* first_oct_dis , void* stream);
int f2b_sampler_gather(const float* rays_d, const int* pts_idx_bounds, int n_rays,
                       const float* s_pts, const float* s_dt, const float* s_t, const int* s_anchors,
                       float* pts, float* dirs, float* dt, float* t, int* anchors, void* stream);
int f2b_edge_samples(const void* edge_pool, const void* trans, const int* edge_idx,
                     const float* edge_coord , int n_pts,
                     float* out_pts , int* out_idx , void* stream);
int f2b_oct_mark_visit(const int* pts_idx_bounds, int n_rays, const int* oct_idx, int oct_stride,
                       const float* weights, const float* alphas,
                       int* vote_weight, int* vote_alpha, int* visit_mark, int* visit_cnt,
                       void* stream);
int f2b_oct_update_stats(const int* vote_weight, const int* vote_alpha, const int* visit_mark,
                         int* weight_stats, int* alpha_stats, void* tree_nodes, int n_nodes,
                         void* stream);

int f2b_hash_level_scales(float* scales16_host);
int f2b_table_to_half(const float* table_f32, void* table_f16, int64_t n, void* stream);
int f2b_hash_fwd(const void* table_f16, const int* prim_pool, const float* bias_pool,
                 int n_volumes, int local_size,
                 const float* pts, const int* vol, int vol_stride, int n_pts,
                 void* out_f16, void* stream);
int f2b_hash_fwd_levels(const void* table_f16, const int* prim_pool, const float* bias_pool,
                        int n_volumes, int local_size, const float* pts, const int* vol,
                        int vol_stride, int n_pts, int level_lo, int n_levels, void* out_f16, void* stream);
int f2b_hash_bwd(const int* prim_pool, const float* bias_pool, int n_volumes, int local_size,
                 const float* pts, const int* vol, int vol_stride, int n_pts,
                 const void* grad_feat, int grad_is_f16, float grad_mul,
                 float* grad_table, void* stream);
int f2b_hash_bwd_levels(const int* prim_pool, const float* bias_pool, int n_volumes, int local_size,
                        const float* pts, const int* vol, int vol_stride, int n_pts,
                        const void* grad_feat, int grad_is_f16, float grad_mul, float* grad_table,
                        int level_lo, int n_levels, void* stream);

int f2b_mlp_fwd(const void* in_f16, const void* params_f16, int n_hidden_matmuls, int n_pts,
                void* out_f16, void* hidden_save_f16, void* stream);
int f2b_mlp_fwd_f32(const void* in_f16, const void* params_f16, int n_hidden_matmuls, int n_pts,
                    float* out_f32, void* out_f16, void* hidden_save_f16, void* stream);
int f2b_mlp_bwd(const void* dout_f16, const void* in_f16, const void* hidden_save_f16,
                const void* params_f16, int n_hidden_matmuls, int n_pts,
                void* din_f16, float* dparams_f32, void* stream);
int f2b_cast_f32_to_f16(const float* src, void* dst, int64_t n, float scale, void* stream);
int f2b_cast_f16_to_f32(const void* src, float* dst, int64_t n, float scale, void* stream);

int f2b_field_fwd(const void* table_f16, const int* prim_pool, const float* bias_pool, int n_volumes,
                  int local_size, const void* mlp_params_f16, const float* pts, const int* vol, int vol_stride,
                  int n_pts, int logit_only, float* out_f32, void* feat_save_f16, void* hidden_save_f16,
                  void* stream);

int f2b_field_fwd_slots(const void* table_f16, const int* prim_pool, const float* bias_pool, int n_volumes,
                        int local_size, const void* mlp_params_f16, const float* slot_pts, const int* slot_vol,
                        int vol_stride, const int* ray_counts, int n_rays, int slot_size, int logit_only,
                        float* out_f32, void* feat_save_f16, void* stream);

int f2b_field_shade_fwd(const void* feat_f16 , const void* field_params_f16, const float* dirs ,
                        const float* app_emb , const int* pt_emb_idx , int n_pts,
                        float* logit , void* mlp_in_f16 , void* hidden_save_f16 ,
                        void* stream);
int f2b_shader_mlp_rgb_fwd(const void* mlp_in_f16, const void* shader_params_f16, int n_pts, void* raw_f16, float* rgb,
                           void* hidden_save_f16 , void* stream);
int f2b_mlp_bwd2(const void* dout_f16, const void* in_f16, const void* hidden0_f16, const void* hidden1_f16,
                 const void* params_f16, int n_hidden_matmuls, int n_pts, void* din_f16, float* dparams_f32, void* stream);

int f2b_set_mlp_impl(int impl);
int f2b_get_mlp_impl(void);
int f2b_mlp_fwd_v0(const void* in_f16, const void* params_f16, int n_hidden_matmuls, int n_pts,
                   void* out_f16, void* hidden_save_f16, void* stream);
int f2b_mlp_bwd_v0(const void* dout_f16, const void* in_f16, const void* hidden_save_f16,
                   const void* params_f16, int n_hidden_matmuls, int n_pts,
                   void* din_f16, float* dparams_f32, void* stream);
int f2b_mlp_fwd_tc(const void* in_f16, const void* params_f16, int n_hidden_matmuls, int n_pts,
                   void* out_f16, void* hidden_save_f16, void* stream);
int f2b_mlp_bwd_tc(const void* dout_f16, const void* in_f16, const void* hidden_save_f16,
                   const void* params_f16, int n_hidden_matmuls, int n_pts,
                   void* din_f16, float* dparams_f32, void* stream);

int f2b_sh_encode(const float* dirs, int n_pts, int degree , float* out, void* stream);
int f2b_scatter_idx(const int* pts_idx_bounds, const int* emb_idx, int n_rays, int* out, void* stream);
int f2b_shader_prep(const float* scene_feat , const float* dirs ,
                    const float* app_emb , const int* pt_emb_idx ,
                    int n_pts, void* mlp_in_f16 , void* stream);
int f2b_shader_act(const void* raw_out_f16 , int n_pts, float* rgb , void* stream);
int f2b_shader_act_bwd(const void* raw_out_f16, const float* d_rgb, int n_pts, float loss_scale,
                       void* d_raw_f16, void* stream);
int f2b_shader_prep_bwd(const void* d_mlp_in_f16 , const int* pts_idx_bounds ,
                        const int* emb_idx , int n_rays, float inv_loss_scale,
                        float* d_scene_feat , float* d_app_emb , void* stream);
int f2b_shader_prep_bwd_f16(const void* d_mlp_in_f16 , const float* d_logit ,
                            const int* pts_idx_bounds, const int* emb_idx, int n_rays, float inv_loss_scale,
                            float field_loss_scale, void* d_field_out_f16 , float* d_app_emb, void* stream);

int f2b_octree_proc(const void* tree_nodes, const int* weight_stats, const int* alpha_stats, const int* visit_cnt,
                    int n_nodes, int subdivide, int brute_force, void* work_nodes, int* work_i32, void* nodes_out,
                    int* weight_stats_out, int* alpha_stats_out, int* n_nodes_out, void* stream);
int f2b_octree_mark_invisible(void* tree_nodes, int n_nodes, const float* intri, const float* w2c, const float* bounds,
                              int n_cams, void* stream);

int f2b_img2world_rays(const float* poses, const float* intri, const float* dist_params, const int* cam_indices,
                       const int* ij, int n_rays, float* rays_o , float* rays_d ,
                       void* stream);
int f2b_gather_pixels(const float* images, const int* cam_indices, const int* ij, int height, int width, int n,
                      float* out , void* stream);

int f2b_adam_step(float* param, const float* grad, float* exp_avg, float* exp_avg_sq, int64_t n, int64_t n_live,
                  double lr, double beta1, double beta2, double eps, double weight_decay, int64_t step,
                  void* shadow_f16 , void* stream);

int f2b_early_stop(const float* logit, int logit_stride, const float* dt, const int* pts_idx_bounds,
                   int n_rays, float* weights, float* alphas, uint8_t* keep,
                   int* ray_counts ,
                   int* new_bounds , int* total_kept , void* stream);
int f2b_early_stop_rays(const float* logit, int logit_stride, const float* dt, const int* pts_idx_bounds,
                        int n_rays, float* weights, float* alphas, uint8_t* keep, int* ray_counts, void* stream);
int f2b_count_scan(const int* counts, int n, int* bounds, int* total, void* stream);
int f2b_slot_bounds(const int* ray_counts, int n_rays, int slot_size, int first_ray, int* slot_bounds, void* stream);
int f2b_compact_slots(const uint8_t* keep, const int* slot_bounds, const int* new_bounds, int n_rays,
                      const float* rays_d, const float* s_pts, const float* s_dt, const float* s_t,
                      const int* s_anchors, const void* feat_slots_f16 , float* pts_o, float* dirs_o,
                      float* dt_o, float* t_o, int* anchors_o, void* feat_o_f16 , void* stream);
int f2b_compact_samples(const uint8_t* keep, const int* old_bounds, const int* new_bounds, int n_rays,
                        const float* pts, const float* dirs, const float* dt, const float* t,
                        const int* anchors, const void* feat_f16 ,
                        float* pts_o, float* dirs_o, float* dt_o, float* t_o, int* anchors_o,
                        void* feat_o_f16 , void* stream);
int f2b_composite_fwd(const float* logit, int logit_stride, const float* rgb, const float* dt,
                      const float* t, const int* pts_idx_bounds, const float* bg_color, int n_rays,
                      float* colors, float* disparity, float* depth, float* weights, void* stream);
int f2b_composite_bwd(const float* logit, int logit_stride, const float* rgb, const float* dt,
                      const float* t, const int* pts_idx_bounds, const float* bg_color, int n_rays,
                      const float* d_colors, const float* d_disparity, const float* d_depth,
                      const float* d_weights, float grad_scaling_progress,
                      float* d_logit, int dlogit_stride, float* d_rgb, void* stream);
int f2b_composite_act_bwd(const float* logit, int logit_stride, const float* rgb, const float* dt, const float* t,
                          const int* pts_idx_bounds, const float* bg_color, int n_rays, const float* d_colors,
                          const float* d_disparity, const float* d_depth, const float* d_weights,
                          float grad_scaling_progress, const void* raw_f16 , float loss_scale,
                          float* d_logit, int dlogit_stride, void* d_raw_f16 , void* stream);
int f2b_flex_sum(const float* val, int vec, const int* idx_start_end, int n_outs, float* sum, void* stream);
int f2b_flex_accumulate_sum(const float* val, const int* idx_start_end, int n_outs, int include_this,
                            float* out, void* stream);
int f2b_weight_var_fwd(const float* weights, const int* idx_start_end, int n_outs, float* out_vars, void* stream);
int f2b_weight_var_bwd(const float* weights, const int* idx_start_end, int n_outs, const float* dl_dvars,
                       float* dl_dw, void* stream);

typedef struct f2b_render {
  const void* tree_nodes; int n_nodes; const void* trans; int n_trans; const void* edge_pool;
  float near_t, far_t, sample_l; int scale_by_dis, max_hits, count_all_hits;
  const void* table16; const int* prim; const float* bias; int n_volumes, local_size;
  const float* field_params; int n_field_params; const float* shader_params; int n_shader_params;
  void* fparams16; void* sparams16;
  const float* app_emb; int n_emb;
  int n_rays; const float* rays_o; const float* rays_d ; const float* noise; const float* bg;
  const int* ray_emb_idx;
  int skip_march;
  float* s_pts; float* s_dt; float* s_t; int* s_anchors; int* counts; int* chunk_bounds; int* slot_bounds;
  float* first_oct_dis; int* totals ;
  float* logit_s; void* feat_s; float* w0; float* a0; uint8_t* keep; int* kept_counts; int* new_bounds; int* total_kept;
  int n_kept; int n_edge_pairs;
  float* pts; float* dirs; float* dt; float* t; int* anchors; void* feat_q;
  const int* edge_idx; const float* edge_coord; float* e_pts; int* e_anc;
  int* pt_emb_idx;
  float* logit; void* mlp_in; void* f_hidden ; float* edge32; void* raw; float* rgb; void* s_hidden ;
  float* colors; float* disparity; float* depth; float* weights;
  const float* d_colors; const float* d_disparity; const float* d_depth; const float* d_weights; const float* d_edge ;
  float gs_progress, shader_loss_scale, field_loss_scale, table_grad_mul;
  float* d_logit; void* d_raw; void* d_in16; void* d_scene16; void* dfeat16;
  float* d_sparams; float* d_fparams; float* d_table; int64_t table_numel; int64_t table_live; float* d_app;
  int scatter_mode;
  int* nonfinite;
  void* stream; void* side_stream;
} f2b_render;
int f2b_render_sizeof(void);
int f2b_render_phase1(const f2b_render* r);
int f2b_render_phase2_fwd(const f2b_render* r);
int f2b_render_bwd(const f2b_render* r);
int f2b_render_grad_finalize(const f2b_render* r);

int f2b_render_fwd_fused(const void* table_f16, const int* prim_pool, const float* bias_pool, int n_volumes, int local_size,
                         const void* field_params_f16, const void* shader_params_f16, const float* slot_pts, const float* slot_dt,
                         const float* slot_t, const int* slot_anchors, const int* ray_counts, const float* rays_d, const float* bg,
                         int n_rays, int slot_size, const int* total_all, int* ticket, float* colors, float* disparity,
                         float* depth, int* kept_counts, float* weights_slots, void* stream);
int f2b_gather_kept_weights(const float* weights_slots, const int* new_bounds, int n_rays, int slot_size, float* weights,
                            void* stream);

#ifdef __cplusplus
}
#endif
#endif
```

Before: 943,900.

## Fuse field MLP backward with hash-grid gradient scatter in a warp-specialized kernel

Adds a field_bwd_scatter kernel. Four tensor-core warps run the field MLP backward per tile and write the input gradients into a shared-memory ring, guarded by mbarriers. Extra scatter warps read that ring and do the hash-table atomic scatter for the kept and edge samples. This replaces the separate mlp_bwd2 and hash_bwd launches and the global dfeat16 round trip, which were meant to cost launch time and memory traffic. It adds a complex producer/consumer pipeline and periodic atomic flushes of the weight gradient. It applies only for a single-cut, no-hidden-layer, TC-impl path and is on by default through an environment flag.

```diff
diff --git a/f2nerf_b200/_lib.py b/f2nerf_b200/_lib.py
--- a/f2nerf_b200/_lib.py
+++ b/f2nerf_b200/_lib.py
@@ -51,6 +51,7 @@
     "f2b_field_shade_fwd": [_P, _P, _P, _P, _P, c_int, _P, _P, _P, _P],
     "f2b_shader_mlp_rgb_fwd": [_P, _P, c_int, _P, _P, _P, _P],
     "f2b_mlp_bwd2": [_P, _P, _P, _P, _P, c_int, c_int, _P, _P, _P],
+    "f2b_field_bwd_scatter": [_P, _P, _P, c_int, _P, _P, c_int, _P, _P, _P, _P, c_int, c_int, c_float, _P, _P, _P],
     "f2b_mlp_fwd_v0": [_P, _P, c_int, c_int, _P, _P, _P],
     "f2b_mlp_bwd_v0": [_P, _P, _P, _P, c_int, c_int, _P, _P, _P],
     "f2b_mlp_fwd_tc": [_P, _P, c_int, c_int, _P, _P, _P],
@@ -162,7 +163,10 @@
     return torch.cuda.current_stream().cuda_stream
 
 
-KERNELS_PER_CALL = {"f2b_render_sizeof": 0, "f2b_render_phase1": 7, "f2b_render_phase2_fwd": 10, "f2b_render_bwd": 8, "f2b_render_grad_finalize": 2,
+FIELD_BWD_SCATTER = os.environ.get("F2B_FIELD_BWD_SCATTER", "1") != "0"
+
+KERNELS_PER_CALL = {"f2b_render_sizeof": 0, "f2b_render_phase1": 7, "f2b_render_phase2_fwd": 10,
+                    "f2b_render_bwd": 5 if FIELD_BWD_SCATTER else 8, "f2b_render_grad_finalize": 2, "f2b_field_bwd_scatter": 1,
                     "f2b_sampler_count": 2, "f2b_sampler_march": 2, "f2b_sampler_march_bg": 2, "f2b_early_stop": 2, "f2b_hash_level_scales": 1, "f2b_device_info": 0,
                     "f2b_abi_version": 0, "f2b_set_mlp_impl": 0, "f2b_get_mlp_impl": 0}
 LAUNCHES = 0
diff --git a/f2nerf_b200/csrc/hash.cu b/f2nerf_b200/csrc/hash.cu
--- a/f2nerf_b200/csrc/hash.cu
+++ b/f2nerf_b200/csrc/hash.cu
@@ -45,8 +45,6 @@
   }
 }
 
-constexpr int kDirectHeads = 24;
-
 template <bool GRAD_F16>
 __device__ __forceinline__ void hash_bwd_task(int64_t group, int l, int lane, const int* __restrict__ prim_pool,
                                               const float* __restrict__ bias_pool, int n_volumes, int local_size,
@@ -65,57 +63,14 @@
     }
   }
   const bool live = valid && !(g0 == 0.f && g1 == 0.f);
-  if (!__any_sync(0xffffffffu, live)) return;
-  g0 *= grad_mul; g1 *= grad_mul;
-  Corner8 c;
+  float x0 = 0.f, x1 = 0.f, x2 = 0.f;
   int v = -1;
   if (live) {
     const float p0 = __ldg(pts + i * 3), p1 = __ldg(pts + i * 3 + 1), p2 = __ldg(pts + i * 3 + 2);
-    const float x0 = fmul(fadd(p0, 1.f), .5f), x1 = fmul(fadd(p1, 1.f), .5f), x2 = fmul(fadd(p2, 1.f), .5f);
+    x0 = fmul(fadd(p0, 1.f), .5f); x1 = fmul(fadd(p1, 1.f), .5f); x2 = fmul(fadd(p2, 1.f), .5f);
     v = __ldg(vol + i * vol_stride);
-    const int tv = l * n_volumes + v;
-    corners(x0, x1, x2, level_scale(l), prim_pool + tv * 3, bias_pool + tv * 3, (unsigned)local_size, c);
-  } else {
-#pragma unroll
-    for (int k = 0; k < 8; k++) { c.idx[k] = 0; c.w[k] = 0.f; }
-    c.cell[0] = c.cell[1] = c.cell[2] = 0;
   }
-  const unsigned pcx = __shfl_up_sync(0xffffffffu, c.cell[0], 1), pcy = __shfl_up_sync(0xffffffffu, c.cell[1], 1),
-                 pcz = __shfl_up_sync(0xffffffffu, c.cell[2], 1);
-  const int prev_v = __shfl_up_sync(0xffffffffu, v, 1);
-  const bool head = (lane == 0) || !live || c.cell[0] != pcx || c.cell[1] != pcy || c.cell[2] != pcz || v != prev_v;
-  const unsigned heads = __ballot_sync(0xffffffffu, head);
-  float* base = grad_table + size_t(l) * local_size;
-  if (__popc(heads) > kDirectHeads) {
-    if (live) {
-#pragma unroll
-      for (int k = 0; k < 8; k++)
-        atomicAdd(reinterpret_cast<float2*>(base + size_t(c.idx[k]) * 2), make_float2(c.w[k] * g0, c.w[k] * g1));
-    }
-    return;
-  }
-  const unsigned below = heads & ((2u << lane) - 1u);
-  const int run_start = 31 - __clz(below);
-  float s[16];
-#pragma unroll
-  for (int k = 0; k < 8; k++) { s[2 * k] = c.w[k] * g0; s[2 * k + 1] = c.w[k] * g1; }
-  const int max_run = __reduce_max_sync(0xffffffffu, lane - run_start + 1);
-#pragma unroll
-  for (int o = 1; o < 32; o <<= 1) {
-    if (o >= max_run) break;
-    const bool take = (lane - o) >= run_start;
-#pragma unroll
-    for (int k = 0; k < 16; k++) {
-      const float u = __shfl_up_sync(0xffffffffu, s[k], o);
-      if (take) s[k] += u;
-    }
-  }
-  const bool tail = (lane == 31) || ((heads >> (lane + 1)) & 1u);
-  if (live && tail) {
-#pragma unroll
-    for (int k = 0; k < 8; k++)
-      atomicAdd(reinterpret_cast<float2*>(base + size_t(c.idx[k]) * 2), make_float2(s[2 * k], s[2 * k + 1]));
-  }
+  hash_bwd_level(l, lane, valid, x0, x1, x2, v, g0, g1, prim_pool, bias_pool, n_volumes, local_size, grad_mul, grad_table);
 }
 
 template <bool GRAD_F16>
diff --git a/f2nerf_b200/csrc/hash.cuh b/f2nerf_b200/csrc/hash.cuh
--- a/f2nerf_b200/csrc/hash.cuh
+++ b/f2nerf_b200/csrc/hash.cuh
@@ -82,4 +82,60 @@
   }
 }
 
+constexpr int kDirectHeads = 24;
+
+__device__ __forceinline__ void hash_bwd_level(int l, int lane, bool valid, float x0, float x1, float x2, int v, float g0, float g1,
+                                               const int* __restrict__ prim_pool, const float* __restrict__ bias_pool, int n_volumes,
+                                               int local_size, float grad_mul, float* __restrict__ grad_table) {
+  const bool live = valid && !(g0 == 0.f && g1 == 0.f);
+  if (!__any_sync(0xffffffffu, live)) return;
+  g0 *= grad_mul; g1 *= grad_mul;
+  Corner8 c;
+  if (live) {
+    const int tv = l * n_volumes + v;
+    corners(x0, x1, x2, level_scale(l), prim_pool + tv * 3, bias_pool + tv * 3, (unsigned)local_size, c);
+  } else {
+#pragma unroll
+    for (int k = 0; k < 8; k++) { c.idx[k] = 0; c.w[k] = 0.f; }
+    c.cell[0] = c.cell[1] = c.cell[2] = 0;
+    v = -1;
+  }
+  const unsigned pcx = __shfl_up_sync(0xffffffffu, c.cell[0], 1), pcy = __shfl_up_sync(0xffffffffu, c.cell[1], 1),
+                 pcz = __shfl_up_sync(0xffffffffu, c.cell[2], 1);
+  const int prev_v = __shfl_up_sync(0xffffffffu, v, 1);
+  const bool head = (lane == 0) || !live || c.cell[0] != pcx || c.cell[1] != pcy || c.cell[2] != pcz || v != prev_v;
+  const unsigned heads = __ballot_sync(0xffffffffu, head);
+  float* base = grad_table + size_t(l) * local_size;
+  if (__popc(heads) > kDirectHeads) {
+    if (live) {
+#pragma unroll
+      for (int k = 0; k < 8; k++)
+        atomicAdd(reinterpret_cast<float2*>(base + size_t(c.idx[k]) * 2), make_float2(c.w[k] * g0, c.w[k] * g1));
+    }
+    return;
+  }
+  const unsigned below = heads & ((2u << lane) - 1u);
+  const int run_start = 31 - __clz(below);
+  float s[16];
+#pragma unroll
+  for (int k = 0; k < 8; k++) { s[2 * k] = c.w[k] * g0; s[2 * k + 1] = c.w[k] * g1; }
+  const int max_run = __reduce_max_sync(0xffffffffu, lane - run_start + 1);
+#pragma unroll
+  for (int o = 1; o < 32; o <<= 1) {
+    if (o >= max_run) break;
+    const bool take = (lane - o) >= run_start;
+#pragma unroll
+    for (int k = 0; k < 16; k++) {
+      const float u = __shfl_up_sync(0xffffffffu, s[k], o);
+      if (take) s[k] += u;
+    }
+  }
+  const bool tail = (lane == 31) || ((heads >> (lane + 1)) & 1u);
+  if (live && tail) {
+#pragma unroll
+    for (int k = 0; k < 8; k++)
+      atomicAdd(reinterpret_cast<float2*>(base + size_t(c.idx[k]) * 2), make_float2(s[2 * k], s[2 * k + 1]));
+  }
 }
+
+}
diff --git a/f2nerf_b200/csrc/mlp_tc_bwd.cu b/f2nerf_b200/csrc/mlp_tc_bwd.cu
--- a/f2nerf_b200/csrc/mlp_tc_bwd.cu
+++ b/f2nerf_b200/csrc/mlp_tc_bwd.cu
@@ -1,5 +1,7 @@
 #include "common.cuh"
 #include "tc.cuh"
+#include "hash.cuh"
+#include <stdlib.h>
 
 namespace f2b {
 using namespace tc;
@@ -274,13 +276,10 @@
 };
 
 template <int NH>
-__device__ __forceinline__ void prefetch_tile_rc(const __half* __restrict__ dout, const __half* __restrict__ in, int tile, int n_pts,
-                                                 uint32_t stage) {
+__device__ __forceinline__ void prefetch_tile_rc(const __half* __restrict__ dout, const __half* __restrict__ in, int rows, uint32_t stage) {
   using S = RcSmem<NH>;
-  const int rows = min(kBT, n_pts - tile * kBT);
-  const size_t t0 = size_t(tile) * kBT;
-  const unsigned char* s_do = reinterpret_cast<const unsigned char*>(dout + t0 * 16);
-  const unsigned char* s_x = reinterpret_cast<const unsigned char*>(in + t0 * 32);
+  const unsigned char* s_do = reinterpret_cast<const unsigned char*>(dout);
+  const unsigned char* s_x = reinterpret_cast<const unsigned char*>(in);
 #pragma unroll
   for (int j = 0; j < 2; j++) {
     const int c = threadIdx.x + kBT * j, r = c >> 1;
@@ -348,7 +347,7 @@
   const uint32_t stage0 = smem_u32(sm + S::STAGE0);
 
   int tile = blockIdx.x;
-  if (tile < n_tiles) prefetch_tile_rc<NH>(dout, in, tile, n_pts, stage0);
+  if (tile < n_tiles) prefetch_tile_rc<NH>(dout + size_t(tile) * kBT * 16, in + size_t(tile) * kBT * 32, min(kBT, n_pts - tile * kBT), stage0);
   asm volatile("cp.async.commit_group;" ::: "memory");
   stage_w<32>(params, 64, sm + S::W0);
   if (NH) stage_w<64>(params + 64 * 32, 64, sm + S::WH);
@@ -374,7 +373,9 @@
     const int p = tile * kBT + tid;
     const bool valid = p < n_pts;
     const int next = tile + gridDim.x;
-    if (next < n_tiles) prefetch_tile_rc<NH>(dout, in, next, n_pts, stage0 + (buf ^ 1) * S::STAGE_BYTES);
+    if (next < n_tiles)
+      prefetch_tile_rc<NH>(dout + size_t(next) * kBT * 16, in + size_t(next) * kBT * 32, min(kBT, n_pts - next * kBT),
+                           stage0 + (buf ^ 1) * S::STAGE_BYTES);
     asm volatile("cp.async.commit_group;" ::: "memory");
     asm volatile("cp.async.wait_group 1;" ::: "memory");
     fence_async_smem();
@@ -507,6 +508,210 @@
   }
   __syncthreads();
   if (warp == 0) tmem_dealloc(tmem, S::TMEM_COLS);
+}
+
+
+template <int SCATTER_WARPS>
+struct FbsSmem {
+  using R = RcSmem<0>;
+  static constexpr int SLOTS = SCATTER_WARPS / 4 < 2 ? 2 : SCATTER_WARPS / 4;
+  static constexpr int RING = R::BAR;
+  static constexpr int SLOT_WORDS = F2B_N_LEVELS * kBT;
+  static constexpr int BAR = RING + SLOTS * SLOT_WORDS * 4;
+  static constexpr int BYTES = BAR + 16 * (SLOTS + 1) + 1024;
+  static constexpr int TMEM_COLS = R::TMEM_COLS;
+};
+
+__device__ __forceinline__ void tensor_bar() { asm volatile("bar.sync 1, 128;" ::: "memory"); }
+
+__device__ __forceinline__ void flush_field_wgrad(uint32_t tmem_row, int warp, int lane, float* __restrict__ dparams) {
+  using S = RcSmem<0>;
+  const int row = warp * 16 + lane;
+  float* g0 = dparams;
+  float* go = dparams + 64 * 32;
+#pragma unroll
+  for (int q = 0; q < 2; q++) {
+    uint32_t r[16];
+    tmem_ld16(tmem_row + S::C_GW0 + 16 * q, r);
+    tmem_ld_wait();
+    if (lane < 16)
+#pragma unroll
+      for (int e = 0; e < 16; e++) atomicAdd(g0 + row * 32 + 16 * q + e, __uint_as_float(r[e]));
+  }
+  uint32_t r[16];
+  tmem_ld16(tmem_row + S::C_GWO, r);
+  tmem_ld_wait();
+  if (lane < 16)
+#pragma unroll
+    for (int e = 0; e < 16; e++) atomicAdd(go + e * 64 + row, __uint_as_float(r[e]));
+}
+
+template <int SCATTER_WARPS, int MIN_CTAS>
+__global__ void __launch_bounds__(kBT + 32 * SCATTER_WARPS, MIN_CTAS)
+field_bwd_scatter_kernel(const __half* __restrict__ dout, const __half* __restrict__ in, const __half* __restrict__ params,
+                         int n_kept, const float* __restrict__ pts, const int* __restrict__ anchors, int n_edge,
+                         const float* __restrict__ e_pts, const int* __restrict__ e_anc, const int* __restrict__ prim_pool,
+                         const float* __restrict__ bias_pool, int n_volumes, int local_size, float grad_mul,
+                         float* __restrict__ dparams, float* __restrict__ grad_table, int flush_every) {
+  static_assert(SCATTER_WARPS % 4 == 0, "a tile's 128 rows are four 32-row scatter groups");
+  using S = RcSmem<0>;
+  using F = FbsSmem<SCATTER_WARPS>;
+  extern __shared__ unsigned char smem_raw[];
+  unsigned char* sm = reinterpret_cast<unsigned char*>((reinterpret_cast<uintptr_t>(smem_raw) + 1023) & ~uintptr_t(1023));
+  uint64_t* mbar = reinterpret_cast<uint64_t*>(sm + F::BAR);
+  uint64_t* full = mbar + 1;
+  uint64_t* empty = full + F::SLOTS;
+  uint32_t* tmem_slot = reinterpret_cast<uint32_t*>(empty + F::SLOTS);
+  uint32_t* ring = reinterpret_cast<uint32_t*>(sm + F::RING);
+  const int tid = threadIdx.x, warp = tid >> 5, lane = tid & 31;
+  const int tiles_k = (n_kept + kBT - 1) / kBT;
+  const int n_tiles = tiles_k + (n_edge + kBT - 1) / kBT;
+  const uint32_t stage0 = smem_u32(sm + S::STAGE0);
+  auto tile_rows = [&](int t, int64_t& row0) -> int {
+    if (t < tiles_k) { row0 = int64_t(t) * kBT; return min(kBT, n_kept - t * kBT); }
+    row0 = n_kept + int64_t(t - tiles_k) * kBT;
+    return min(kBT, n_edge - (t - tiles_k) * kBT);
+  };
+
+  if (warp < 4 && blockIdx.x < n_tiles) {
+    int64_t r0;
+    const int rows = tile_rows(blockIdx.x, r0);
+    prefetch_tile_rc<0>(dout + r0 * 16, in + r0 * 32, rows, stage0);
+    asm volatile("cp.async.commit_group;" ::: "memory");
+  }
+  stage_w<32>(params, 64, sm + S::W0);
+  stage_w<64>(params + 64 * 32, 16, sm + S::WO);
+  if (tid == 0) {
+    mbar_init(mbar, 1);
+    for (int s = 0; s < F::SLOTS; s++) { mbar_init(full + s, kBT); mbar_init(empty + s, 4); }
+  }
+  if (warp == 0) tmem_alloc(tmem_slot, F::TMEM_COLS);
+  fence_before_sync();
+  __syncthreads();
+  fence_after_sync();
+  const uint32_t tmem = *tmem_slot;
+
+  if (warp < 4) {
+    const uint32_t tmem_row = tmem + (uint32_t(warp * 32) << 16);
+    const uint32_t s_w0 = smem_u32(sm + S::W0), s_wo = smem_u32(sm + S::WO), s_h0 = smem_u32(sm + S::H0);
+    constexpr uint32_t id_fwd64 = idesc_f16_f32(128, 64);
+    constexpr uint32_t id_act64 = idesc_f16_f32(128, 64, 0, 1);
+    constexpr uint32_t id_act32 = idesc_f16_f32(128, 32, 0, 1);
+    constexpr uint32_t id_gw16 = idesc_f16_f32(64, 16, 1, 1);
+    constexpr uint32_t id_gw32 = idesc_f16_f32(64, 32, 1, 1);
+    uint32_t phase = 0, buf = 0;
+    int it = 0, since = 0;
+    for (int tile = blockIdx.x; tile < n_tiles; tile += gridDim.x, buf ^= 1, it++) {
+      const int next = tile + gridDim.x;
+      if (next < n_tiles) {
+        int64_t r0;
+        const int rows = tile_rows(next, r0);
+        prefetch_tile_rc<0>(dout + r0 * 16, in + r0 * 32, rows, stage0 + (buf ^ 1) * S::STAGE_BYTES);
+      }
+      asm volatile("cp.async.commit_group;" ::: "memory");
+      asm volatile("cp.async.wait_group 1;" ::: "memory");
+      fence_async_smem();
+      fence_before_sync();
+      tensor_bar();
+      const uint32_t sb = stage0 + buf * S::STAGE_BYTES;
+      const uint32_t s_do = sb + S::DO, s_x = sb + S::X;
+      const uint32_t acc = since != 0;
+      if (tid == 0) {
+        fence_after_sync();
+#pragma unroll
+        for (int k = 0; k < 2; k++) mma_f16(tmem + S::C_ACT, kmajor_desc(s_x + 32 * k, 64), kmajor_desc(s_w0 + 32 * k, 64), id_fwd64, k);
+        mma_commit(mbar);
+      }
+      mbar_wait(mbar, phase); phase ^= 1;
+      fence_after_sync();
+      relu_fwd_epilogue(tmem_row + S::C_ACT, sm + S::H0, tid);
+      fence_before_sync();
+      fence_async_smem();
+      tensor_bar();
+      if (tid == 0) {
+        fence_after_sync();
+        mma_f16(tmem + S::C_ACT, kmajor_desc(s_do, 32), mnmajor_desc(s_wo, 128, 0), id_act64, 0);
+#pragma unroll
+        for (int k = 0; k < 8; k++)
+          mma_f16(tmem + S::C_GWO, mnmajor_desc(s_h0, 128, k), mnmajor_desc(s_do, 32, k), id_gw16, (k > 0) | acc);
+        mma_commit(mbar);
+      }
+      mbar_wait(mbar, phase); phase ^= 1;
+      fence_after_sync();
+      relu_bwd_epilogue(tmem_row + S::C_ACT, sm + S::H0, sm + S::H0, tid);
+      fence_before_sync();
+      fence_async_smem();
+      tensor_bar();
+      if (tid == 0) {
+        fence_after_sync();
+#pragma unroll
+        for (int k = 0; k < 4; k++)
+          mma_f16(tmem + S::C_ACT, kmajor_desc(s_h0 + 32 * k, 128), mnmajor_desc(s_w0, 64, k), id_act32, k);
+#pragma unroll
+        for (int k = 0; k < 8; k++)
+          mma_f16(tmem + S::C_GW0, mnmajor_desc(s_h0, 128, k), mnmajor_desc(s_x, 64, k), id_gw32, (k > 0) | acc);
+        mma_commit(mbar);
+      }
+      since++;
+      mbar_wait(mbar, phase); phase ^= 1;
+      fence_after_sync();
+      const int slot = it % F::SLOTS;
+      mbar_wait(empty + slot, ((it / F::SLOTS) & 1) ^ 1);
+      uint32_t* dst = ring + slot * F::SLOT_WORDS + tid;
+#pragma unroll
+      for (int q = 0; q < 2; q++) {
+        uint32_t r[16];
+        tmem_ld16(tmem_row + S::C_ACT + 16 * q, r);
+        tmem_ld_wait();
+#pragma unroll
+        for (int e = 0; e < 8; e++) dst[(8 * q + e) * kBT] = pk(__uint_as_float(r[2 * e]), __uint_as_float(r[2 * e + 1]));
+      }
+      mbar_arrive(full + slot);
+      if (since == flush_every) { flush_field_wgrad(tmem_row, warp, lane, dparams); since = 0; }
+    }
+    asm volatile("cp.async.wait_group 0;" ::: "memory");
+    fence_before_sync();
+    tensor_bar();
+    if (since) {
+      fence_after_sync();
+      flush_field_wgrad(tmem_row, warp, lane, dparams);
+      fence_before_sync();
+    }
+  } else {
+    constexpr int kGroups = SCATTER_WARPS / 4;
+    const int sw = warp - 4, grp = sw >> 2, quarter = sw & 3;
+    int it = grp;
+    for (int tile = blockIdx.x + grp * gridDim.x; tile < n_tiles; tile += kGroups * gridDim.x, it += kGroups) {
+      const bool edge = tile >= tiles_k;
+      const int n_seg = edge ? n_edge : n_kept;
+      const int64_t i = int64_t(edge ? tile - tiles_k : tile) * kBT + quarter * 32 + lane;
+      const bool valid = i < n_seg;
+      float x0 = 0.f, x1 = 0.f, x2 = 0.f;
+      int v = -1;
+      if (valid) {
+        const float* p = (edge ? e_pts : pts) + i * 3;
+        const float p0 = __ldg(p), p1 = __ldg(p + 1), p2 = __ldg(p + 2);
+        x0 = fmul(fadd(p0, 1.f), .5f); x1 = fmul(fadd(p1, 1.f), .5f); x2 = fmul(fadd(p2, 1.f), .5f);
+        v = edge ? __ldg(e_anc + i) : __ldg(anchors + i * 3);
+      }
+      const int slot = it % F::SLOTS;
+      mbar_wait(full + slot, (it / F::SLOTS) & 1);
+      const uint32_t* src = ring + slot * F::SLOT_WORDS + quarter * 32 + lane;
+#pragma unroll 1
+      for (int l = 0; l < F2B_N_LEVELS; l++) {
+        const uint32_t w = src[l * kBT];
+        const float2 g = __half22float2(*reinterpret_cast<const __half2*>(&w));
+        hash_bwd_level(l, lane, valid, x0, x1, x2, v, g.x, g.y, prim_pool, bias_pool, n_volumes, local_size, grad_mul, grad_table);
+      }
+      __syncwarp();
+      if (lane == 0) mbar_arrive(empty + slot);
+    }
+  }
+  __syncthreads();
+  if (warp == 0) {
+    fence_after_sync();
+    tmem_dealloc(tmem, F::TMEM_COLS);
+  }
 }
 
 }
@@ -562,3 +767,48 @@
   return f2b_mlp_bwd2_tc(dout_f16, in_f16, h, h + size_t(n_hidden_matmuls ? 1 : 0) * n_pts * 64, params_f16, n_hidden_matmuls, n_pts,
                          din_f16, dparams_f32, stream);
 }
+
+template <int SW, int CTAS>
+static int launch_field_bwd_scatter(int grid, int flush_every, const void* dout_f16, const void* in_f16, const void* params_f16, int n_kept,
+                                    const float* pts, const int* anchors, int n_edge, const float* e_pts, const int* e_anc,
+                                    const int* prim_pool, const float* bias_pool, int n_volumes, int local_size, float grad_mul,
+                                    float* dparams_f32, float* grad_table, cudaStream_t st) {
+  cudaFuncSetAttribute(field_bwd_scatter_kernel<SW, CTAS>, cudaFuncAttributeMaxDynamicSharedMemorySize, FbsSmem<SW>::BYTES);
+  field_bwd_scatter_kernel<SW, CTAS><<<grid, kBT + 32 * SW, FbsSmem<SW>::BYTES, st>>>(
+      (const __half*)dout_f16, (const __half*)in_f16, (const __half*)params_f16, n_kept, pts, anchors, n_edge, e_pts, e_anc, prim_pool,
+      bias_pool, n_volumes, local_size, grad_mul, dparams_f32, grad_table, flush_every);
+  return check_launch("f2b_field_bwd_scatter");
+}
+
+extern "C" int f2b_field_bwd_scatter(const void* dout_f16, const void* in_f16, const void* params_f16, int n_kept, const float* pts,
+                                     const int* anchors, int n_edge, const float* e_pts, const int* e_anc, const int* prim_pool,
+                                     const float* bias_pool, int n_volumes, int local_size, float grad_mul, float* dparams_f32,
+                                     float* grad_table, void* stream) {
+  F2B_REQUIRE(n_kept >= 0 && n_edge >= 0, "f2b_field_bwd_scatter: negative row count");
+  if (n_kept + n_edge <= 0) return F2B_OK;
+  F2B_REQUIRE(dout_f16 && in_f16 && params_f16 && prim_pool && bias_pool && dparams_f32 && grad_table,
+              "f2b_field_bwd_scatter: null pointer");
+  F2B_REQUIRE((n_kept == 0 || (pts && anchors)) && (n_edge == 0 || (e_pts && e_anc)), "f2b_field_bwd_scatter: null point segment");
+  F2B_REQUIRE(n_volumes > 0 && local_size > 0 && (local_size % 2) == 0, "f2b_field_bwd_scatter: bad n_volumes/local_size");
+  static int warps = -1, ctas = -1;
+  if (warps < 0) {
+    const char* w = getenv("F2B_FBS_WARPS");
+    const char* c = getenv("F2B_FBS_CTAS");
+    warps = w ? atoi(w) : 8;
+    ctas = c ? atoi(c) : 2;
+    if (warps != 4 && warps != 12) warps = 8;
+    if (ctas != 3) ctas = 2;
+  }
+  int sms = 148;
+  f2b_device_info(&sms, nullptr);
+  const int n_tiles = div_up(n_kept, kBT) + div_up(n_edge, kBT);
+  const int grid = n_tiles < sms * ctas ? n_tiles : sms * ctas;
+  const cudaStream_t st = as_stream(stream);
+  const int flush_every = div_up(n_tiles, int64_t(sms) * 4);
+#define F2B_FBS(SW, CT) launch_field_bwd_scatter<SW, CT>(grid, flush_every, dout_f16, in_f16, params_f16, n_kept, pts, anchors, n_edge, e_pts, e_anc, \
+                                                         prim_pool, bias_pool, n_volumes, local_size, grad_mul, dparams_f32, grad_table, st)
+  if (warps == 12) return F2B_FBS(12, 2);
+  if (warps == 8) return ctas == 2 ? F2B_FBS(8, 2) : F2B_FBS(8, 3);
+  return ctas == 2 ? F2B_FBS(4, 2) : F2B_FBS(4, 3);
+#undef F2B_FBS
+}
diff --git a/f2nerf_b200/csrc/render.cu b/f2nerf_b200/csrc/render.cu
--- a/f2nerf_b200/csrc/render.cu
+++ b/f2nerf_b200/csrc/render.cu
@@ -1,4 +1,5 @@
 #include "common.cuh"
+#include <stdlib.h>
 
 namespace f2b {
 
@@ -37,6 +38,12 @@
   } while (0)
 
 static inline char* off(void* p, int64_t bytes) { return reinterpret_cast<char*>(p) + bytes; }
+
+static bool field_bwd_scatter_on() {
+  static int on = -1;
+  if (on < 0) { const char* e = getenv("F2B_FIELD_BWD_SCATTER"); on = !(e && atoi(e) == 0); }
+  return on != 0;
+}
 
 extern "C" int f2b_render_sizeof(void) { return (int)sizeof(f2b_render); }
 
@@ -88,6 +95,7 @@
   const int64_t nk = r->n_kept, ne = 2 * int64_t(r->n_edge_pairs), nq = nk + ne;
   cudaStream_t st = as_stream(r->stream), side = as_stream(r->side_stream);
   const bool emb = r->app_emb && r->ray_emb_idx;
+  const bool fused = r->scatter_mode == 0 && field_bwd_scatter_on();
   F2B_CUDA(cudaMemsetAsync(r->d_sparams, 0, sizeof(float) * r->n_shader_params, st), "f2b_render_bwd");
   F2B_CUDA(cudaMemsetAsync(r->d_fparams, 0, sizeof(float) * r->n_field_params, st), "f2b_render_bwd");
   F2B_CUDA(cudaMemsetAsync(r->d_table, 0, sizeof(float) * r->table_numel, st), "f2b_render_bwd");
@@ -105,8 +113,11 @@
                          r->stream));
     F2B_TRY(f2b_shader_prep_bwd_f16(r->d_in16, r->d_logit, r->new_bounds, emb ? r->ray_emb_idx : nullptr, r->n_rays,
                                     1.f / r->shader_loss_scale, r->field_loss_scale, r->d_scene16, emb ? r->d_app : nullptr, r->stream));
-    F2B_TRY(f2b_mlp_bwd2(r->d_scene16, r->feat_q, r->f_hidden, nullptr, r->fparams16, 0, (int)nk, r->dfeat16, r->d_fparams, r->stream));
+    if (!fused) F2B_TRY(f2b_mlp_bwd2(r->d_scene16, r->feat_q, r->f_hidden, nullptr, r->fparams16, 0, (int)nk, r->dfeat16, r->d_fparams, r->stream));
   }
+  if (fused)
+    return f2b_field_bwd_scatter(r->d_scene16, r->feat_q, r->fparams16, (int)nk, r->pts, r->anchors, (int)ne, r->e_pts, r->e_anc, r->prim,
+                                 r->bias, r->n_volumes, r->local_size, r->table_grad_mul, r->d_fparams, r->d_table, r->stream);
   if (ne > 0)
     F2B_TRY(f2b_mlp_bwd2(off(r->d_scene16, nk * 32), off(r->feat_q, nk * 64), r->f_hidden ? off(r->f_hidden, nk * 128) : nullptr, nullptr, r->fparams16, 0, (int)ne,
                          off(r->dfeat16, nk * 64), r->d_fparams, r->stream));
diff --git a/f2nerf_b200/csrc/tc.cuh b/f2nerf_b200/csrc/tc.cuh
--- a/f2nerf_b200/csrc/tc.cuh
+++ b/f2nerf_b200/csrc/tc.cuh
@@ -50,6 +50,9 @@
 __device__ __forceinline__ void mbar_init(uint64_t* mbar, uint32_t count) {
   asm volatile("mbarrier.init.shared::cta.b64 [%0], %1;" ::"r"(smem_u32(mbar)), "r"(count) : "memory");
 }
+__device__ __forceinline__ void mbar_arrive(uint64_t* mbar) {
+  asm volatile("mbarrier.arrive.shared::cta.b64 _, [%0];" ::"r"(smem_u32(mbar)) : "memory");
+}
 __device__ __forceinline__ void mbar_wait(uint64_t* mbar, uint32_t parity) {
   asm volatile(
       "{\n\t.reg .pred P1;\n\tLAB_WAIT:\n\t"
diff --git a/f2nerf_b200/ops.py b/f2nerf_b200/ops.py
--- a/f2nerf_b200/ops.py
+++ b/f2nerf_b200/ops.py
@@ -104,6 +104,16 @@
     return grad_table
 
 
+def field_bwd_scatter(d_out16, feat16, params16, pts, anchors, e_pts, e_anc, prim_pool, bias_pool, n_volumes, local_size, grad_mul,
+                      d_params, grad_table):
+    n_kept, n_edge = pts.shape[0], d_out16.shape[0] - pts.shape[0]
+    if n_edge and (e_pts is None or e_pts.shape[0] != n_edge):
+        raise ValueError("field_bwd_scatter: edge rows without their edge points")
+    call("f2b_field_bwd_scatter", d_out16, feat16, params16, n_kept, pts, anchors, n_edge, e_pts, e_anc, prim_pool, bias_pool,
+         int(n_volumes), int(local_size), float(grad_mul), d_params, grad_table, stream())
+    return d_params, grad_table
+
+
 def field_fwd(table_f16, prim_pool, bias_pool, n_volumes, local_size, params_f16, pts, vol, vol_stride=1, logit_only=False,
               save=False, save_feat=None):
     n = pts.shape[0]
diff --git a/f2nerf_b200/renderer.py b/f2nerf_b200/renderer.py
--- a/f2nerf_b200/renderer.py
+++ b/f2nerf_b200/renderer.py
@@ -497,8 +497,9 @@
         slab_hook = getattr(renderer, "grad_slab_hook_", None)
         f_scale = field.mlp_.loss_scale_
         grad_mul = (1.0 / f_scale) * (getattr(renderer, "grad_premul_", 1.0) if slab_hook is not None else 1.0)
+        two_kernel = slab_hook is not None or not _lib.FIELD_BWD_SCATTER
         B = dict(d_logit=f32(n_kept), d_raw=f16(n_kept, 16), d_in16=f16(n_kept, 32), d_scene16=f16(n_kept + n_edge, 16),
-                 dfeat16=f16(n_kept + n_edge, 32), d_sparams=f32(ra.n_shader_params), d_fparams=f32(ra.n_field_params),
+                 dfeat16=f16(n_kept + n_edge, 32) if two_kernel else None, d_sparams=f32(ra.n_shader_params), d_fparams=f32(ra.n_field_params),
                  d_table=renderer._table_grad_buffer(ctx.table_shape, dev),
                  nonfinite=torch.empty((2,), dtype=torch.int32, device=dev))
         if emb_on:
@@ -606,7 +607,7 @@
         nh_s, nh_f = shader.mlp_.n_hidden_matmuls, field.mlp_.n_hidden_matmuls
         f16 = lambda *sh: torch.empty(sh, dtype=torch.float16, device=dev)
         d_logit = torch.empty((n_kept,), dtype=torch.float32, device=dev)
-        d_raw, d_in16, d_scene16, dfeat16 = f16(n_kept, 16), f16(n_kept, 32), f16(n_q, 16), f16(n_q, 32)
+        d_raw, d_in16, d_scene16 = f16(n_kept, 16), f16(n_kept, 32), f16(n_q, 16)
         d_sparams, d_fparams = zeros(sparams16.numel()), zeros(fparams16.numel())
         d_table = torch.zeros_like(field.feat_pool_)
         d_app = torch.zeros_like(renderer.app_emb_) if ray_emb_idx is not None else None
@@ -634,6 +635,9 @@
             with torch.cuda.stream(side):
                 ops.hash_bwd(*hash_args, pts, anc, stride, dfeat16[s0:s1], grad_mul, d_table)
 
+        fused = (_lib.FIELD_BWD_SCATTER and slab_hook is None and len(ctx.cuts) == 1 and nh_f == 0
+                 and _lib.lib.f2b_get_mlp_impl() == 1)
+        dfeat16 = None if fused else f16(n_q, 32)
         for r0, r1, s0, s1 in ctx.cuts:
             if s1 <= s0:
                 continue
@@ -646,11 +650,17 @@
                  stream())
             ops.shader_prep_bwd_f16(d_in16, d_logit, bounds[r0:r1], None if ray_emb_idx is None else ray_emb_idx[r0:r1],
                                     1.0 / s_scale, f_scale, d_scene16, d_app)
+            if fused:
+                continue
             call("f2b_mlp_bwd2", d_scene16[s0:s1], feat16[s0:s1], None if f_hidden is None else f_hidden[0, s0:s1],
                  f_hidden[1, s0:s1] if (nh_f and f_hidden is not None) else None, fparams16, int(nh_f), ns, dfeat16[s0:s1], d_fparams,
                  stream())
             scatter(segments[0][0][s0:s1], segments[0][1][s0:s1], segments[0][2], s0, s1)
-        for pts_e, anc_e, stride_e, first, rows in segments[1:]:
+        if fused:
+            edge = segments[1] if len(segments) > 1 else (None, None, 1, n_kept, 0)
+            ops.field_bwd_scatter(d_scene16, feat16, fparams16, segments[0][0], segments[0][1], edge[0], edge[1], *hash_args,
+                                  grad_mul, d_fparams, d_table)
+        for pts_e, anc_e, stride_e, first, rows in ([] if fused else segments[1:]):
             if rows > 0:
                 call("f2b_mlp_bwd2", d_scene16[first:first + rows], feat16[first:first + rows],
                      None if f_hidden is None else f_hidden[0, first:first + rows],
diff --git a/f2nerf_b200/shim/B200Renderer.cpp b/f2nerf_b200/shim/B200Renderer.cpp
--- a/f2nerf_b200/shim/B200Renderer.cpp
+++ b/f2nerf_b200/shim/B200Renderer.cpp
@@ -46,6 +46,10 @@
 void* P(const Tensor& t) { return t.defined() ? t.data_ptr() : nullptr; }
 bool fused_forward() {
   static const bool on = [] { const char* e = getenv("F2B_FUSED_FORWARD"); return !e || atoi(e) != 0; }();
+  return on;
+}
+bool field_bwd_scatter() {
+  static const bool on = [] { const char* e = getenv("F2B_FIELD_BWD_SCATTER"); return !e || atoi(e) != 0; }();
   return on;
 }
 bool validate_weights() {
@@ -203,7 +207,7 @@
     const float s_scale = shader->mlp_->loss_scale_, f_scale = field->mlp_->loss_scale_;
     Tensor d_logit = torch::empty({n_kept}, CUDAFloat);
     Tensor d_raw = torch::empty({n_kept, 16}, kHalf), d_in16 = torch::empty({n_kept, 32}, kHalf);
-    Tensor d_scene16 = torch::empty({n_q, 16}, kHalf), dfeat16 = torch::empty({n_q, 32}, kHalf);
+    Tensor d_scene16 = torch::empty({n_q, 16}, kHalf);
     Tensor d_sparams = torch::zeros({k.sparams16.numel()}, CUDAFloat), d_fparams = torch::zeros({k.fparams16.numel()}, CUDAFloat);
     const int64_t table_numel = ctx->saved_data["table_numel"].toInt();
     const int local_size = ((field->pool_size_ / N_LEVELS) >> 4) << 4;
@@ -231,14 +235,22 @@
                            (int) n_kept, P(d_in16), PF(d_sparams), cur_stream()));
     F2B_CHECK(f2b_shader_prep_bwd_f16(P(d_in16), PF(d_logit), PI(k.bounds), emb_on ? PI(k.ray_emb_idx) : nullptr, n_rays,
                                       1.f / s_scale, f_scale, P(d_scene16), PF(d_app), cur_stream()));
-    F2B_CHECK(f2b_mlp_bwd2(P(d_scene16), P(k.feat16), P(k.f_hidden), nullptr, P(k.fparams16), 0, (int) n_q, P(dfeat16),
-                           PF(d_fparams), cur_stream()));
-    F2B_CHECK(f2b_hash_bwd(field->prim_pool_.data_ptr<int>(), field->bias_pool_.data_ptr<float>(), field->n_volumes_, local_size,
-                           PF(k.pts), PI(k.anchors), 3, (int) n_kept, P(dfeat16), 1, 1.f / f_scale, PF(d_table), cur_stream()));
-    if (n_q > n_kept) {
+    if (field_bwd_scatter()) {
+      F2B_CHECK(f2b_field_bwd_scatter(P(d_scene16), P(k.feat16), P(k.fparams16), (int) n_kept, PF(k.pts), PI(k.anchors),
+                                      (int) (n_q - n_kept), n_q > n_kept ? PF(k.e_pts) : nullptr, n_q > n_kept ? PI(k.e_anc) : nullptr,
+                                      field->prim_pool_.data_ptr<int>(), field->bias_pool_.data_ptr<float>(), field->n_volumes_,
+                                      local_size, 1.f / f_scale, PF(d_fparams), PF(d_table), cur_stream()));
+    } else {
+      Tensor dfeat16 = torch::empty({n_q, 32}, kHalf);
+      F2B_CHECK(f2b_mlp_bwd2(P(d_scene16), P(k.feat16), P(k.f_hidden), nullptr, P(k.fparams16), 0, (int) n_q, P(dfeat16),
+                             PF(d_fparams), cur_stream()));
       F2B_CHECK(f2b_hash_bwd(field->prim_pool_.data_ptr<int>(), field->bias_pool_.data_ptr<float>(), field->n_volumes_, local_size,
-                             PF(k.e_pts), PI(k.e_anc), 1, (int) (n_q - n_kept), (char*) P(dfeat16) + n_kept * 64, 1, 1.f / f_scale,
-                             PF(d_table), cur_stream()));
+                             PF(k.pts), PI(k.anchors), 3, (int) n_kept, P(dfeat16), 1, 1.f / f_scale, PF(d_table), cur_stream()));
+      if (n_q > n_kept) {
+        F2B_CHECK(f2b_hash_bwd(field->prim_pool_.data_ptr<int>(), field->bias_pool_.data_ptr<float>(), field->n_volumes_, local_size,
+                               PF(k.e_pts), PI(k.e_anc), 1, (int) (n_q - n_kept), (char*) P(dfeat16) + n_kept * 64, 1, 1.f / f_scale,
+                               PF(d_table), cur_stream()));
+      }
     }
     d_sparams = d_sparams / s_scale;
     d_fparams = d_fparams / f_scale;
diff --git a/include/f2nerf_b200.h b/include/f2nerf_b200.h
--- a/include/f2nerf_b200.h
+++ b/include/f2nerf_b200.h
@@ -110,6 +110,10 @@
                            void* hidden_save_f16 , void* stream);
 int f2b_mlp_bwd2(const void* dout_f16, const void* in_f16, const void* hidden0_f16, const void* hidden1_f16,
                  const void* params_f16, int n_hidden_matmuls, int n_pts, void* din_f16, float* dparams_f32, void* stream);
+int f2b_field_bwd_scatter(const void* dout_f16, const void* in_f16, const void* params_f16, int n_kept, const float* pts,
+                          const int* anchors, int n_edge, const float* e_pts, const int* e_anc, const int* prim_pool,
+                          const float* bias_pool, int n_volumes, int local_size, float grad_mul, float* dparams_f32,
+                          float* grad_table, void* stream);
 
 int f2b_set_mlp_impl(int impl);
 int f2b_get_mlp_impl(void);
@@ -213,7 +217,7 @@
   float* colors; float* disparity; float* depth; float* weights;
   const float* d_colors; const float* d_disparity; const float* d_depth; const float* d_weights; const float* d_edge ;
   float gs_progress, shader_loss_scale, field_loss_scale, table_grad_mul;
-  float* d_logit; void* d_raw; void* d_in16; void* d_scene16; void* dfeat16;
+  float* d_logit; void* d_raw; void* d_in16; void* d_scene16; void* dfeat16 ;
   float* d_sparams; float* d_fparams; float* d_table; int64_t table_numel; int64_t table_live; float* d_app;
   int scatter_mode;
   int* nonfinite;
```

Measured after the change: 996,500, median of 6. 5.6% higher.
